# jeffreychou777/GenComm

Hardware: AMD Instinct MI355X
Metric: scenes/sec (higher is better)
Workload: dtype f32

## Files before the change

gencomm_amd/_lib.py:

```python
from __future__ import annotations

import ctypes as C
import os
import shutil
import subprocess
import threading
from typing import List, Tuple

PKG_DIR = os.path.dirname(os.path.abspath(__file__))
REPO_DIR = os.path.dirname(PKG_DIR)
CSRC_DIR = os.path.join(PKG_DIR, "csrc")
LIB_PATH = os.environ.get("GENCOMM_HIP_LIB", os.path.join(PKG_DIR, "libgencomm_hip.so"))
ABI_VERSION = 12
MODE_ARITH, MODE_SAMPLER, MODE_TILE_WANT, MODE_ENH_FUSE, MODE_CONV8H_MASK, MODE_XCD_REMAP, MODE_DATAFLOW, MODE_RESFUSE_EMU, MODE_TILE8, MODE_BWD_STREAMS, MODE_PERSIST = range(11)

_lock = threading.Lock()
_lib = None

c_float_p = C.c_void_p
_i, _ll, _p = C.c_int, C.c_longlong, C.c_void_p

_SIGNATURES = {
    "gencomm_abi_version": (_i, []),
    "gencomm_last_error": (C.c_char_p, []),
    "gencomm_build_info": (C.c_char_p, []),
    "gencomm_set_mode": (_i, [_i, _ll]),
    "gencomm_get_mode": (_ll, [_i]),
    "gencomm_timer_num_kernels": (_i, []),
    "gencomm_timer_kernel_name": (C.c_char_p, [_i]),
    "gencomm_timer_start": (_i, [_i, _i]),
    "gencomm_timer_stop": (_i, [C.POINTER(C.c_double), C.POINTER(_i)]),
    "gencomm_timer_start_mask": (_i, [C.c_ulonglong, _i]),
    "gencomm_timer_stop_families": (_i, [C.POINTER(C.c_double), C.POINTER(_i), C.POINTER(C.c_double), _i]),
    "gencomm_klog_start": (_i, []),
    "gencomm_klog_stop": (_i, [C.c_char_p, _i]),
    "gencomm_clock_probe": (_i, [_p, _i, _p]),
    "gencomm_quad_iou_fwd": (_i, [_p, _i, _p, _i, _p, _p]),
    "gencomm_unet_num_params": (_i, [_i, _i, _i, _i]),
    "gencomm_unet_param_info": (_i, [_i, _i, _i, _i, _i, C.c_char_p, _i, C.POINTER(_ll), C.POINTER(_ll)]),
    "gencomm_unet_raw_floats": (_ll, [_i, _i, _i, _i]),
    "gencomm_unet_prepared_floats": (_ll, [_i, _i, _i, _i, _i]),
    "gencomm_unet_prepare": (_i, [_p, _p, _i, _i, _i, _i, _i, _p]),
    "gencomm_unet_bwd_workspace_bytes": (_ll, [_i, _i, _i, _i, _i, _i, _i]),
    "gencomm_unet_fwd_train": (_i, [_p, _p, _p, _p, _i, _i, _i, _i, _i, _i, _i, _i, _i, _p, _ll, _p]),
    "gencomm_unet_fwd_train_step": (_i, [_p, _p, _p, _p, _i, _p, _p, C.c_ulonglong, _i, _i, _i, _i, _i, _i, _i, _i, _p, _ll, _p]),
    "gencomm_unet_bwd": (_i, [_p, _p, _p, _p, _i, _p, _p, _p, _p, _i, _i, _i, _i, _i, _i, _i, _i, _i, _p, _ll, _p]),
    "gencomm_unet_bwd_chain": (_i, [_p, _p, _p, _p, _i, _p, C.c_float, C.c_float, _p, _p, _p, _p, _i, _i, _i, _i, _i, _i, _i, _i, _i, _p, _ll, _p]),
    "gencomm_conv8_fwd": (_i, [_p, _p, _p, _p, _p, _p, _i, _i, _i, _i, _p]),
    "gencomm_denoise_workspace_bytes": (_ll, [_i, _i, _i, _i, _i, _i, _i]),
    "gencomm_dataflow_error": (_i, [_p, _i, _i, _i, _i, _i, _i, _i, _p]),
    "gencomm_dataflow_words": (_i, [_p, _i, _i, _i, _i, _i, _i, _i, C.POINTER(C.c_uint), _i, _p]),
    "gencomm_unet_fwd": (_i, [_p, _p, _p, _p, _i, _i, _i, _i, _i, _i, _i, _i, _i, _p, _ll, _p]),
    "gencomm_denoise_fwd": (_i, [_p, _p, _p, _i, _p, _p, _p, _p, _p, C.c_ulonglong,
                                 _i, _i, _i, _i, _i, _i, _i, _i, _p, _ll, _p]),
    "gencomm_denoise_fwd_dseed": (_i, [_p, _p, _p, _i, _p, _p, _p, _p, _p, C.c_ulonglong, _p,
                                       _i, _i, _i, _i, _i, _i, _i, _i, _p, _ll, _p]),
    "gencomm_q_sample_fwd": (_i, [_p, _p, _i, _p, _p, C.c_ulonglong, C.c_uint, _p, _i, _i, _i, _i, _p]),
    "gencomm_step_noise_fwd": (_i, [_p, C.c_ulonglong, C.c_uint, _p, _i, _i, _i, _i, _i, _p]),
    "gencomm_enhancer_num_params": (_i, [_i]),
    "gencomm_enhancer_param_info": (_i, [_i, _i, C.c_char_p, _i, C.POINTER(_ll), C.POINTER(_ll)]),
    "gencomm_enhancer_raw_floats": (_ll, [_i]),
    "gencomm_enhancer_workspace_bytes": (_ll, [_i, _i, _i, _i]),
    "gencomm_enhancer_fwd": (_i, [_p, _p, _p, _i, _i, _i, _i, _p, _ll, _p]),
    "gencomm_msgext_num_params": (_i, [_i]),
    "gencomm_msgext_param_info": (_i, [_i, _i, C.c_char_p, _i, C.POINTER(_ll), C.POINTER(_ll)]),
    "gencomm_msgext_raw_floats": (_ll, [_i]),
    "gencomm_msgext_workspace_bytes": (_ll, [_i, _i, _i, _i]),
    "gencomm_msgext_fwd": (_i, [_p, _p, _p, _i, _i, _i, _i, _p, _ll, _p]),
    "gencomm_pillar_encode_fwd": (_i, [_p, _p, _p, _p, _p, _p, _p, _p, _p, _p, _i, _i, _i, _i, _i,
                                       C.POINTER(C.c_float), C.POINTER(C.c_float), _p]),
    "gencomm_conv2d_prepare": (_i, [_p, _p, _i, _i, _i, _i, _i, _p]),
    "gencomm_conv2d_prepared_floats": (_ll, [_i, _i, _i, _i, _i]),
    "gencomm_conv2d_fold": (_i, [_p, _p, _p, _p, _p, C.c_float, _i, _p, _p, _p]),
    "gencomm_conv2d_fwd": (_i, [_p, _p, _p, _p, _p] + [_i] * 13 + [_p]),
    "gencomm_conv2d_act_res_fwd": (_i, [_p, _p, _p, _p, _p, _p] + [_i] * 10 + [_p]),
    "gencomm_split3_attn_fwd": (_i, [_p] * 10 + [_i, _i, _i, _p]),
    "gencomm_warp_affine_bwd": (_i, [_p, _p, _p, _i, _i, _i, _i, _p]),
    "gencomm_hgt_attn_bwd": (_i, [_p, _p, _p, _p, _i, _i, _i, _i, _p]),
    "gencomm_win_attn_bwd_scratch_floats": (_ll, [_i, _i, _i, _i, _i]),
    "gencomm_win_attn_bwd": (_i, [_p] * 7 + [_i] * 6 + [_p]),
    "gencomm_conv2d_wgrad": (_i, [_p, _p, _p, _p, _i, _i, _i, _i, _i, _i, _i, _i, _p]),
    "gencomm_conv2d_wgrad_scratch_floats": (_ll, [_i] * 8),
    "gencomm_conv2d_wgrad_ws": (_i, [_p, _p, _p, _p, _i, _i, _i, _i, _i, _i, _i, _i, _p, _ll, _p]),
    "gencomm_conv2d_wgrad_fixed_scratch_floats": (_ll, [_i] * 6),
    "gencomm_conv2d_wgrad_fixed": (_i, [_p, _p, _p, _p, _i, _i, _i, _i, _i, _i, _p, _ll, _p]),
    "gencomm_gn_nchw_fwd": (_i, [_p, _p, _p, _p, _p, C.c_float, _i, _i, _i, _i, _i, _p]),
    "gencomm_ln_nchw_fwd": (_i, [_p, _p, _p, _p, C.c_float, _i, _i, _i, _i, _p]),
    "gencomm_ln_nchw_bwd": (_i, [_p, _p, _p, _p, _p, _p, _p, C.c_float, _i, _i, _i, _i, _p]),
    "gencomm_dwconv3x3_fwd": (_i, [_p, _p, _p, _p, _i, _i, _i, _i, _i, _p]),
    "gencomm_dwconv3x3_wgrad": (_i, [_p, _p, _p, _p, _i, _i, _i, _i, _p]),
    "gencomm_conv3x3_c16_scratch_floats": (_ll, []),
    "gencomm_conv3x3_c16_fwd": (_i, [_p, _i, _p, _i, _p, _i, _p, _i, _i, _i, _p]),
    "gencomm_dwconv3x3_act_fwd": (_i, [_p, _i, _i, _p, _p, _p, _i, _i, _i, _i, _i, _p]),
    "gencomm_dwconv3x3_act_wgrad": (_i, [_p, _i, _i, _p, _p, _p, _i, _i, _i, _i, _p]),
    "gencomm_gelu_bwd": (_i, [_p, _p, _p, _ll, _p]),
    "gencomm_lincomb_fwd": (_i, [_p, _p, _p, _p, C.c_float, C.c_float, C.c_float, _ll, _p]),
    "gencomm_ew_slice_fwd": (_i, [_i, _p, _p, _p, _p, _p, _p] + [_i] * 9 + [_p]),
    "gencomm_nc_scale_fwd": (_i, [_p, _p, _p, _p, _i, _i, _i, _p]),
    "gencomm_nc_dot_fwd": (_i, [_p, _p, _p, _i, _i, _i, _p]),
    "gencomm_det_workspace_bytes": (C.c_longlong, [_i, _i, _i]),
    "gencomm_nms_workspace_bytes": (C.c_longlong, []),
    "gencomm_nms_max_candidates": (_i, []),
    "gencomm_det_decode_fwd": (_i, [_p, _p, _p, _p, _p, _i, _i, _i, _i, C.c_float, C.c_float, _i, _p, _p, _p, _p, _i, _p, C.c_longlong, _p]),
    "gencomm_nms_rotated_fwd": (_i, [_p, _p, _p, C.c_float, _i, _p, _p, _p, _p, _p, _p, C.c_longlong, _p]),
    "gencomm_bbox_overlaps_fwd": (_i, [_p, _p, _p, _i, _i, _p]),
    "gencomm_det_mc_workspace_bytes": (_ll, [_p, _p, _i, _i]),
    "gencomm_det_mc_decode_fwd": (_i, [_p, _p, _p, _p, _p, _p, _i, _i, _i, C.c_float, _i, _p, _p, _p, _p, _p, _p, _i, _p, _ll, _p]),
    "gencomm_det_mc_gather_fwd": (_i, [_p, _p, _p, _p, _p, _i, _i, _p, _p, _p]),
    "gencomm_warp_affine_fwd": (_i, [_p, _p, _p, _i, _i, _i, _i, _p]),
    "gencomm_hgt_attn_fwd": (_i, [_p, _p, _p, _i, _i, _i, _i, _p]),
    "gencomm_win_attn_fwd": (_i, [_p, _p, _p, _i, _i, _i, _i, _i, _i, _p]),
    "gencomm_swap_attn_fwd": (_i, [_p, _p, _p, _p] + [_i] * 8 + [_p]),
    "gencomm_swap_attn_train_fwd": (_i, [_p] * 5 + [_i] * 8 + [_p]),
    "gencomm_swap_attn_bwd": (_i, [_p] * 8 + [_i] * 8 + [_p]),
    "gencomm_agent_mean_fwd": (_i, [_p, _p, _i, _i, _ll, _p]),
    "gencomm_v2v_warp_pairs_fwd": (_i, [_p, _p, _p, _p, _i, _i, _i, _i, _p]),
    "gencomm_v2v_aggregate_fwd": (_i, [_p] * 7 + [_i] * 6 + [_p]),
    "gencomm_gru_gate_fwd": (_i, [_p, _p, _i, _i, _i, _p]),
    "gencomm_gru_gate_bwd": (_i, [_p, _p, _p, _i, _i, _i, _p]),
    "gencomm_v2v_aggregate_train_fwd": (_i, [_p] * 8 + [_i] * 6 + [_p]),
    "gencomm_v2v_aggregate_bwd": (_i, [_p] * 7 + [_i] * 6 + [_p]),
    "gencomm_v2v_warp_pairs_bwd_scratch_floats": (_ll, [_i]),
    "gencomm_v2v_warp_pairs_bwd": (_i, [_p] * 7 + [_i] * 6 + [_p]),
    "gencomm_umgm_param_floats": (_ll, [_i, _i, C.POINTER(_i), _i]),
    "gencomm_umgm_workspace_bytes": (_ll, [_ll, _i]),
    "gencomm_umgm_fwd": (_i, [_p, _p, _p, _p, C.c_ulonglong, _i, _p, _p, _p, _p, _p, _ll, _i, _i, _i, C.POINTER(_i), _i, _p, _ll, _p]),
    "gencomm_umgm_encode_fwd": (_i, [_p, _p, _p, _ll, _i, _i, _i, C.POINTER(_i), _i, _p]),
    "gencomm_umgm_decode_fwd": (_i, [_p, _p, _p, _ll, _i, _i, _i, C.POINTER(_i), _i, _p]),
    "gencomm_umgm_noise_fwd": (_i, [_p, C.c_ulonglong, _ll, _i, C.POINTER(_i), _i, _p]),
    "gencomm_umgm_bwd_workspace_bytes": (_ll, [_ll, _i, _i, C.POINTER(_i), _i]),
    "gencomm_umgm_bwd": (_i, [_p, _p, _p, _p, C.c_ulonglong, _i, _p, _p, _p, _p, _p, _i, _ll, _i, _i, _i, C.POINTER(_i), _i, _p, _ll, _p]),
    "gencomm_rows_wgrad_fixed_scratch_floats": (_ll, [_ll, _i, _i]),
    "gencomm_rows_wgrad_fixed": (_i, [_p, _p, _p, _ll, _i, _i, _p, _ll, _p]),
    "gencomm_convnext_block_fwd": (_i, [_p] * 11 + [_i] * 4 + [_p]),
    "gencomm_convnext_block_bwd_workspace_bytes": (_ll, [_i] * 6),
    "gencomm_convnext_block_bwd": (_i, [_p] * 21 + [_i] * 6 + [_p, _ll, _p]),
    "gencomm_gconv3x3_prepare": (_i, [_p, _p, _i, _p]),
    "gencomm_gconv3x3_fwd": (_i, [_p] * 5 + [_i] * 7 + [_p]),
    "gencomm_pyramid_score_fwd": (_i, [_p] * 6 + [_i] * 4 + [_p]),
    "gencomm_warp_weightfuse_fwd": (_i, [_p] * 5 + [_i] * 5 + [_p]),
    "gencomm_iou3d_pairwise_fwd": (_i, [_p, _i, _p, _i, _i, _p, _p]),
    "gencomm_iou3d_max_boxes": (_i, []),
    "gencomm_iou3d_nms_workspace_bytes": (_ll, [_i]),
    "gencomm_iou3d_nms_fwd": (_i, [_p, _i, C.c_float, _i, _p, _p, _p, _ll, _p]),
    "gencomm_bn2d_train_fwd": (_i, [_p, _p, _p, _p, _p, _p, _p, _p, C.c_float, C.c_float, _i, _i, _i, _i, _p, _p]),
    "gencomm_bn2d_train_bwd": (_i, [_p, _p, _p, _p, _p, _p, _p, _p, _p, _i, _i, _i, _i, _p]),
    "gencomm_slot_max_fwd": (_i, [_p, _p, _p, _i, _i, _i, _p]),
    "gencomm_convbn_train_fwd": (_i, [_p] * 10 + [C.c_float, C.c_float, _i] + [_p] * 5 + [_i] * 8 + [_p]),
    "gencomm_convbn_train_bwd": (_i, [_p] * 9 + [_i] + [_p] * 9 + [_ll] + [_i] * 7 + [_p]),
    "gencomm_pfn_train_fwd": (_i, [_p, _p, _p, _p, _p, _p, _p, C.c_float, C.c_float, _p, _p, _p, _p, _i, _i, _i, _i, _p]),
    "gencomm_pfn_train_bwd": (_i, [_p, _p, _p, _p, _p, _p, _p, _p, _p, _p, _p, _p, _i, _i, _i, _i, _p]),
    "gencomm_pfn_moment_doubles": (_ll, [_i]),
    "gencomm_pfn_bwd_scratch_doubles": (_ll, [_i, _i]),
    "gencomm_slot_max_bwd": (_i, [_p, _p, _p, _i, _i, _i, _p]),
    "gencomm_head_loss": (_i, [_p] * 10 + [_i] * 5 + [_p, C.c_double] + [C.c_float] * 7 + [_i, _p]),
    "gencomm_head_loss_mc": (_i, [_p] * 4 + [_i] + [_p] * 4 + [_i] * 5 + [C.c_double] * 2 + [_p]),
    "gencomm_target_assign_workspace_bytes": (_ll, [_i, _i, _i]),
    "gencomm_target_standup_fwd": (_i, [_p, _i, _i, _p, _p]),
    "gencomm_target_assign_fwd": (_i, [_p, _i, _i, _p, _i, _p, _p, _p, _p] + [_i] * 6 + [_p, _p, _p, _i, _p, _ll, _p]),
    "gencomm_dcn_sample_fwd": (_i, [_p, _p, _p, _i, _i, _i, _i, _p]),
    "gencomm_dcn_scatter_bwd": (_i, [_p, _p, _p, _p, _p, _i, _i, _i, _i, _p]),
    "gencomm_dcn_scatter_scratch_floats": (_ll, [_i, _i, _i, _i]),
    "gencomm_dcn_scatter_bwd_ws": (_i, [_p, _p, _p, _p, _p, _i, _i, _i, _i, _p, _ll, _p]),
    "gencomm_sp_out_dims": (_i, [_p, _p, _p, _p, _p]),
    "gencomm_sp_index_workspace_bytes": (_ll, [_i]),
    "gencomm_sp_index_fwd": (_i, [_p, _i, _i, _p, _p, _p, _p, _ll, _p]),
    "gencomm_sp_sites_capacity": (_ll, [_i, _p, _p]),
    "gencomm_sp_sites_workspace_bytes": (_ll, [_i, _p, _p]),
    "gencomm_sp_sites_fwd": (_i, [_p, _i, _i, _p, _p, _p, _p, _p, _p, _p, _ll, _p]),
    "gencomm_sp_rules_fwd": (_i, [_p, _i, _p, _i, _i, _p, _p, _p, _p, _p, _p]),
    "gencomm_sp_prepared_floats": (_ll, [_i, _i, _i]),
    "gencomm_sp_prepare": (_i, [_p, _p, _i, _i, _i, _i, _p]),
    "gencomm_sp_conv_fwd": (_i, [_p, _p, _p, _p, _p, _p, _i, _i, _i, _i, _i, _p]),
    "gencomm_sp_dense_fwd": (_i, [_p, _p, _i, _i, _i, _p, _p, _p]),
    "gencomm_mean_vfe_fwd": (_i, [_p, _p, _p, _p, _i, _i, _i, _p]),
    "gencomm_bnrow_train_fwd": (_i, [_p, _p, _p, _p, _p, _p, _p, _p, C.c_float, C.c_float, _i, _i, _i, _p]),
    "gencomm_bnrow_train_bwd": (_i, [_p, _p, _p, _p, _p, _p, _p, _p, _p, _i, _i, _i, _p]),
    "gencomm_sp_rules_inv_fwd": (_i, [_p, _i, _p, _i, _i, _p, _p, _p, _p, _p, _p]),
    "gencomm_sp_wgrad": (_i, [_p, _p, _p, _p, _i, _i, _i, _i, _p]),
    "gencomm_voxelize_workspace_bytes": (_ll, [_i]),
    "gencomm_voxelize_fwd": (_i, [_p, _i, _i, C.POINTER(C.c_float), C.POINTER(C.c_float), _i, _i, _p, _p, _p, _p, _p, _ll, _p]),
    "gencomm_voxelize_batch_workspace_bytes": (_ll, [_i, _i, _i]),
    "gencomm_voxelize_batch_fwd": (_i, [_p, _i, _i, _p, _i, _p, _p, _i, C.POINTER(C.c_float), C.POINTER(C.c_float), _i, _i, _i, _p, _p, _p, _p, _p, _p, _ll, _p]),
    "gencomm_warp_attfuse_fwd": (_i, [_p, _p, _p, _p, _i, _i, _i, _i, _i, _p]),
    "gencomm_warp_attfuse_bwd_scratch_floats": (_ll, [_i, _i, _i]),
    "gencomm_warp_attfuse_bwd": (_i, [_p, _p, _p, _p, _p, _p, _i, _i, _i, _i, _i, _p]),
    "gencomm_warp_maxfuse_fwd": (_i, [_p, _p, _p, _p, _i, _i, _i, _i, _i, _p]),
    "gencomm_warp_maxfuse_bwd_scratch_floats": (_ll, [_i, _i, _i, _i, _i]),
    "gencomm_warp_maxfuse_bwd": (_i, [_p, _p, _p, _p, _p, _p, _i, _i, _i, _i, _i, _p]),
    "gencomm_warp_attfuse_tok_fwd": (_i, [_p, _p, _p, _p, _i, _i, _i, _i, _i, _p]),
    "gencomm_lss_workspace_bytes": (_ll, [_i, _i, _i, _i, _i, _i, C.POINTER(_i)]),
    "gencomm_lss_splat_fwd": (_i, [_p] * 8 + [C.POINTER(C.c_float), C.POINTER(C.c_float), C.POINTER(_i)] + [_i] * 6 + [_p, _p, _p, _ll, _p]),
    "gencomm_lss_depth_target_fwd": (_i, [_p, _i, _i, _i, _i, _i, _i, C.c_float, C.c_float, _i, _p, _p, _p]),
    "gencomm_maxpool3x3s2_fwd": (_i, [_p, _p, _i, _i, _i, _i, _p]),
    "gencomm_lss_splat_bwd_workspace_bytes": (_ll, [_i, _i, C.POINTER(_i)]),
    "gencomm_lss_splat_bwd": (_i, [_p, _p, _ll, _p, C.POINTER(_i)] + [_i] * 6 + [_p, _p, _p, _ll, _p]),
    "gencomm_maxpool3x3s2_bwd": (_i, [_p, _p, _p, _i, _i, _i, _i, _p]),
    "gencomm_stem7x7_wgrad_scratch_floats": (_ll, [_i] * 5),
    "gencomm_stem7x7_wgrad": (_i, [_p, _p, _p] + [_i] * 5 + [_p, _ll, _p]),
    "gencomm_depth_focal_loss": (_i, [_p, _p, _p, _p, _i, _i, _i, _i, C.c_float, C.c_float, C.c_float, _p]),
}
EXPORTED_SYMBOLS = tuple(_SIGNATURES)


class GenCommHipError(RuntimeError):
    pass


def hip_sources() -> List[str]:
    return [os.path.join(CSRC_DIR, "gencomm_abi.hip"), os.path.join(CSRC_DIR, "gencomm_abi_aux.hip")]


def source_hash() -> str:
    import hashlib
    h = hashlib.sha256()
    for f in sorted(os.listdir(CSRC_DIR)) + [os.path.join(REPO_DIR, "include", "gencomm_hip.h")]:
# ... 144 lines not shown
```

gencomm_amd/csrc/common.h:

```cpp
#pragma once
#include <hip/hip_runtime.h>
#include <stdint.h>
#include <stdio.h>
#include <string.h>

namespace gc {

constexpr int kWave = 64;
constexpr int kMaxResBlocks = 48;

enum Status : int {
  GC_OK = 0,
  GC_ERR_ARG = 1,
  GC_ERR_WORKSPACE = 2,
  GC_ERR_HIP = 3,
};

char* last_error_buf();
inline int fail(int code, const char* msg) {
  snprintf(last_error_buf(), 512, "%s", msg);
  return code;
}
#define GC_CHECK_ARG(cond, msg) \
  do {                          \
    if (!(cond)) return ::gc::fail(::gc::GC_ERR_ARG, msg); \
  } while (0)
#define GC_HIP(expr)                                                             \
  do {                                                                           \
    hipError_t e__ = (expr);                                                     \
    if (e__ != hipSuccess) {                                                     \
      snprintf(::gc::last_error_buf(), 512, "%s failed: %s", #expr, hipGetErrorString(e__)); \
      return ::gc::GC_ERR_HIP;                                                   \
    }                                                                            \
  } while (0)

struct LdsAttrOnce {
  unsigned long long done = 0;
  template <class K>
  int set(K kernel, int bytes) {
    int d = 0;
    GC_HIP(hipGetDevice(&d));
    const unsigned long long bit = d < 64 ? 1ull << d : 0ull;
    if (done & bit) return 0;
    GC_HIP(hipFuncSetAttribute((const void*)kernel, hipFuncAttributeMaxDynamicSharedMemorySize, bytes));
    __atomic_fetch_or(&done, bit, __ATOMIC_RELAXED);
    return 0;
  }
};

inline size_t align_up(size_t v, size_t a) { return (v + a - 1) / a * a; }

enum ModeKey : int {
  MODE_ARITH = 0,
  MODE_SAMPLER = 1,
  MODE_TILE_WANT = 2,
  MODE_ENH_FUSE = 3,
  MODE_CONV8H_MASK = 4,
  MODE_XCD_REMAP = 5,
  MODE_DATAFLOW = 6,
  MODE_RESFUSE_EMU = 7,
  MODE_TILE8 = 8,
  MODE_BWD_STREAMS = 9,
  MODE_PERSIST = 10,
  MODE_COUNT = 11
};
struct Modes {
  long long v[MODE_COUNT];
  bool split() const { return v[MODE_ARITH] != 1; }
  bool split2() const { return v[MODE_ARITH] == 3; }
  bool bf16() const { return v[MODE_ARITH] == 2; }
  int xcd() const { return v[MODE_XCD_REMAP] != 0 ? 1 : 0; }
};
Modes modes_snapshot();

enum KernelFamily : int {
  KF_CONV_IN = 0, KF_CONV8 = 1, KF_CONV16 = 2, KF_DOWN = 3, KF_UP = 4, KF_CONV_OUT = 5, KF_Q_SAMPLE = 6,
  KF_ENH_LN = 7, KF_ENH_PCONV = 8, KF_ENH_GEMM1 = 9, KF_ENH_DWGATE = 10, KF_ENH_GEMM2 = 11,
  KF_ENH_GATE = 12, KF_ENH_OUT = 13, KF_WARP_ATTFUSE = 14, KF_LATENT_STEP = 15, KF_CONV8_RES1 = 16, KF_CONV8_RES2 = 17,
  KF_DATAFLOW = 18,
  KF_CONV2D = 19,
  KF_COUNT = 20
};
inline const char* kernel_family_name(int id) {
  static const char* names[KF_COUNT] = {
      "conv_in_h_kernel | conv_in_kernel", "conv8h_kernel<1,GN,0> | conv8_kernel (ResnetBlock conv1, 8 -> 8)",
      "conv8h_kernel<2,GN,0> | conv8_kernel (ResnetBlock conv1, 16 -> 8)", "down8x2_kernel | down8_kernel",
      "conv8h_kernel<UP> | conv8_kernel<UP>", "conv_out_h_kernel | conv_out_kernel", "q_sample_kernel", "enh_ln_kernel",
      "enh_pconv_h_kernel | enh_pconv_kernel", "enh_front_h_kernel | gemm_*_mfma_kernel<0>", "enh_dwgate_kernel",
      "gemm_*_mfma_kernel<1>", "enh_gate_kernel", "enh_scale_transpose_kernel", "warp_attfuse_kernel | warp_attfuse_tok_kernel",
      "latent_step_h_kernel | latent_step_kernel", "conv8h_kernel<1,GN,RES=1> | conv8_kernel (ResnetBlock conv2 + identity)",
      "conv8h_kernel<1,GN,RES=2> | conv8_kernel (ResnetBlock conv2 + nin_shortcut)",
      "unet_dataflow_kernel (UNet body of one call, persistent)",
      "conv2d_h3l_kernel | conv2d_h3_kernel | conv2d_igemm_kernel (general 3x3 / 1x1 / 2x2 convolution; slot = FLOPs)"};
  return (id >= 0 && id < KF_COUNT) ? names[id] : "?";
}
struct KernelTimer {
  unsigned long long mask = 0;
  int cap = 0, count = 0;
  hipEvent_t* ev = nullptr;
  int* fam = nullptr;
  double* bytes = nullptr;
};
KernelTimer& kernel_timer();
struct TimedLaunch {
  bool armed;
  hipStream_t st;
  TimedLaunch(int family, hipStream_t s, double algorithmic_bytes = 0.0) : st(s) {
    KernelTimer& t = kernel_timer();
    armed = ((t.mask >> family) & 1ull) && t.count < t.cap;
    if (armed) {
      t.fam[t.count] = family;
      t.bytes[t.count] = algorithmic_bytes;
      (void)hipEventRecord(t.ev[2 * t.count], st);
    }
  }
  ~TimedLaunch() {
    if (armed) {
      KernelTimer& t = kernel_timer();
      (void)hipEventRecord(t.ev[2 * t.count + 1], st);
      ++t.count;
    }
  }
};

bool klog_armed();
void klog_note(const char* name);
#define GC_KLOG(name)                                   \
  do {                                                  \
    if (::gc::klog_armed()) ::gc::klog_note(name);      \
  } while (0)

typedef const float __attribute__((address_space(4)))* cfloat_p;
__device__ __forceinline__ cfloat_p as_const(const float* p) { return (cfloat_p)(p); }

struct BlockId { int x, y, z; };
__device__ __forceinline__ BlockId xcd_block_dims(int remap, unsigned lin, unsigned gx, unsigned gy, unsigned total) {
  unsigned nl = lin;
  if (remap) {
    const unsigned xcd = lin & 7u, j = lin >> 3;
    const unsigned q = total >> 3, r = total & 7u;
    nl = xcd * q + (xcd < r ? xcd : r) + j;
  }
  BlockId b;
  const unsigned row = nl / gx;
  b.x = (int)(nl - row * gx);
  b.z = (int)(row / gy);
  b.y = (int)(row - (unsigned)b.z * gy);
  return b;
}
__device__ __forceinline__ BlockId xcd_block_lin(int remap, unsigned lin) {
  const unsigned gx = gridDim.x, gy = gridDim.y;
  BlockId b;
  {
    const unsigned row = lin / gx;
    b.x = (int)(lin - row * gx);
    b.z = (int)(row / gy);
    b.y = (int)(row - (unsigned)b.z * gy);
  }
  if (remap) {
    const unsigned total = gx * gy * gridDim.z;
    const unsigned xcd = lin & 7u, j = lin >> 3;
    const unsigned q = total >> 3, r = total & 7u;
    const unsigned nl = xcd * q + (xcd < r ? xcd : r) + j;
    const unsigned row = nl / gx;
    b.x = (int)(nl - row * gx);
    b.z = (int)(row / gy);
    b.y = (int)(row - (unsigned)b.z * gy);
  }
  return b;
}
__device__ __forceinline__ BlockId xcd_block(int remap) {
  BlockId b{(int)blockIdx.x, (int)blockIdx.y, (int)blockIdx.z};
  if (remap) {
    const unsigned gx = gridDim.x, gy = gridDim.y;
    const unsigned total = gx * gy * gridDim.z;
    const unsigned lin = blockIdx.x + gx * (blockIdx.y + gy * blockIdx.z);
    const unsigned xcd = lin & 7u, j = lin >> 3;
    const unsigned q = total >> 3, r = total & 7u;
    const unsigned nl = xcd * q + (xcd < r ? xcd : r) + j;
    const unsigned row = nl / gx;
    b.x = (int)(nl - row * gx);
    b.z = (int)(row / gy);
    b.y = (int)(row - (unsigned)b.z * gy);
  }
  return b;
}

__device__ __forceinline__ float sigmoid_f(float x) {
  return __builtin_amdgcn_rcpf(1.0f + __builtin_amdgcn_exp2f(x * -1.4426950408889634f));
}
__device__ __forceinline__ float silu_f(float x) { return x * sigmoid_f(x); }
__device__ __forceinline__ float gelu_erf_f(float x) {
  const float t = fminf(fabsf(x) * 0.70710678118654752440f, 4.3f);
  float q = fmaf(-1.0021018e-4f, t, 4.6151079e-4f);
  q = fmaf(q, t, 2.3023714e-3f);
  q = fmaf(q, t, -2.9452650e-2f);
  q = fmaf(q, t, 1.4896373e-1f);
  q = fmaf(q, t, 9.1832864e-1f);
  q = fmaf(q, t, 1.6279137e+0f);
  const float erf_abs = 1.0f - __builtin_amdgcn_exp2f(-t * q);
  const float h = 0.5f * x;
  return fmaf(h, copysignf(erf_abs, x), h);
}
__device__ __forceinline__ void gelu_and_grad_f(float x, float* gelu, float* grad) {
  const float t = fminf(fabsf(x) * 0.70710678118654752440f, 4.3f);
  float q = fmaf(-1.0021018e-4f, t, 4.6151079e-4f);
  q = fmaf(q, t, 2.3023714e-3f);
  q = fmaf(q, t, -2.9452650e-2f);
  q = fmaf(q, t, 1.4896373e-1f);
  q = fmaf(q, t, 9.1832864e-1f);
  q = fmaf(q, t, 1.6279137e+0f);
  const float erf_abs = 1.0f - __builtin_amdgcn_exp2f(-t * q);
  const float Phi = fmaf(0.5f, copysignf(erf_abs, x), 0.5f);
  const float phi = 0.3989422804014327f * __builtin_amdgcn_exp2f(x * x * -0.72134752044448170368f);
  *gelu = x * Phi;
  *grad = fmaf(x, phi, Phi);
}
// ... 205 lines not shown
```

gencomm_amd/csrc/enhancer_host.h:

```cpp
#pragma once
#include <algorithm>
#include <stdlib.h>
#include <string.h>
#include <string>
#include <vector>

#include "enhancer_kernels.h"
#include "unet_plan.h"

namespace gc {

struct EnhancerPlan {
  int C = 0, dc = 0, dcp = 0, hid = 0;
  std::vector<ParamEntry> params;
  long long raw_floats = 0;
  long long n1w, n1b, n2w, n2b, pcw, l1w, l1b, dww, dwb, l2w, l2b, fc1, bnw, bnb, fc2;

  long long add(const std::string& name, long long numel) {
    params.push_back({name, numel, raw_floats});
    const long long o = raw_floats;
    raw_floats += numel;
    return o;
  }
  const char* build(int C_) {
    if (C_ < 8 || C_ % 8 != 0) return "enhancer: C must be a positive multiple of 8";
    C = C_; dc = C / 4; dcp = (dc + 15) / 16 * 16; hid = 2 * C;
    params.clear(); raw_floats = 0;
    n1w = add("block_1.norm1.weight", C);
    n1b = add("block_1.norm1.bias", C);
    n2w = add("block_1.norm2.weight", C);
    n2b = add("block_1.norm2.bias", C);
    pcw = add("block_1.mlp.partial_conv3.weight", (long long)dc * dc * 9);
    l1w = add("block_1.mlp.linear1.0.weight", (long long)2 * hid * C);
    l1b = add("block_1.mlp.linear1.0.bias", 2 * hid);
    dww = add("block_1.mlp.dwconv.0.weight", (long long)hid * 9);
    dwb = add("block_1.mlp.dwconv.0.bias", hid);
    l2w = add("block_1.mlp.linear2.0.weight", (long long)C * hid);
    l2b = add("block_1.mlp.linear2.0.bias", C);
    fc1 = add("split_attn.fc1.weight", (long long)C * C);
    bnw = add("split_attn.bn1.weight", C);
    bnb = add("split_attn.bn1.bias", C);
    fc2 = add("split_attn.fc2.weight", (long long)C * C);
    return nullptr;
  }
};

struct EnhancerWs {
  size_t Y, Z, Zc, Hd, G, O, colsum, gate, wT, tab1, tab2, wsc, total;
};

inline EnhancerWs enhancer_ws(const EnhancerPlan& p, int n, int H, int W) {
  const size_t M = (size_t)n * H * W;
  EnhancerWs w{};
  size_t off = 0;
  auto take = [&](size_t floats) { const size_t o = off; off += align_up(floats * sizeof(float), 256); return o; };
  w.colsum = take((size_t)n * p.C);
  w.gate = take((size_t)n * p.C);
  w.wT = take(std::max((size_t)9 * p.dc * p.dcp, (size_t)(p.dc / 16) * ((9 * p.dc + 31) / 32) * 896 + 64));
  w.Y = take(M * p.C);
  w.Z = take(M * p.C);
  w.Zc = take(M * p.dc);
  w.Hd = take(M * 2 * p.hid);
  w.G = take(M * p.hid);
  w.O = w.Hd;
  w.tab1 = take((size_t)(p.hid / 16) * (p.C / 16) * 896);
  w.tab2 = take((size_t)(p.hid / 16) * (p.C / 32 > 0 ? p.C / 32 : 1) * 896);
  w.wsc = take(64);
  w.total = off;
  return w;
}
inline int enh_fuse_level(const Modes& m, int C) { return (m.split() && C == 64) ? (int)m.v[MODE_ENH_FUSE] : 0; }
inline size_t enhancer_workspace_bytes(const EnhancerPlan& p, int n, int H, int W) { return enhancer_ws(p, n, H, W).total; }

inline int enhancer_enqueue(const EnhancerPlan& p, const float* raw, const float* x, float* out,
                            int n, int H, int W, char* wsp, hipStream_t st, const Modes& m) {
  const EnhancerWs w = enhancer_ws(p, n, H, W);
  const int HW = H * W, C = p.C;
  auto F = [&](size_t off) { return reinterpret_cast<float*>(wsp + off); };
  GC_HIP(hipMemsetAsync(F(w.colsum), 0, (size_t)n * C * sizeof(float), st));

  {
    EnhLnArgs a{x, raw + p.n1w, raw + p.n1b, raw + p.n2w, raw + p.n2b, F(w.Y), F(w.Z), F(w.Zc), C, p.dc, HW};
    const size_t sh = ((size_t)C * 65 + 256 + 128) * sizeof(float);
    if (sh > 48 * 1024) GC_HIP(hipFuncSetAttribute((const void*)enh_ln_kernel, hipFuncAttributeMaxDynamicSharedMemorySize, (int)sh));
    TimedLaunch tl(KF_ENH_LN, st);
    if (C == 64) enh_ln64_kernel<<<dim3((HW + 255) / 256, n), 256, 0, st>>>(a);
    else enh_ln_kernel<<<dim3((HW + 63) / 64, n), 256, sh, st>>>(a);
  }
  if (m.split() && (p.dc == 16 || p.dc == 32 || p.dc == 64) && (C & 3) == 0) {
    const int nslice = (9 * p.dc + 31) / 32;
    enh_prep_pconv_h_kernel<<<(p.dc / 16) * nslice * 4, 256, 0, st>>>(raw + p.pcw, F(w.wT), p.dc, nslice);
    TimedLaunch tl(KF_ENH_PCONV, st);
    EnhPconvHArgs a{F(w.Zc), F(w.wT), F(w.Z), C, p.dc, H, W, nslice};
    const bool wide = p.dc <= 32 && (long long)((W + 31) / 32) * ((H + 15) / 16) * n >= 256;
    const size_t sh = (size_t)18 * (wide ? 34 : 18) * p.dc * 5;
    if (wide) {
      if (sh > 48 * 1024) GC_HIP(hipFuncSetAttribute((const void*)enh_pconv_h_kernel<32>, hipFuncAttributeMaxDynamicSharedMemorySize, (int)sh));
      enh_pconv_h_kernel<32><<<dim3((W + 31) / 32, (H + 15) / 16, n), 256, sh, st>>>(a);
    } else {
      if (sh > 48 * 1024) GC_HIP(hipFuncSetAttribute((const void*)enh_pconv_h_kernel<16>, hipFuncAttributeMaxDynamicSharedMemorySize, (int)sh));
      enh_pconv_h_kernel<16><<<dim3((W + 15) / 16, (H + 15) / 16, n), 256, sh, st>>>(a);
    }
  } else
  {
    enh_prep_pconv_kernel<<<(9 * p.dc * p.dcp + 255) / 256, 256, 0, st>>>(raw + p.pcw, F(w.wT), p.dc, p.dcp);
    TimedLaunch tl(KF_ENH_PCONV, st);
    EnhPconvArgs a{F(w.Zc), F(w.wT), F(w.Z), C, p.dc, p.dcp, H, W};
    if (p.dc <= 32) {
      const size_t sh = (size_t)18 * 18 * (p.dc + 1) * sizeof(float);
      enh_pconv_kernel<16, 16><<<dim3((W + 15) / 16, (H + 15) / 16, n), 256, sh, st>>>(a);
    } else {
      const size_t sh = (size_t)10 * 18 * (p.dc + 1) * sizeof(float);
      if (sh > 48 * 1024) GC_HIP(hipFuncSetAttribute((const void*)enh_pconv_kernel<16, 8>, hipFuncAttributeMaxDynamicSharedMemorySize, (int)sh));
      enh_pconv_kernel<16, 8><<<dim3((W + 15) / 16, (H + 7) / 8, n), 128, sh, st>>>(a);
    }
  }
  const int fuse = enh_fuse_level(m, C);
  if (fuse != 0) {
    enh_wscale_kernel<<<2, 256, 0, st>>>(raw + p.l1w, (long long)2 * p.hid * C, raw + p.l2w, (long long)C * p.hid, F(w.wsc));
    enh_prep_front_kernel<<<32, 256, 0, st>>>(raw + p.l1w, F(w.tab1), C, p.hid, F(w.wsc));
    if (fuse >= 2) enh_prep_back_kernel<<<16, 256, 0, st>>>(raw + p.l2w, F(w.tab2), C, p.hid, F(w.wsc));
    EnhFrontArgs a{F(w.Z), F(w.tab1), raw + p.l1b, raw + p.dww, raw + p.dwb, F(w.G), C, p.hid, H, W,
                   F(w.tab2), raw + p.l2b, F(w.Y), F(w.O), F(w.colsum), F(w.wsc)};
    TimedLaunch tl(KF_ENH_GEMM1, st);
    if (fuse >= 2) enh_front_h_kernel<true><<<dim3((W + 7) / 8, (H + 7) / 8, n), 256, 0, st>>>(a);
    else enh_front_h_kernel<false><<<dim3((W + 7) / 8, (H + 7) / 8, n), 256, 0, st>>>(a);
  } else {
  {
    GemmArgs a{F(w.Z), raw + p.l1w, raw + p.l1b, nullptr, F(w.Hd), nullptr, HW, 2 * p.hid, C};
    TimedLaunch tl(KF_ENH_GEMM1, st);
    if (m.split() && (C & 3) == 0) gemm_f16s_mfma_kernel<0><<<dim3((HW + 127) / 128, (2 * p.hid + 63) / 64, n), 256, 0, st>>>(a);
    else gemm_f32_mfma_kernel<0><<<dim3((HW + 127) / 128, (2 * p.hid + 63) / 64, n), 256, 0, st>>>(a);
  }
  {
    constexpr int SL = 8;
    EnhDwArgs a{F(w.Hd), raw + p.dww, raw + p.dwb, F(w.G), p.hid, H, W};
    const long long total = (long long)H * ((W + SL - 1) / SL) * p.hid;
    TimedLaunch tl(KF_ENH_DWGATE, st);
    enh_dwgate_kernel<SL><<<dim3((unsigned)((total + 255) / 256), n), 256, 0, st>>>(a);
  }
  }
  float* const Otok = F(w.O);
  if (fuse < 2) {
    GemmArgs a{F(w.G), raw + p.l2w, raw + p.l2b, F(w.Y), F(w.O), F(w.colsum), HW, C, p.hid};
    TimedLaunch tl(KF_ENH_GEMM2, st);
    if (m.split() && (p.hid & 3) == 0) gemm_f16s_mfma_kernel<1><<<dim3((HW + 127) / 128, (C + 63) / 64, n), 256, 0, st>>>(a);
    else gemm_f32_mfma_kernel<1><<<dim3((HW + 127) / 128, (C + 63) / 64, n), 256, 0, st>>>(a);
  }
  {
    EnhGateArgs a{F(w.colsum), raw + p.fc1, raw + p.bnw, raw + p.bnb, raw + p.fc2, F(w.gate), C, 1.0f / (float)HW};
    TimedLaunch tl(KF_ENH_GATE, st);
    enh_gate_kernel<<<n, 256, (2 * C + 8) * sizeof(float), st>>>(a);
  }
  if (out != nullptr) {
    EnhOutArgs a{Otok, F(w.gate), out, C, HW};
    const size_t sh = (size_t)32 * (C + 1) * sizeof(float);
    TimedLaunch tl(KF_ENH_OUT, st);
    enh_scale_transpose_kernel<<<dim3((HW + 31) / 32, n), 256, sh, st>>>(a);
  }
  GC_HIP(hipGetLastError());
  return GC_OK;
}

}
```

gencomm_amd/csrc/enhancer_kernels.h:

```cpp
#pragma once
#include "common.h"

namespace gc {

using f32x16 = __attribute__((ext_vector_type(16))) float;
using ef32x4 = __attribute__((ext_vector_type(4))) float;

struct EnhLnArgs {
  const float* x;
  const float* g1; const float* b1; const float* g2; const float* b2;
  float* Y; float* Z; float* Zc;
  int C, dc, HW;
};

__global__ __launch_bounds__(256) void enh_ln_kernel(const EnhLnArgs a) {
  extern __shared__ float smem[];
  const int C = a.C, S = 65;
  float* tile = smem;
  float* part = smem + (size_t)C * S;
  float* mu = part + 256;
  float* rs = mu + 64;
  const int tid = threadIdx.x, q = tid >> 6, p = tid & 63;
  const int n = blockIdx.y, p0 = blockIdx.x * 64;
  const int np = min(64, a.HW - p0);
  const bool pv = p < np;
  const float* __restrict__ xp = a.x + (size_t)n * C * a.HW + p0;
  for (int c = q; c < C; c += 4) tile[c * S + p] = pv ? xp[(size_t)c * a.HW + p] : 0.f;
  __syncthreads();
  const float invC = 1.0f / (float)C;

  auto moments = [&](float eps) {
    float s = 0.f;
    for (int c = q; c < C; c += 4) s += tile[c * S + p];
    part[q * 64 + p] = s;
    __syncthreads();
    const float m = (part[p] + part[64 + p] + part[128 + p] + part[192 + p]) * invC;
    __syncthreads();
    float v = 0.f;
    for (int c = q; c < C; c += 4) { const float d = tile[c * S + p] - m; v = fmaf(d, d, v); }
    part[q * 64 + p] = v;
    __syncthreads();
    const float var = (part[p] + part[64 + p] + part[128 + p] + part[192 + p]) * invC;
    __syncthreads();
    if (q == 0) { mu[p] = m; rs[p] = 1.0f / sqrtf(var + eps); }
    __syncthreads();
  };

  moments(1e-5f);
  {
    const float m = mu[p], r = rs[p];
    for (int c = q; c < C; c += 4) {
      const float v = tile[c * S + p];
      tile[c * S + p] = v + fmaf((v - m) * r, a.g1[c], a.b1[c]);
    }
  }
  __syncthreads();
  moments(1e-5f);

  float* __restrict__ Yp = a.Y + ((size_t)n * a.HW + p0) * C;
  float* __restrict__ Zp = a.Z + ((size_t)n * a.HW + p0) * C;
  float* __restrict__ Zcp = a.Zc + ((size_t)n * a.HW + p0) * a.dc;
  const int tot = np * C;
  for (int i = tid; i < tot; i += 256) {
    const int pp = i / C, c = i - pp * C;
    const float y = tile[c * S + pp];
    const float z = fmaf((y - mu[pp]) * rs[pp], a.g2[c], a.b2[c]);
    Yp[i] = y;
    Zp[i] = z;
    if (c < a.dc) Zcp[pp * a.dc + c] = z;
  }
}

__global__ __launch_bounds__(256) void enh_ln64_kernel(const EnhLnArgs a) {
  constexpr int C = 64, S = 65;
  __shared__ float tile[4][64 * S];
  const int tid = threadIdx.x, wv = tid >> 6, p = tid & 63;
  const int n = blockIdx.y, p0 = (blockIdx.x * 4 + wv) * 64;
  if (p0 >= a.HW) return;
  const int np = min(64, a.HW - p0);
  const bool pv = p < np;
  const float* __restrict__ xp = a.x + (size_t)n * C * a.HW + p0 + p;
  float v[C];
#pragma unroll
  for (int c = 0; c < C; ++c) v[c] = pv ? xp[(size_t)c * a.HW] : 0.f;
  const float invC = 1.0f / (float)C;
  float s = 0.f;
#pragma unroll
  for (int c = 0; c < C; ++c) s += v[c];
  float m = s * invC, q = 0.f;
#pragma unroll
  for (int c = 0; c < C; ++c) { const float d = v[c] - m; q = fmaf(d, d, q); }
  float r = 1.0f / sqrtf(q * invC + 1e-5f);
#pragma unroll
  for (int c = 0; c < C; ++c) v[c] = v[c] + fmaf((v[c] - m) * r, as_const(a.g1)[c], as_const(a.b1)[c]);
  s = 0.f;
#pragma unroll
  for (int c = 0; c < C; ++c) s += v[c];
  m = s * invC; q = 0.f;
#pragma unroll
  for (int c = 0; c < C; ++c) { const float d = v[c] - m; q = fmaf(d, d, q); }
  r = 1.0f / sqrtf(q * invC + 1e-5f);
  float* __restrict__ tw = tile[wv];
  float* __restrict__ Yp = a.Y + ((size_t)n * a.HW + p0) * C;
  float* __restrict__ Zp = a.Z + ((size_t)n * a.HW + p0) * C;
  float* __restrict__ Zcp = a.Zc + ((size_t)n * a.HW + p0) * a.dc;
  const int tot = np * C;
#pragma unroll
  for (int c = 0; c < C; ++c) tw[p * S + c] = v[c];
  __builtin_amdgcn_wave_barrier();
  for (int i = p; i < tot; i += 64) Yp[i] = tw[(i >> 6) * S + (i & 63)];
  __builtin_amdgcn_wave_barrier();
#pragma unroll
  for (int c = 0; c < C; ++c) tw[p * S + c] = fmaf((v[c] - m) * r, as_const(a.g2)[c], as_const(a.b2)[c]);
  __builtin_amdgcn_wave_barrier();
  for (int i = p; i < tot; i += 64) Zp[i] = tw[(i >> 6) * S + (i & 63)];
  const int totc = np * a.dc;
  for (int i = p; i < totc; i += 64) { const int pp = i / a.dc, c = i - pp * a.dc; Zcp[i] = tw[pp * S + c]; }
}

struct EnhPconvArgs {
  const float* Zc;
  const float* wT;
  float* Z;
  int C, dc, dcp, H, W;
};

template <int TW, int TH>
__global__ __launch_bounds__(TW * TH) void enh_pconv_kernel(const EnhPconvArgs a) {
  extern __shared__ float smem[];
  const int dc = a.dc, PS = dc + 1;
  constexpr int LW = TW + 2, LH = TH + 2;
  const int tid = threadIdx.x, n = blockIdx.z;
  const int x0 = blockIdx.x * TW, y0 = blockIdx.y * TH;
  const float* __restrict__ zp = a.Zc + (size_t)n * a.H * a.W * dc;
  for (int i = tid; i < LH * LW * dc; i += TW * TH) {
    const int pix = i / dc, c = i - pix * dc;
    const int r = pix / LW, col = pix - r * LW;
    const int gy = y0 - 1 + r, gx = x0 - 1 + col;
    float v = 0.f;
    if (gy >= 0 && gy < a.H && gx >= 0 && gx < a.W) v = zp[((size_t)gy * a.W + gx) * dc + c];
    smem[pix * PS + c] = v;
  }
  __syncthreads();
  const int tx = tid % TW, ty = tid / TW;
  const int gy = y0 + ty, gx = x0 + tx;
  const bool ok = gy < a.H && gx < a.W;
  float* __restrict__ op = a.Z + ((size_t)n * a.H * a.W + (size_t)gy * a.W + gx) * a.C;
  for (int ob = 0; ob < dc; ob += 16) {
    float acc[16];
#pragma unroll
    for (int o = 0; o < 16; ++o) acc[o] = 0.f;
#pragma unroll 1
    for (int tap = 0; tap < 9; ++tap) {
      const int dy = tap / 3, dx = tap - dy * 3;
      const float* sp = smem + ((ty + dy) * LW + tx + dx) * PS;
      const float* __restrict__ wp = a.wT + (size_t)tap * dc * a.dcp + ob;
#pragma unroll 4
      for (int ic = 0; ic < dc; ++ic) {
        const float v = sp[ic];
#pragma unroll
        for (int o = 0; o < 16; ++o) acc[o] = fmaf(wp[(size_t)ic * a.dcp + o], v, acc[o]);
      }
    }
    if (ok) {
#pragma unroll
      for (int o = 0; o < 16; ++o) if (ob + o < dc) op[ob + o] = acc[o];
    }
  }
}

__global__ void enh_prep_pconv_kernel(const float* __restrict__ w, float* __restrict__ wT, int dc, int dcp) {
  const int total = 9 * dc * dcp;
  for (int i = blockIdx.x * blockDim.x + threadIdx.x; i < total; i += gridDim.x * blockDim.x) {
    const int tap = i / (dc * dcp), rem = i - tap * dc * dcp, ic = rem / dcp, oc = rem - ic * dcp;
    wT[i] = oc < dc ? w[((size_t)oc * dc + ic) * 9 + tap] : 0.f;
  }
}

struct GemmArgs {
  const float* A; const float* Bw; const float* bias; const float* res;
  float* out; float* colsum;
  int M, N, K;
};

template <int EPI>
__global__ __launch_bounds__(256) void gemm_f32_mfma_kernel(const GemmArgs a) {
  constexpr int BM = 128, BN = 64, KC = 32, S = KC + 2;
  __shared__ __align__(16) float As[BM * S];
  __shared__ __align__(16) float Bs[BN * S];
  const int tid = threadIdx.x, w = tid >> 6, l = tid & 63, r = l & 31, h = l >> 5;
  const int ag = blockIdx.z;
  const int m0 = blockIdx.x * BM, n0 = blockIdx.y * BN;
  const float* __restrict__ Ap = a.A + (size_t)ag * a.M * a.K;
  const bool kvec = (a.K & 3) == 0;

  f32x16 acc0, acc1;
#pragma unroll
  for (int i = 0; i < 16; ++i) { acc0[i] = 0.f; acc1[i] = 0.f; }

  for (int k0 = 0; k0 < a.K; k0 += KC) {
    __syncthreads();
    {
      const int kq = tid & 7, gk = k0 + 4 * kq;
#pragma unroll
      for (int i = 0; i < 4; ++i) {
        const int row = (tid >> 3) + 32 * i, gm = m0 + row;
        float4 v = make_float4(0.f, 0.f, 0.f, 0.f);
        if (gm < a.M) {
          const float* src = Ap + (size_t)gm * a.K + gk;
          if (kvec && gk + 3 < a.K) v = *reinterpret_cast<const float4*>(src);
          else {
            if (gk + 0 < a.K) v.x = src[0];
            if (gk + 1 < a.K) v.y = src[1];
            if (gk + 2 < a.K) v.z = src[2];
            if (gk + 3 < a.K) v.w = src[3];
          }
        }
        float* d = &As[row * S + 4 * kq];
        *reinterpret_cast<float2*>(d) = make_float2(v.x, v.y);
        *reinterpret_cast<float2*>(d + 2) = make_float2(v.z, v.w);
      }
#pragma unroll
      for (int i = 0; i < 2; ++i) {
        const int row = (tid >> 3) + 32 * i, gn = n0 + row;
        float4 v = make_float4(0.f, 0.f, 0.f, 0.f);
        if (gn < a.N) {
          const float* src = a.Bw + (size_t)gn * a.K + gk;
          if (kvec && gk + 3 < a.K) v = *reinterpret_cast<const float4*>(src);
          else {
            if (gk + 0 < a.K) v.x = src[0];
// ... 688 lines not shown
```

gencomm_amd/csrc/gencomm_abi.hip:

```cpp
#include "../../include/gencomm_hip.h"

#include "common.h"
#include "conv_kernels.h"
#include "detect_kernels.h"
#include "enhancer_host.h"
#include "fusion_kernels.h"
#include "msgext_host.h"
#include "noise_kernels.h"
#include "pillar_kernels.h"
#include "pfn_kernels.h"
#include "train_kernels.h"
#include "wgrad_h3_kernels.h"
#include "unet_bwd_host.h"
#include "unet_host.h"

#include <algorithm>
#include <atomic>
#include <map>
#include <mutex>
#include <string>
#include <stdlib.h>
#include <string.h>

namespace gc {
char* last_error_buf() {
  static thread_local char buf[512] = {0};
  return buf;
}
KernelTimer& kernel_timer() {
  static KernelTimer t;
  return t;
}
static std::atomic<long long> g_modes[MODE_COUNT] = {{0}, {0}, {0}, {2}, {-1}, {1}, {0}, {0}, {-1}, {1}, {16}};
static std::atomic<bool> g_klog_armed{false};
static std::mutex g_klog_mu;
static std::map<std::string, int> g_klog;
bool klog_armed() { return g_klog_armed.load(std::memory_order_relaxed); }
void klog_note(const char* name) {
  std::lock_guard<std::mutex> lk(g_klog_mu);
  ++g_klog[name];
}
Modes modes_snapshot() {
  Modes m;
  for (int i = 0; i < MODE_COUNT; ++i) m.v[i] = g_modes[i].load(std::memory_order_relaxed);
  return m;
}
}

using namespace gc;

extern "C" {

int gencomm_abi_version(void) { return GENCOMM_ABI_VERSION; }
#ifndef GENCOMM_BUILD_FLAGS
#define GENCOMM_BUILD_FLAGS "unknown"
#endif
const char* gencomm_build_info(void) { return GENCOMM_BUILD_FLAGS; }
const char* gencomm_last_error(void) { return last_error_buf(); }

int gencomm_set_mode(int key, long long value) {
  GC_CHECK_ARG(key >= 0 && key < MODE_COUNT, "unknown mode key");
  GC_CHECK_ARG(key != MODE_ARITH || (value >= 0 && value <= 3), "GENCOMM_MODE_ARITH: 0 (three-term f16-pipe path), 1 (exact fp32), 2 (bf16 denoise) or 3 (0 + two-term general convolutions)");
  GC_CHECK_ARG(key != MODE_SAMPLER || (value >= 0 && value <= 2), "GENCOMM_MODE_SAMPLER: 0 (automatic), 1 (direct) or 2 (latent)");
  GC_CHECK_ARG(key != MODE_TILE_WANT || value >= 0, "GENCOMM_MODE_TILE_WANT: 0 (automatic) or a positive workgroup count");
  GC_CHECK_ARG(key != MODE_TILE8 || value >= -1, "GENCOMM_MODE_TILE8: -1 (automatic), 0 (off) or a positive workgroup count");
  GC_CHECK_ARG(key != MODE_BWD_STREAMS || (value >= 0 && value <= 2), "GENCOMM_MODE_BWD_STREAMS: 0 (off), 1 (automatic) or 2 (always)");
  GC_CHECK_ARG(key != MODE_PERSIST || (value >= 0 && value <= 31), "GENCOMM_MODE_PERSIST: a mask of the five layer variants (0 .. 31)");
  g_modes[key].store(value, std::memory_order_relaxed);
  return GC_OK;
}
long long gencomm_get_mode(int key) {
  if (key < 0 || key >= MODE_COUNT) { fail(GC_ERR_ARG, "unknown mode key"); return -1; }
  return g_modes[key].load(std::memory_order_relaxed);
}

int gencomm_timer_num_kernels(void) { return KF_COUNT; }
const char* gencomm_timer_kernel_name(int family) { return kernel_family_name(family); }

int gencomm_timer_start_mask(unsigned long long mask, int capacity) {
  KernelTimer& t = kernel_timer();
  GC_CHECK_ARG(t.ev == nullptr, "timer already armed");
  GC_CHECK_ARG(mask != 0 && (mask >> KF_COUNT) == 0 && capacity >= 1 && capacity <= (1 << 20), "bad family mask / capacity");
  t.ev = new hipEvent_t[2 * (size_t)capacity];
  for (int i = 0; i < 2 * capacity; ++i) {
    if (hipEventCreate(&t.ev[i]) != hipSuccess) {
      for (int j = 0; j < i; ++j) (void)hipEventDestroy(t.ev[j]);
      delete[] t.ev;
      t.ev = nullptr;
      return fail(GC_ERR_HIP, "hipEventCreate failed");
    }
  }
  t.fam = new int[capacity];
  t.bytes = new double[capacity];
  t.mask = mask; t.cap = capacity; t.count = 0;
  return GC_OK;
}
int gencomm_timer_start(int family, int capacity) {
  GC_CHECK_ARG(family >= 0 && family < KF_COUNT, "bad family");
  return gencomm_timer_start_mask(1ull << family, capacity);
}

int gencomm_timer_stop_families(double* ms, int* launches, double* algorithmic_bytes, int n_families) {
  KernelTimer& t = kernel_timer();
  GC_CHECK_ARG(t.ev != nullptr, "timer not armed");
  GC_CHECK_ARG(n_families >= 0 && n_families <= KF_COUNT, "bad n_families");
  for (int f = 0; f < n_families; ++f) {
    if (ms) ms[f] = 0.0;
    if (launches) launches[f] = 0;
    if (algorithmic_bytes) algorithmic_bytes[f] = 0.0;
  }
  int rc = GC_OK;
  for (int i = 0; i < t.count; ++i) {
    float e = 0.f;
    if (hipEventSynchronize(t.ev[2 * i + 1]) != hipSuccess || hipEventElapsedTime(&e, t.ev[2 * i], t.ev[2 * i + 1]) != hipSuccess)
      rc = fail(GC_ERR_HIP, "event timing failed");
    const int f = t.fam[i];
    if (f < n_families) {
      if (ms) ms[f] += e;
      if (launches) launches[f] += 1;
      if (algorithmic_bytes) algorithmic_bytes[f] += t.bytes[i];
    }
  }
  for (int i = 0; i < 2 * t.cap; ++i) (void)hipEventDestroy(t.ev[i]);
  delete[] t.ev;
  delete[] t.fam;
  delete[] t.bytes;
  t = KernelTimer{};
  return rc;
}

int gencomm_timer_stop(double* total_ms, int* launches) {
  double ms[KF_COUNT];
  int n[KF_COUNT];
  const int rc = gencomm_timer_stop_families(ms, n, nullptr, KF_COUNT);
  double sum = 0.0;
  int cnt = 0;
  for (int f = 0; f < KF_COUNT; ++f) { sum += ms[f]; cnt += n[f]; }
  if (total_ms) *total_ms = sum;
  if (launches) *launches = cnt;
  return rc;
}

int gencomm_klog_start(void) {
  std::lock_guard<std::mutex> lk(g_klog_mu);
  g_klog.clear();
  g_klog_armed.store(true, std::memory_order_relaxed);
  return GC_OK;
}
__global__ void clock_probe_kernel(unsigned long long* out, long long spin_ticks) {
  const unsigned long long w0 = wall_clock64(), c0 = clock64();
  unsigned long long w1 = w0;
  while ((long long)(w1 - w0) < spin_ticks) w1 = wall_clock64();
  const unsigned long long c1 = clock64();
  if (threadIdx.x == 0) { out[0] = c1 - c0; out[1] = w1 - w0; }
}
int gencomm_clock_probe(unsigned long long* out_dev, int spin_us, void* stream) {
  GC_CHECK_ARG(out_dev && spin_us >= 1 && spin_us <= 100000, "bad arguments");
  clock_probe_kernel<<<1, 64, 0, (hipStream_t)stream>>>(out_dev, (long long)spin_us * 100);
  GC_HIP(hipGetLastError());
  return GC_OK;
}

int gencomm_klog_stop(char* buf, int cap) {
  g_klog_armed.store(false, std::memory_order_relaxed);
  std::lock_guard<std::mutex> lk(g_klog_mu);
  std::string out;
  for (const auto& kv : g_klog) out += kv.first + "\t" + std::to_string(kv.second) + "\n";
  g_klog.clear();
  GC_CHECK_ARG(buf != nullptr && cap > 0, "null buffer");
  GC_CHECK_ARG((int)out.size() < cap, "buffer too small for the kernel log");
  memcpy(buf, out.c_str(), out.size() + 1);
  return GC_OK;
}

#ifdef GC_STAMPS
int gencomm_diag_read_stamps(unsigned long long* host, int nblocks) {
  GC_HIP(hipDeviceSynchronize());
  GC_HIP(hipMemcpyFromSymbol(host, HIP_SYMBOL(gc::g_stamps), (size_t)nblocks * 8 * sizeof(unsigned long long)));
  return GC_OK;
}
#endif

int gencomm_unet_num_params(int C, int levels, int res_blocks, int attn_mask) {
  UNetPlan p;
  if (const char* e = p.build(C, levels, res_blocks, attn_mask, 1)) { fail(GC_ERR_ARG, e); return -1; }
  return (int)p.params.size();
}

int gencomm_unet_param_info(int C, int levels, int res_blocks, int attn_mask, int index, char* name, int name_cap,
                            long long* numel, long long* offset) {
  UNetPlan p;
  if (const char* e = p.build(C, levels, res_blocks, attn_mask, 1)) return fail(GC_ERR_ARG, e);
  GC_CHECK_ARG(index >= 0 && index < (int)p.params.size(), "param index out of range");
  GC_CHECK_ARG(name && name_cap > 0 && numel && offset, "null output pointer");
  snprintf(name, (size_t)name_cap, "%s", p.params[index].name.c_str());
  *numel = p.params[index].numel;
  *offset = p.params[index].off;
  return GC_OK;
}

long long gencomm_unet_raw_floats(int C, int levels, int res_blocks, int attn_mask) {
  UNetPlan p;
  if (const char* e = p.build(C, levels, res_blocks, attn_mask, 1)) { fail(GC_ERR_ARG, e); return -1; }
  return p.raw_floats;
}

long long gencomm_unet_prepared_floats(int C, int levels, int res_blocks, int attn_mask, int T) {
  UNetPlan p;
  if (const char* e = p.build(C, levels, res_blocks, attn_mask, T)) { fail(GC_ERR_ARG, e); return -1; }
  return p.prepared_floats;
}

int gencomm_unet_prepare(const float* raw, float* prepared, int C, int levels, int res_blocks, int attn_mask, int T, void* stream) {
  UNetPlan p;
  if (const char* e = p.build(C, levels, res_blocks, attn_mask, T)) return fail(GC_ERR_ARG, e);
  GC_CHECK_ARG(raw && prepared, "null pointer");
  return unet_prepare_enqueue(p, raw, prepared, (hipStream_t)stream);
}

long long gencomm_denoise_workspace_bytes(int n, int C, int H, int W, int levels, int res_blocks, int attn_mask) {
// ... 99 lines not shown
}

int gencomm_unet_fwd_train_step(const float* prepared, const float* x_t, const float* cond, float* x_prev, int t, const float* sched_row,
                                const float* step_noise, unsigned long long seed, int n, int C, int H, int W, int levels, int res_blocks,
                                int attn_mask, int T, void* workspace, long long workspace_bytes, void* stream) {
  UNetPlan p;
  if (const char* e = p.build(C, levels, res_blocks, attn_mask, T, true)) return fail(GC_ERR_ARG, e);
  if (int rc = check_dims(n, C, H, W)) return rc;
  GC_CHECK_ARG(attn_mask == 0, "gencomm_unet_fwd_train_step: AttnBlock backward is not implemented (attn_mask must be 0)");
  GC_CHECK_ARG(prepared && x_t && cond && x_prev && sched_row && workspace && x_prev != x_t, "null pointer / in place (x_t is kept for the backward)");
  GC_CHECK_ARG(t >= 1 && t < T, "timestep out of range (step 0 has no update: gencomm_unet_fwd_train)");
  UNetWorkspace w;
  if (const char* e = w.build(p, n, H, W)) return fail(GC_ERR_ARG, e);
  const UNetBwdWs bw = unet_bwd_ws(p, w, n, H, W);
  if ((long long)bw.total > workspace_bytes) return fail(GC_ERR_WORKSPACE, "workspace too small (see gencomm_unet_bwd_workspace_bytes)");
  UNetCall c{&p, &w, prepared, (char*)workspace, n, H, W, (hipStream_t)stream, modes_snapshot()};
  GC_CHECK_ARG(!c.m.bf16(), "gencomm_unet_fwd_train_step keeps fp32 intermediates: not available in bf16 denoise mode (GENCOMM_MODE_ARITH = 2)");
  GC_HIP(hipMemsetAsync(c.amax(), 0, 256, c.st));
  amax_kernel<<<256, 256, 0, c.st>>>(cond, (long long)n * 2 * H * W, c.amax());
  amax_kernel<<<1024, 256, 0, c.st>>>(x_t, (long long)n * C * H * W, c.amax() + 1);
  ConvOutArgs co{};
  co.out = x_prev;
  co.xt = x_t;
  co.sched = sched_row;
  co.noise = step_noise;
  co.seed = seed;
  co.stream_id = (unsigned)t;
  const int rc = unet_enqueue(c, x_t, cond, t, step_noise != nullptr ? 1 : 2, co);
  return rc;
}

int gencomm_unet_bwd_chain(const float* prepared, const float* raw, const float* x_t, const float* cond, int t, const float* grad_x0,
                           float alpha, float beta, const float* d_prev, float* grad_xt, float* grad_cond, float* grad_raw, int n, int C,
                           int H, int W, int levels, int res_blocks, int attn_mask, int T, int forward_done, void* workspace,
                           long long workspace_bytes, void* stream) {
  UNetPlan p;
  if (const char* e = p.build(C, levels, res_blocks, attn_mask, T, true)) return fail(GC_ERR_ARG, e);
  if (int rc = check_dims(n, C, H, W)) return rc;
  GC_CHECK_ARG(attn_mask == 0, "gencomm_unet_bwd: AttnBlock backward is not implemented (attn_mask must be 0)");
  GC_CHECK_ARG(prepared && raw && x_t && cond && grad_x0 && grad_xt && grad_cond && grad_raw && workspace, "null pointer");
  GC_CHECK_ARG(d_prev != grad_xt, "grad_xt must not alias d_prev (tiles read d_prev while others write grad_xt)");
  GC_CHECK_ARG(t >= 0 && t < T, "timestep out of range");
  UNetWorkspace w;
  if (const char* e = w.build(p, n, H, W)) return fail(GC_ERR_ARG, e);
  const UNetBwdWs bw = unet_bwd_ws(p, w, n, H, W);
  if ((long long)bw.total > workspace_bytes) return fail(GC_ERR_WORKSPACE, "workspace too small (see gencomm_unet_bwd_workspace_bytes)");
  const std::vector<DgradEntry> dg = dgrad_entries(p);
  UNetBwdCall b{UNetCall{&p, &w, prepared, (char*)workspace, n, H, W, (hipStream_t)stream, modes_snapshot()}, &bw, raw, grad_raw};
  b.dg = &dg;
  if (d_prev != nullptr) { b.chain_alpha = alpha; b.chain_beta = beta; b.chain_prev = d_prev; }
  GC_CHECK_ARG(!b.c.m.bf16(), "gencomm_unet_bwd reads fp32 intermediates: not available in bf16 denoise mode (GENCOMM_MODE_ARITH = 2)");
  return unet_bwd_enqueue(b, x_t, cond, t, grad_x0, grad_xt, grad_cond, forward_done != 0);
}
int gencomm_unet_bwd(const float* prepared, const float* raw, const float* x_t, const float* cond, int t, const float* grad_x0,
                     float* grad_xt, float* grad_cond, float* grad_raw, int n, int C, int H, int W, int levels, int res_blocks,
                     int attn_mask, int T, int forward_done, void* workspace, long long workspace_bytes, void* stream) {
  return gencomm_unet_bwd_chain(prepared, raw, x_t, cond, t, grad_x0, 1.0f, 0.0f, nullptr, grad_xt, grad_cond, grad_raw, n, C, H, W, levels,
                                res_blocks, attn_mask, T, forward_done, workspace, workspace_bytes, stream);
}

int gencomm_conv8_fwd(const float* src, const float* w_oihw, const float* bias, float* dst, double* dstat,
                      float* scratch, int n, int H, int W, int split, void* stream) {
  GC_CHECK_ARG(src && w_oihw && bias && dst && scratch, "null pointer");
  GC_CHECK_ARG(n >= 1 && n <= 65535 && H >= 1 && W >= 1, "bad n/H/W");
  hipStream_t st = (hipStream_t)stream;
  float* p_w = scratch;
  float* p_wh = scratch + 1024;
  float* p_b = scratch + 3840;
  prep_conv_w_kernel<<<cdiv(576, 256), 256, 0, st>>>(w_oihw, p_w, 8, 8, 8);
  prep_conv8h_kernel<<<1, 256, 0, st>>>(w_oihw, p_wh, 8);
  GC_HIP(hipMemcpyAsync(p_b, bias, 8 * sizeof(float), hipMemcpyDeviceToDevice, st));
  if (dstat) GC_HIP(hipMemsetAsync(dstat, 0, (size_t)n * 16 * sizeof(double), st));
  float* p_amax = scratch + 3856;
  GC_HIP(hipMemsetAsync(p_amax, 0, sizeof(float), st));
  amax_kernel<<<256, 256, 0, st>>>(src, (long long)n * 8 * H * W, p_amax);
  const Modes m = modes_snapshot();
  Conv8Args a{};
  a.src[0] = src; a.w = p_w; a.wh = split ? p_wh : nullptr; a.bias = p_b; a.dst = dst; a.dstat = dstat;
  a.H = a.Hin = H; a.W = a.Win = W;
  a.xcd = m.xcd();
  a.amax = p_amax;
  if (split & 0x100) {
    a.term_mask = split & 63;
    conv8h_kernel<1, false, false, 0, true><<<dim3(cdiv(W, 64), cdiv(H, 16), n), 256, 0, st>>>(a);
    GC_HIP(hipGetLastError());
    return GC_OK;
  }
  launch_conv8<1, false, false, 0>(m, pick_tile(m, n, H, W), a, n, st);
  GC_HIP(hipGetLastError());
  return GC_OK;
}

__global__ void prep_c16_kernel(const float* __restrict__ w, float* __restrict__ dst , int transposed) {
  const int i = blockIdx.x * blockDim.x + threadIdx.x;
  if (i < 8) dst[2 * 1152 + i] = 0.f;
  if (i >= 2 * 1152) return;
  const int o = i & 7, tap = (i >> 3) % 9, ic = (i / 72) & 15, g = i / 1152;
  const int oc = 8 * g + o;
  dst[i] = transposed ? w[((size_t)ic * 16 + oc) * 9 + (8 - tap)] : w[((size_t)oc * 16 + ic) * 9 + tap];
}
long long gencomm_conv3x3_c16_scratch_floats(void) { return 2 * 1152 + 64; }
int gencomm_conv3x3_c16_fwd(const float* x, int x_ct, const float* w, int transposed, float* y, int y_ct, float* scratch, int n, int H, int W,
                            void* stream) {
  GC_CHECK_ARG(x && w && y && scratch && n >= 1 && H >= 1 && W >= 1 && x_ct >= 16 && y_ct >= 16 && (transposed == 0 || transposed == 1), "bad arguments");
  GC_CHECK_ARG(x != y, "in place is not supported (a tile reads its neighbours' pixels)");
  hipStream_t st = (hipStream_t)stream;
  prep_c16_kernel<<<cdiv(2 * 1152, 256), 256, 0, st>>>(w, scratch, transposed);
  Modes m = modes_snapshot();
  m.v[MODE_ARITH] = 1;
  const size_t plane = (size_t)H * W;
  for (int g = 0; g < 2; ++g) {
    Conv8Args a{};
    a.src[0] = x; a.src[1] = x + 8 * plane; a.src_ct = x_ct;
    a.w = scratch + g * 1152; a.bias = scratch + 2 * 1152;
    a.dst = y + (size_t)8 * g * plane; a.dst_ct = y_ct;
    a.H = a.Hin = H; a.W = a.Win = W;
    a.xcd = m.xcd();
    launch_conv8<2, false, false, 0>(m, pick_tile(m, n, H, W), a, n, st);
  }
  GC_HIP(hipGetLastError());
  return GC_OK;
}

static void launch_q_sample(const QSampleArgs& q, int n, bool philox, hipStream_t st) {
  TimedLaunch tl(KF_Q_SAMPLE, st);
  const dim3 qgrid((unsigned)std::max<long long>(1, std::min<long long>((q.per_agent / 64 + 255) / 256, 2048)), n);
  GC_KLOG(philox ? "q_sample_kernel<true> (in-kernel Philox)" : "q_sample_kernel<false> (explicit noise)");
  if (philox) q_sample_kernel<true><<<qgrid, 256, 0, st>>>(q);
  else q_sample_kernel<false><<<qgrid, 256, 0, st>>>(q);
}

int gencomm_q_sample_fwd(const float* sched_row, const float* feat, int n_feat_rows, const int* src_row,
                         const float* noise, unsigned long long seed, unsigned int stream_id,
                         float* out, int n, int C, int H, int W, void* stream) {
  GC_CHECK_ARG(sched_row && feat && src_row && out, "null pointer");
  GC_CHECK_ARG(n >= 1 && n <= 65535 && n_feat_rows >= 1 && C >= 1 && H >= 1 && W >= 1, "bad n/C/H/W");
  QSampleArgs q{feat, src_row, noise, sched_row, out, seed, stream_id, (long long)C * H * W, nullptr, nullptr};
  launch_q_sample(q, n, noise == nullptr, (hipStream_t)stream);
  GC_HIP(hipGetLastError());
  return GC_OK;
}

int gencomm_step_noise_fwd(const float* sched_row, unsigned long long seed, unsigned int stream_id, float* out,
                           int n, int C, int H, int W, int unrounded, void* stream) {
  GC_CHECK_ARG(sched_row && out, "null pointer");
  GC_CHECK_ARG(n >= 1 && n <= 65535 && C >= 2 && (C & 1) == 0 && H >= 1 && W >= 1, "bad n/C/H/W (C must be even)");
  StepNoiseArgs a{out, sched_row, seed, stream_id, C, H, W, unrounded ? 1 : 0, (long long)n * (C / 2) * H * ((W + 3) / 4)};
  const unsigned grid = (unsigned)std::max<long long>(1, std::min<long long>((a.items + 255) / 256, 65536));
  step_noise_kernel<<<grid, 256, 0, (hipStream_t)stream>>>(a);
  GC_HIP(hipGetLastError());
  return GC_OK;
}

int gencomm_denoise_fwd(const float* prepared, const float* sched,
                        const float* feat, int n_feat_rows, const int* src_row, const float* cond,
                        float* out, const float* noise0, const float* step_noise, unsigned long long seed,
                        int n, int C, int H, int W, int levels, int res_blocks, int attn_mask, int T,
                        void* workspace, long long workspace_bytes, void* stream) {
  return gencomm_denoise_fwd_dseed(prepared, sched, feat, n_feat_rows, src_row, cond, out, noise0, step_noise, seed, nullptr,
                                   n, C, H, W, levels, res_blocks, attn_mask, T, workspace, workspace_bytes, stream);
}

int gencomm_denoise_fwd_dseed(const float* prepared, const float* sched,
                              const float* feat, int n_feat_rows, const int* src_row, const float* cond,
                              float* out, const float* noise0, const float* step_noise, unsigned long long seed,
                              const unsigned long long* seed_dev,
                              int n, int C, int H, int W, int levels, int res_blocks, int attn_mask, int T,
                              void* workspace, long long workspace_bytes, void* stream) {
  UNetPlan p;
  if (const char* e = p.build(C, levels, res_blocks, attn_mask, T)) return fail(GC_ERR_ARG, e);
  if (int rc = check_dims(n, C, H, W)) return rc;
  GC_CHECK_ARG(prepared && sched && feat && src_row && cond && out && workspace, "null pointer");
  GC_CHECK_ARG(n_feat_rows >= 1, "n_feat_rows must be positive");
  GC_CHECK_ARG((noise0 == nullptr) == (step_noise == nullptr), "noise0 and step_noise must both be given or both be null");
  UNetWorkspace w;
  if (const char* e = w.build(p, n, H, W)) return fail(GC_ERR_ARG, e);
  if ((long long)w.total > workspace_bytes) return fail(GC_ERR_WORKSPACE, "workspace too small (see gencomm_denoise_workspace_bytes)");
  hipStream_t st = (hipStream_t)stream;
  const bool philox = noise0 == nullptr;
  const long long per_agent = (long long)C * H * W;

  UNetCall c{&p, &w, prepared, (char*)workspace, n, H, W, st, modes_snapshot()};
  if (int rc = check_bf16_mode(c.m, p, W)) return rc;
  GC_HIP(hipMemsetAsync(c.amax(), 0, 256, st));
  amax_kernel<<<256, 256, 0, st>>>(cond, (long long)n * 2 * H * W, c.amax());
  QSampleArgs q{feat, src_row, noise0, sched + (size_t)(T - 1) * 5, out, seed, (unsigned)T, per_agent, seed_dev, c.amax() + 1};
  launch_q_sample(q, n, philox, st);

  const long long smode = c.m.v[MODE_SAMPLER];
  const bool want_latent = smode == 2 || (smode == 0 && pick_tile(c.m, n, H, W) == TILE_64x16);
  const bool latent = want_latent && T >= 2 && (W % 4) == 0;
  if (!latent) {
    for (int i = 0; i < T; ++i) {
      const int t = T - 1 - i;
      ConvOutArgs co{};
      co.out = out;
      co.xt = out;
      co.sched = sched + (size_t)t * 5;
      co.noise = philox ? nullptr : step_noise + (size_t)i * n * per_agent;
      co.seed = seed;
      co.seed_dev = seed_dev;
      co.stream_id = (unsigned)t;
      const int post = t == 0 ? 0 : (philox ? 2 : 1);
      if (int rc = unet_enqueue(c, out, cond, t, post, co)) return rc;
    }
    return GC_OK;
  }
  const int nops = (int)p.ops.size();
  kmap_enqueue(c, cond);
  for (int i = 0; i < T; ++i) {
    const int t = T - 1 - i;
    ConvOutArgs co{};
    co.out = out;
    if (int rc = unet_enqueue_range(c, out, cond, t, 0, co, i == 0 ? 0 : 1, t == 0 ? nops : nops - 1, i != 0, i == 0)) return rc;
    if (t > 0) {
      const float* nz = philox ? nullptr : step_noise + (size_t)i * n * per_agent;
      if (int rc = latent_step_enqueue(c, sched + (size_t)t * 5, nz, seed, (unsigned)t, seed_dev)) return rc;
    }
  }
  return GC_OK;
}

int gencomm_enhancer_num_params(int C) {
  EnhancerPlan p;
  if (const char* e = p.build(C)) { fail(GC_ERR_ARG, e); return -1; }
  return (int)p.params.size();
}
int gencomm_enhancer_param_info(int C, int index, char* name, int name_cap, long long* numel, long long* offset) {
  EnhancerPlan p;
  if (const char* e = p.build(C)) return fail(GC_ERR_ARG, e);
  GC_CHECK_ARG(index >= 0 && index < (int)p.params.size(), "param index out of range");
  GC_CHECK_ARG(name && name_cap > 0 && numel && offset, "null output pointer");
  snprintf(name, (size_t)name_cap, "%s", p.params[index].name.c_str());
  *numel = p.params[index].numel;
  *offset = p.params[index].off;
  return GC_OK;
}
long long gencomm_enhancer_raw_floats(int C) {
  EnhancerPlan p;
  if (const char* e = p.build(C)) { fail(GC_ERR_ARG, e); return -1; }
  return p.raw_floats;
}
long long gencomm_enhancer_workspace_bytes(int n, int C, int H, int W) {
  EnhancerPlan p;
  if (const char* e = p.build(C)) { fail(GC_ERR_ARG, e); return -1; }
  if (n < 1 || H < 1 || W < 1) { fail(GC_ERR_ARG, "n, H, W must be positive"); return -1; }
  return (long long)enhancer_workspace_bytes(p, n, H, W);
}
int gencomm_enhancer_fwd(const float* raw, const float* x, float* out, int n, int C, int H, int W,
                         void* workspace, long long workspace_bytes, void* stream) {
  EnhancerPlan p;
  if (const char* e = p.build(C)) return fail(GC_ERR_ARG, e);
  GC_CHECK_ARG(raw && x && workspace, "null pointer");
  GC_CHECK_ARG(n >= 1 && n <= 65535 && H >= 1 && W >= 1, "bad n/H/W");
  if ((long long)enhancer_workspace_bytes(p, n, H, W) > workspace_bytes)
    return fail(GC_ERR_WORKSPACE, "workspace too small (see gencomm_enhancer_workspace_bytes)");
  return enhancer_enqueue(p, raw, x, out, n, H, W, (char*)workspace, (hipStream_t)stream, modes_snapshot());
}

int gencomm_msgext_num_params(int C) {
  MsgExtPlan p;
  if (const char* e = p.build(C)) { fail(GC_ERR_ARG, e); return -1; }
  return (int)p.params.size();
}
int gencomm_msgext_param_info(int C, int index, char* name, int name_cap, long long* numel, long long* offset) {
  MsgExtPlan p;
  if (const char* e = p.build(C)) return fail(GC_ERR_ARG, e);
  GC_CHECK_ARG(index >= 0 && index < (int)p.params.size(), "param index out of range");
  GC_CHECK_ARG(name && name_cap > 0 && numel && offset, "null output pointer");
  snprintf(name, (size_t)name_cap, "%s", p.params[index].name.c_str());
  *numel = p.params[index].numel;
  *offset = p.params[index].off;
  return GC_OK;
}
long long gencomm_msgext_raw_floats(int C) {
  MsgExtPlan p;
  if (const char* e = p.build(C)) { fail(GC_ERR_ARG, e); return -1; }
  return p.raw_floats;
}
long long gencomm_msgext_workspace_bytes(int n, int C, int H, int W) {
  MsgExtPlan p;
  if (const char* e = p.build(C)) { fail(GC_ERR_ARG, e); return -1; }
  if (n < 1 || H < 1 || W < 1) { fail(GC_ERR_ARG, "n, H, W must be positive"); return -1; }
  return (long long)msgext_ws(p, n, H, W).total;
}
int gencomm_msgext_fwd(const float* raw, const float* x, float* out, int n, int C, int H, int W,
                       void* workspace, long long workspace_bytes, void* stream) {
  MsgExtPlan p;
  if (const char* e = p.build(C)) return fail(GC_ERR_ARG, e);
  GC_CHECK_ARG(raw && x && out && workspace, "null pointer");
  GC_CHECK_ARG(n >= 1 && n <= 65535 && H >= 1 && W >= 1 && (long long)H * W * (C + 64) < (1LL << 31), "bad n/H/W");
  if ((long long)msgext_ws(p, n, H, W).total > workspace_bytes)
    return fail(GC_ERR_WORKSPACE, "workspace too small (see gencomm_msgext_workspace_bytes)");
  return msgext_enqueue(p, raw, x, out, n, H, W, (char*)workspace, (hipStream_t)stream);
}

int gencomm_pillar_encode_fwd(const float* voxel_features, const int* voxel_num_points, const int* voxel_coords,
                              const float* linear_w, const float* bn_weight, const float* bn_bias,
                              const float* bn_running_mean, const float* bn_running_var,
                              float* out, float* scratch128, int M, int P, int B, int nx, int ny,
                              const float* voxel_size3, const float* pc_range6, void* stream) {
  GC_CHECK_ARG(voxel_features && voxel_num_points && voxel_coords && linear_w && bn_weight && bn_bias &&
               bn_running_mean && bn_running_var && out && scratch128 && voxel_size3 && pc_range6, "null pointer");
  GC_CHECK_ARG(M >= 0 && P >= 1 && P <= 32 && B >= 1 && nx >= 1 && ny >= 1, "bad M/P/B/nx/ny (P <= 32 point slots)");
  hipStream_t st = (hipStream_t)stream;
  GC_HIP(hipMemsetAsync(out, 0, (size_t)B * 64 * nx * ny * sizeof(float), st));
  bn_fold_kernel<<<1, 64, 0, st>>>(bn_weight, bn_bias, bn_running_mean, bn_running_var, 1e-3f, scratch128, scratch128 + 64, 64);
  if (M > 0) {
    PillarArgs a{voxel_features, voxel_num_points, voxel_coords, linear_w, scratch128, scratch128 + 64, out, M, P, B, nx, ny,
                 voxel_size3[0], voxel_size3[1], voxel_size3[2],
                 voxel_size3[0] / 2 + pc_range6[0], voxel_size3[1] / 2 + pc_range6[1], voxel_size3[2] / 2 + pc_range6[2]};
    pillar_vfe_scatter_kernel<<<(M + 3) / 4, 256, 0, st>>>(a);
  }
  GC_HIP(hipGetLastError());
  return GC_OK;
}

int gencomm_conv2d_prepare(const float* weight, float* prepared, int Cin, int Cout, int KH, int KW, int transposed, void* stream) {
  GC_CHECK_ARG(weight && prepared, "null pointer");
  GC_CHECK_ARG(Cin >= 1 && Cout >= 1 && KH >= 1 && KW >= 1, "bad Cin/Cout/KH/KW");
  GC_CHECK_ARG(transposed >= 0 && transposed <= 2, "transposed: 0 (Conv2d), 1 (ConvTranspose2d, kernel == stride) or 2 (input-gradient convolution)");
  const long long total = (long long)Cin * Cout * KH * KW;
  const int M = transposed == 1 ? Cout * KH * KW : Cout, T = transposed == 1 ? 1 : KH * KW;
  if (h3_eligible(Cin, M, transposed == 1 ? 1 : KH, transposed == 1 ? 1 : KW)) {
    unsigned char* blob = reinterpret_cast<unsigned char*>(prepared + total);
    PrepW3Args a{weight, prepared, blob, reinterpret_cast<float*>(blob + h3_blob_bytes(Cin, M, T)), Cin, Cout, KH, KW, transposed,
                 M, T, h3_chunks(Cin), h3_blocks(M)};
    GC_CHECK_ARG(a.nchunk <= 65535 && T <= 65535, "too many input-channel chunks");
    conv_w3_rowscale_kernel<<<16 * a.nb, 256, 0, (hipStream_t)stream>>>(a);
    conv_prep_w3_kernel<<<dim3(a.nb, a.nchunk, T), 128, 0, (hipStream_t)stream>>>(a);
    GC_HIP(hipGetLastError());
    return GC_OK;
  }
  PrepWArgs a{weight, prepared, Cin, Cout, KH, KW, transposed};
  conv_prep_w_kernel<<<(unsigned)((total + 255) / 256), 256, 0, (hipStream_t)stream>>>(a);
  GC_HIP(hipGetLastError());
  return GC_OK;
}
long long gencomm_conv2d_prepared_floats(int Cin, int Cout, int KH, int KW, int transposed) {
  if (Cin < 1 || Cout < 1 || KH < 1 || KW < 1 || transposed < 0 || transposed > 2) {
    fail(GC_ERR_ARG, "gencomm_conv2d_prepared_floats: bad dims");
    return -1;
  }
  return conv2d_prepared_floats(Cin, Cout, KH, KW, transposed);
}
static void conv2d_attach_w3(Conv2dArgs& a, const float* prepared, int KH, int KW) {
  if (!h3_eligible(a.Cin, a.CoutP, KH, KW)) return;
  const unsigned char* blob = reinterpret_cast<const unsigned char*>(prepared + (size_t)a.Cin * a.CoutP * KH * KW);
  a.w3 = blob;
  a.wsc = reinterpret_cast<const float*>(blob + h3_blob_bytes(a.Cin, a.CoutP, KH * KW));
}

int gencomm_conv2d_fold(const float* bn_weight, const float* bn_bias, const float* bn_running_mean, const float* bn_running_var,
                        const float* conv_bias, float eps, int C, float* scale, float* shift, void* stream) {
  GC_CHECK_ARG(scale && shift && C >= 1, "null pointer / bad C");
  GC_CHECK_ARG((bn_weight == nullptr) == (bn_bias == nullptr) && (bn_weight == nullptr) == (bn_running_mean == nullptr) &&
               (bn_weight == nullptr) == (bn_running_var == nullptr), "BatchNorm tensors must be all present or all null");
  FoldArgs a{bn_weight, bn_bias, bn_running_mean, bn_running_var, conv_bias, scale, shift, eps, C};
  conv_fold_kernel<<<(C + 63) / 64, 64, 0, (hipStream_t)stream>>>(a);
  GC_HIP(hipGetLastError());
  return GC_OK;
}

int gencomm_conv2d_fwd(const float* x, const float* prepared, const float* scale, const float* shift, float* y,
                       int N, int Cin, int H, int W, int Cout, int KH, int KW, int stride, int pad, int relu,
                       int ups, int out_ctotal, int out_coff, void* stream) {
  GC_CHECK_ARG(x && prepared && scale && shift && y, "null pointer");
  GC_CHECK_ARG(N >= 1 && Cin >= 1 && H >= 1 && W >= 1 && Cout >= 1 && stride >= 1 && pad >= 0 && ups >= 1, "bad dims");
  const bool subpixel = KH == 2 && KW == 2 && ups == 2 && stride == 1 && pad == 0;
  GC_CHECK_ARG(ups == 1 || subpixel || (KH == 1 && KW == 1 && stride == 1 && pad == 0),
               "ups > 1 runs as a 1x1 GEMM (ConvTranspose2d, kernel == stride) or as the 2x2 sub-pixel form of a transposed 3x3 stride-2 convolution");
  GC_CHECK_ARG(out_coff >= 0 && out_coff + Cout <= out_ctotal, "output channel slice out of range");
  const int Ho = subpixel ? H : (H + 2 * pad - KH) / stride + 1, Wo = subpixel ? W : (W + 2 * pad - KW) / stride + 1;
  GC_CHECK_ARG(Ho >= 1 && Wo >= 1, "empty output");
  Conv2dArgs a{x, prepared, scale, shift, y, Cin, H, W, Cout * ups * ups, Ho, Wo, stride, pad, relu, ups, out_ctotal, out_coff};
  conv2d_attach_w3(a, prepared, KH, KW);
  return conv2d_enqueue(a, N, KH, KW, (hipStream_t)stream);
}
int gencomm_conv2d_act_res_fwd(const float* x, const float* prepared, const float* scale, const float* shift, const float* residual, float* y,
                               int N, int Cin, int H, int W, int Cout, int KH, int KW, int stride, int pad, int act, void* stream) {
  GC_CHECK_ARG(x && prepared && scale && shift && y, "null pointer");
  GC_CHECK_ARG(N >= 1 && Cin >= 1 && H >= 1 && W >= 1 && Cout >= 1 && stride >= 1 && pad >= 0 && act >= 0 && act <= 3, "bad dims");
  const int Ho = (H + 2 * pad - KH) / stride + 1, Wo = (W + 2 * pad - KW) / stride + 1;
  GC_CHECK_ARG(Ho >= 1 && Wo >= 1, "empty output");
  Conv2dArgs a{x, prepared, scale, shift, y, Cin, H, W, Cout, Ho, Wo, stride, pad, act, 1, Cout, 0};
  a.res = residual;
  conv2d_attach_w3(a, prepared, KH, KW);
  return conv2d_enqueue(a, N, KH, KW, (hipStream_t)stream);
}

long long gencomm_conv2d_wgrad_scratch_floats(int N, int Cin, int Hi, int Wi, int Cout, int K, int stride, int pad) {
  if (!(N >= 1 && Cin >= 1 && Cout >= 1 && Hi >= 1 && Wi >= 1 && (K == 1 || K == 3) && (stride == 1 || stride == 2) && pad >= 0)) {
    fail(GC_ERR_ARG, "gencomm_conv2d_wgrad_scratch_floats: bad dims");
    return -1;
  }
  const int Ho = (Hi + 2 * pad - K) / stride + 1, Wo = (Wi + 2 * pad - K) / stride + 1;
  if (K == 3 && Cin >= 32 && Cout >= 32 && Ho >= 1 && Wo >= 1) return (long long)wgrad3x3_wide_scratch_floats(N, Cin, Cout, Ho, Wo, stride);
  return 0;
}
int gencomm_conv2d_wgrad_ws(const float* dy, const float* x, float* dw, float* db, int N, int Cin, int Hi, int Wi, int Cout,
                            int K, int stride, int pad, float* scratch, long long scratch_floats, void* stream) {
  GC_CHECK_ARG(dy && x && dw, "null pointer");
  GC_CHECK_ARG(N >= 1 && Cin >= 1 && Cout >= 1 && Hi >= 1 && Wi >= 1 && (K == 1 || K == 3) && (stride == 1 || stride == 2) && pad >= 0, "bad dims");
  const int Ho = (Hi + 2 * pad - K) / stride + 1, Wo = (Wi + 2 * pad - K) / stride + 1;
  GC_CHECK_ARG(Ho >= 1 && Wo >= 1, "empty output");
  if (K == 1 && stride == 1 && pad == 0 && ((Cin >= 32 && Cout >= 32) || ((long long)N * Hi * Wi >= (1 << 16) && std::max(Cin, Cout) >= 32)))
    return wgrad1x1_enqueue(dy, x, dw, db, N, Cin, Cout, Hi * Wi, (hipStream_t)stream);
  if (K == 3 && Cin >= 32 && Cout >= 32) {
    const long long need = (long long)wgrad3x3_wide_scratch_floats(N, Cin, Cout, Ho, Wo, stride);
    GC_CHECK_ARG(scratch == nullptr || scratch_floats >= need, "scratch smaller than gencomm_conv2d_wgrad_scratch_floats");
// ... 451 lines not shown
```

gencomm_amd/csrc/unet_host.h:

```cpp
#pragma once
#include <stdlib.h>

#include "attn_kernels.h"
#include "conv8b_kernels.h"
#include "conv8h_kernels.h"
#include "conv8h8_kernels.h"
#include "dataflow_kernels.h"
#include "latent_kernels.h"
#include "latenth_kernels.h"
#include "unet_kernels.h"
#include "unet_plan.h"

namespace gc {

inline int cdiv(int a, int b) { return (a + b - 1) / b; }

enum TileCfg { TILE_64x16 = 0, TILE_32x16 = 1, TILE_32x8 = 2 };
inline long long tile_want(const Modes& m) {
  return m.v[MODE_TILE_WANT] > 0 ? m.v[MODE_TILE_WANT] : (m.split() ? 160LL : 512LL);
}
inline TileCfg pick_tile(const Modes& m, int n, int H, int W, int zmul = 1) {
  if (m.bf16()) return TILE_64x16;
  const long long want = tile_want(m);
  if ((long long)cdiv(W, 64) * cdiv(H, 16) * n * zmul >= want) return TILE_64x16;
  if ((long long)cdiv(W, 32) * cdiv(H, 16) * n * zmul >= want) return TILE_32x16;
  return TILE_32x8;
}
inline void tile_dims(TileCfg t, int* tw, int* th) {
  *tw = t == TILE_64x16 ? 64 : 32;
  *th = t == TILE_32x8 ? 8 : 16;
}

inline int device_cu_count() {
  static int cus[64] = {0};
  int dev = 0;
  if (hipGetDevice(&dev) != hipSuccess || dev < 0 || dev >= 64) return 256;
  if (cus[dev] == 0) {
    int v = 0;
    if (hipDeviceGetAttribute(&v, hipDeviceAttributeMultiprocessorCount, dev) != hipSuccess || v <= 0) v = 256;
    cus[dev] = v;
  }
  return cus[dev];
}

template <int NSRC, bool GN, bool UP, int RES>
inline void launch_conv8(const Modes& m, TileCfg t, const Conv8Args& a, int n, hipStream_t st) {
  const double abytes = 4.0 * n * ((double)NSRC * 8 * a.Hin * a.Win + (RES == 1 ? 8.0 : RES == 2 ? 16.0 : 0.0) * a.H * a.W + 8.0 * a.H * a.W);
  TimedLaunch tl(UP ? KF_UP : (NSRC == 2 ? KF_CONV16 : (RES == 1 ? KF_CONV8_RES1 : RES == 2 ? KF_CONV8_RES2 : KF_CONV8)), st, abytes);
  int tw, th;
  tile_dims(t, &tw, &th);
  const dim3 grid(cdiv(a.W, tw), cdiv(a.H, th), n);
  const int variant = UP ? 16 : (RES == 2 ? 8 : (RES == 1 ? 4 : (NSRC == 2 ? 2 : 1)));
  if constexpr (RES != 3)
  if (t == TILE_64x16 && a.wh != nullptr && m.split() && (m.v[MODE_CONV8H_MASK] & variant)) {
    if constexpr (GN && !UP) {
      const long long t8 = m.v[MODE_TILE8] >= 0 ? m.v[MODE_TILE8] : (m.v[MODE_TILE_WANT] == 0 ? 256 : 0);
      if (t8 > 0 && (long long)grid.x * grid.y * grid.z < t8 && (a.W & 3) == 0 && a.W >= 4) {
        GC_KLOG(NSRC == 2 ? "conv8h8_kernel<2,GN,0> (64x8 tiles)" : RES == 2 ? "conv8h8_kernel<1,GN,2> (64x8 tiles)" : RES == 1 ? "conv8h8_kernel<1,GN,1> (64x8 tiles)" : "conv8h8_kernel<1,GN,0> (64x8 tiles)");
        conv8h8_kernel<NSRC, GN, RES><<<dim3(cdiv(a.W, 64), cdiv(a.H, 8), n), 256, 0, st>>>(a);
        return;
      }
    }
    if constexpr (GN || UP) {
      const long long tiles = (long long)grid.x * grid.y * grid.z;
      const int slots = 3 * device_cu_count();
      if ((m.v[MODE_PERSIST] & variant) && tiles > slots && (UP ? (a.Win & 1) == 0 : (a.W & 3) == 0)) {
        GC_KLOG(UP ? "conv8hp_kernel<1,0,UP,0> (persistent)" : NSRC == 2 ? "conv8hp_kernel<2,GN,0,0> (persistent)" : RES == 2 ? "conv8hp_kernel<1,GN,0,2> (persistent)"
                   : RES == 1 ? "conv8hp_kernel<1,GN,0,1> (persistent)" : "conv8hp_kernel<1,GN,0,0> (persistent)");
        conv8hp_kernel<NSRC, GN, UP, RES><<<dim3((unsigned)slots), 256, 0, st>>>(a, (int)grid.x, (int)grid.y, (int)grid.z);
        return;
      }
    }
    GC_KLOG(UP ? "conv8h_kernel<1,0,UP,0>" : NSRC == 2 ? "conv8h_kernel<2,GN,0,0>" : RES == 2 ? "conv8h_kernel<1,GN,0,2>" : RES == 1 ? "conv8h_kernel<1,GN,0,1>" : GN ? "conv8h_kernel<1,GN,0,0>" : "conv8h_kernel<1,0,0,0>");
    conv8h_kernel<NSRC, GN, UP, RES><<<grid, 256, 0, st>>>(a);
    return;
  }
  GC_KLOG(t == TILE_64x16 ? "conv8_kernel<64,16,4,...> (exact fp32)" : t == TILE_32x16 ? "conv8_kernel<32,16,4,...> (exact fp32)" : "conv8_kernel<32,8,1,...> (exact fp32)");
  switch (t) {
    case TILE_64x16: conv8_kernel<64, 16, 4, NSRC, GN, UP, RES><<<grid, 256, 0, st>>>(a); break;
    case TILE_32x16: conv8_kernel<32, 16, 4, NSRC, GN, UP, RES><<<grid, 128, 0, st>>>(a); break;
    default: conv8_kernel<32, 8, 1, NSRC, GN, UP, RES><<<grid, 256, 0, st>>>(a); break;
  }
}

template <int NSRC, bool GN, bool UP, int RES>
inline void launch_conv8b(const Conv8BArgs& a, int n, hipStream_t st) {
  const double elt = 2.0;
  const double abytes = elt * n * ((double)NSRC * 8 * a.Hin * a.Win + (RES == 1 ? 8.0 : RES == 2 ? 16.0 : 0.0) * a.H * a.W + 8.0 * a.H * a.W);
  TimedLaunch tl(UP ? KF_UP : (NSRC == 2 ? KF_CONV16 : (RES == 1 ? KF_CONV8_RES1 : RES == 2 ? KF_CONV8_RES2 : KF_CONV8)), st, abytes);
  GC_KLOG("conv8b_kernel<...> (bf16 storage)");
  conv8b_kernel<NSRC, GN, UP, RES><<<dim3(cdiv(a.W, 64), cdiv(a.H, 16), n), 256, 0, st>>>(a);
}

struct UNetCall {
  const UNetPlan* plan;
  const UNetWorkspace* ws;
  const float* prepared;
  char* wsp;
  int n, H, W;
  hipStream_t st;
  Modes m;
  float* amax() const { return reinterpret_cast<float*>(wsp + ws->amax_off); }
  int is_f32(int id) const { return (!m.bf16() || id == plan->hs0_tensor) ? 1 : 0; }

  float* tensor_ptr(int id) const {
    const TensorPlan& t = plan->tensors[id];
    return reinterpret_cast<float*>(wsp + ws->level_base[t.level] + ws->slot_bytes[t.level] * t.slot);
  }
  double* stat_ptr(int id) const { return reinterpret_cast<double*>(wsp) + (size_t)id * n * 16; }
};

inline Conv8Args conv1_args(const UNetCall& c, const Op& o, int t) {
  const ResBlockPlan& b = c.plan->blocks[o.blk];
  const float* P = c.prepared;
  const int Hl = c.ws->Hl[o.level], Wl = c.ws->Wl[o.level];
  Conv8Args a{};
  a.src[0] = c.tensor_ptr(o.src[0]); a.sstat[0] = c.stat_ptr(o.src[0]);
  if (o.src[1] >= 0) { a.src[1] = c.tensor_ptr(o.src[1]); a.sstat[1] = c.stat_ptr(o.src[1]); }
  a.gamma = P + b.n1w; a.beta = P + b.n1b;
  a.w = P + b.p_c1w; a.wh = P + b.p_c1wh; a.bias = P + b.p_bias1 + (size_t)t * 8;
  a.dst = c.tensor_ptr(o.dst); a.dstat = c.stat_ptr(o.dst);
  a.H = a.Hin = Hl; a.W = a.Win = Wl;
  a.inv_cnt = 1.0 / ((b.cin == 8 ? 2.0 : 4.0) * Hl * Wl);
  a.xcd = c.m.xcd();
  return a;
}
inline Conv8Args conv2_args(const UNetCall& c, const Op& o) {
  const ResBlockPlan& b = c.plan->blocks[o.blk];
  const float* P = c.prepared;
  const int Hl = c.ws->Hl[o.level], Wl = c.ws->Wl[o.level];
  Conv8Args a{};
  a.src[0] = c.tensor_ptr(o.src[0]); a.sstat[0] = c.stat_ptr(o.src[0]);
  a.gamma = P + b.n2w; a.beta = P + b.n2b;
  a.w = P + b.p_c2w; a.wh = P + b.p_c2wh; a.bias = P + b.p_bias2;
  a.res[0] = c.tensor_ptr(o.res[0]);
  if (o.res[1] >= 0) { a.res[1] = c.tensor_ptr(o.res[1]); a.ninw = P + b.p_ninw; }
  a.dst = c.tensor_ptr(o.dst); a.dstat = c.stat_ptr(o.dst);
  a.H = a.Hin = Hl; a.W = a.Win = Wl;
  a.inv_cnt = 1.0 / (2.0 * Hl * Wl);
  a.xcd = c.m.xcd();
  return a;
}
inline Conv8Args up_args(const UNetCall& c, const Op& o) {
  const UNetPlan& p = *c.plan;
  const float* P = c.prepared;
  const int lin = o.level + 1;
  Conv8Args a{};
  a.src[0] = c.tensor_ptr(o.src[0]);
  a.sstat[0] = c.stat_ptr(o.src[0]);
  a.w = P + p.up[lin].p_w; a.wh = P + p.up[lin].p_wh; a.bias = P + p.up[lin].b;
  a.dst = c.tensor_ptr(o.dst); a.dstat = c.stat_ptr(o.dst);
  a.H = c.ws->Hl[o.level]; a.W = c.ws->Wl[o.level]; a.Hin = c.ws->Hl[lin]; a.Win = c.ws->Wl[lin];
  a.xcd = c.m.xcd();
  return a;
}
inline DownArgs down_args(const UNetCall& c, const Op& o) {
  const UNetPlan& p = *c.plan;
  const float* P = c.prepared;
  const int lin = o.level - 1;
  return DownArgs{c.tensor_ptr(o.src[0]), P + p.down[lin].p_w, P + p.down[lin].b, c.tensor_ptr(o.dst), c.stat_ptr(o.dst),
                  c.ws->Hl[o.level], c.ws->Wl[o.level], c.ws->Hl[lin], c.ws->Wl[lin], !c.is_f32(o.src[0]), !c.is_f32(o.dst)};
}

inline bool resfuse_emulated(const UNetCall& c, const ResBlockPlan& b, TileCfg tc, bool wvec) {
  return c.m.v[MODE_RESFUSE_EMU] != 0 && b.cin == 8 && tc == TILE_64x16 && c.m.split() && !c.m.bf16() && wvec;
}

inline bool df_eligible(const UNetCall& c, int f, int l) {
  if (c.m.v[MODE_DATAFLOW] == 0 || !c.m.split() || c.m.bf16() || l - f < 2 || l - f > DF_MAX_OPS || c.n > 64 * 1024) return false;
  if (c.m.v[MODE_CONV8H_MASK] != -1) return false;
  for (int oi = f; oi < l; ++oi) {
    const Op& o = c.plan->ops[oi];
    if (o.kind != OP_RES_CONV1 && o.kind != OP_RES_CONV2 && o.kind != OP_DOWN && o.kind != OP_UP) return false;
    if (o.kind == OP_DOWN) {
      if ((c.ws->Wl[o.level - 1] & 3) != 0) return false;
    } else if (pick_tile(c.m, c.n, c.ws->Hl[o.level], c.ws->Wl[o.level]) != TILE_64x16) return false;
  }
  return true;
}
inline int df_enqueue(const UNetCall& c, int t, int f, int l, bool upload) {
  const UNetPlan& p = *c.plan;
  DfProgram* dprog = reinterpret_cast<DfProgram*>(c.wsp + c.ws->df_prog_off);
  unsigned* words = reinterpret_cast<unsigned*>(c.wsp + c.ws->df_words_off);
  const int nops = l - f;
  if (upload) {
    static thread_local DfProgram hp;
    hp.nops = nops; hp.n = c.n;
    int qlen[8] = {0, 0, 0, 0, 0, 0, 0, 0};
    for (int k = 0; k < nops; ++k) {
      const Op& o = p.ops[f + k];
      DfOp& d = hp.ops[k];
      d = DfOp{};
      const int Hl = c.ws->Hl[o.level], Wl = c.ws->Wl[o.level];
      if (o.kind == OP_DOWN) {
        d.kind = DF_DOWN; d.tx = cdiv(Hl * ((Wl + 1) / 2), 256); d.ty = 1; d.down = down_args(c, o);
      } else {
        d.tx = cdiv(Wl, 64); d.ty = cdiv(Hl, 16);
        if (o.kind == OP_RES_CONV1) {
          d.kind = p.blocks[o.blk].cin == 8 ? DF_CONV1 : DF_CONV16; d.conv = conv1_args(c, o, 0); d.bias_stride = 8;
        } else if (o.kind == OP_RES_CONV2) {
          d.kind = p.blocks[o.blk].cin == 8 ? DF_CONV2_RES1 : DF_CONV2_RES2; d.conv = conv2_args(c, o);
        } else {
          d.kind = DF_UP; d.conv = up_args(c, o);
        }
      }
      d.tiles = d.tx * d.ty;
      d.items = d.tiles * c.n;
      const int qq = d.items >> 3, rr = d.items & 7;
      for (int x = 0; x <= 8; ++x) d.item_base[x] = x * qq + (x < rr ? x : rr);
      for (int x = 0; x < 8; ++x) { d.ticket_base[x] = qlen[x]; qlen[x] += d.item_base[x + 1] - d.item_base[x]; }
    }
    for (int x = 0; x < 8; ++x) hp.queue_len[x] = qlen[x];
    for (int k0 = 0; k0 < nops; k0 += DF_CHUNK) {
      DfUploadArgs ua{};
      ua.dst = dprog; ua.first = k0; ua.count = std::min(DF_CHUNK, nops - k0); ua.nops = nops; ua.n = c.n;
      for (int x = 0; x < 8; ++x) ua.queue_len[x] = qlen[x];
      for (int k = 0; k < ua.count; ++k) ua.ops[k] = hp.ops[k0 + k];
      df_upload_kernel<<<1, 64, 0, c.st>>>(ua);
    }
  }
  int dev = 0, cus = 256;
  if (hipGetDevice(&dev) == hipSuccess) (void)hipDeviceGetAttribute(&cus, hipDeviceAttributeMultiprocessorCount, dev);
  DfArgs da{dprog, words, words + 8, words + 8 + 64 * (size_t)c.n, t, c.m.v[MODE_DATAFLOW] == 2 ? 1 : 0};
  GC_KLOG("unet_dataflow_kernel (persistent, per-agent layer dependencies)");
  TimedLaunch tl(KF_DATAFLOW, c.st);
  unet_dataflow_kernel<<<dim3(3 * cus), HC_NT, 0, c.st>>>(da);
  GC_HIP(hipGetLastError());
  return GC_OK;
}

inline int unet_enqueue_range(const UNetCall& c, const float* x_t, const float* cond, int t, int post,
                              ConvOutArgs co, int first, int last, bool keep_hs0_stats, bool df_upload = true) {
  const UNetPlan& p = *c.plan;
  const float* P = c.prepared;
  {
    const size_t skip = keep_hs0_stats ? (size_t)c.n * 16 * sizeof(double) : 0;
    GC_HIP(hipMemsetAsync(c.wsp + skip, 0, c.ws->stats_bytes - skip, c.st));
  }
  const int df_f = std::max(first, 1), df_l = std::min(last, (int)p.ops.size() - 1);
  const bool dataflow = df_eligible(c, df_f, df_l);
  for (int oi = first; oi < last; ++oi) {
    if (dataflow && oi == df_f) {
      if (int rc = df_enqueue(c, t, df_f, df_l, df_upload)) return rc;
      oi = df_l - 1;
      continue;
    }
    const Op& o = p.ops[oi];
    const int Hl = c.ws->Hl[o.level], Wl = c.ws->Wl[o.level];
    switch (o.kind) {
      case OP_CONV_IN: {
        ConvInArgs a{cond, x_t, P + p.conv_in.p_w, P + p.conv_in.b, c.tensor_ptr(o.dst), c.stat_ptr(o.dst), p.C, Hl, Wl, c.m.xcd()};
        const TileCfg tc = pick_tile(c.m, c.n, Hl, Wl);
        int tw, th;
        tile_dims(tc, &tw, &th);
        const dim3 grid(cdiv(Wl, tw), cdiv(Hl, th), c.n);
        TimedLaunch tl(KF_CONV_IN, c.st);
        if (tc == TILE_64x16 && c.m.split() && (Wl & 3) == 0) {
          ConvInHArgs ah{cond, x_t, P + p.p_wch, P + p.p_wxh, P + p.p_wc5h + HL_W5TAB3, P + p.conv_in.b, c.tensor_ptr(o.dst),
                         c.stat_ptr(o.dst), p.C, Hl, Wl, c.m.xcd(), c.amax()};
          GC_KLOG("conv_in_h_kernel");
          conv_in_h_kernel<<<grid, 256, 0, c.st>>>(ah);
        } else {
          GC_KLOG("conv_in_kernel<tile> (exact fp32)");
          if (tc == TILE_64x16) conv_in_kernel<64, 16, 4><<<grid, 256, 0, c.st>>>(a);
          else if (tc == TILE_32x16) conv_in_kernel<32, 16, 4><<<grid, 128, 0, c.st>>>(a);
          else conv_in_kernel<32, 8, 1><<<grid, 256, 0, c.st>>>(a);
        }
        break;
      }
      case OP_RES_CONV1: {
        const ResBlockPlan& b = p.blocks[o.blk];
        if (c.m.bf16()) {
          Conv8BArgs a{};
          a.src[0] = c.tensor_ptr(o.src[0]); a.src_f32[0] = c.is_f32(o.src[0]); a.sstat[0] = c.stat_ptr(o.src[0]);
          if (o.src[1] >= 0) { a.src[1] = c.tensor_ptr(o.src[1]); a.src_f32[1] = c.is_f32(o.src[1]); a.sstat[1] = c.stat_ptr(o.src[1]); }
          a.gamma = P + b.n1w; a.beta = P + b.n1b; a.wb = P + b.p_c1wb; a.bias = P + b.p_bias1 + (size_t)t * 8;
          a.dst = c.tensor_ptr(o.dst); a.dst_f32 = c.is_f32(o.dst); a.dstat = c.stat_ptr(o.dst);
          a.H = a.Hin = Hl; a.W = a.Win = Wl; a.inv_cnt = 1.0 / ((b.cin == 8 ? 2.0 : 4.0) * Hl * Wl); a.xcd = c.m.xcd();
          if (b.cin == 8) launch_conv8b<1, true, false, 0>(a, c.n, c.st);
          else launch_conv8b<2, true, false, 0>(a, c.n, c.st);
          break;
        }
        const Conv8Args a = conv1_args(c, o, t);
        const TileCfg tc = pick_tile(c.m, c.n, Hl, Wl);
        if (resfuse_emulated(c, b, tc, (Wl & 3) == 0)) {
          Conv8Args e = a;
          e.term_mask = 63 | 64;
          TimedLaunch tl(KF_CONV8, c.st, 4.0 * c.n * 8.0 * Hl * Wl);
          GC_KLOG("conv8h_kernel<1,GN,0,0,DIAG> (MODE_RESFUSE_EMU: statistics only)");
          conv8h_kernel<1, true, false, 0, true><<<dim3(cdiv(Wl, 64), cdiv(Hl, 16), c.n), 256, 0, c.st>>>(e);
          break;
        }
        if (b.cin == 8) launch_conv8<1, true, false, 0>(c.m, tc, a, c.n, c.st);
        else launch_conv8<2, true, false, 0>(c.m, tc, a, c.n, c.st);
        break;
      }
      case OP_RES_CONV2: {
        const ResBlockPlan& b = p.blocks[o.blk];
        if (c.m.bf16()) {
          Conv8BArgs a{};
          a.src[0] = c.tensor_ptr(o.src[0]); a.src_f32[0] = c.is_f32(o.src[0]); a.sstat[0] = c.stat_ptr(o.src[0]);
          a.gamma = P + b.n2w; a.beta = P + b.n2b; a.wb = P + b.p_c2wb; a.bias = P + b.p_bias2;
          a.res[0] = c.tensor_ptr(o.res[0]); a.res_f32[0] = c.is_f32(o.res[0]);
          if (o.res[1] >= 0) { a.res[1] = c.tensor_ptr(o.res[1]); a.res_f32[1] = c.is_f32(o.res[1]); a.ninw = P + b.p_ninw; }
          a.dst = c.tensor_ptr(o.dst); a.dst_f32 = c.is_f32(o.dst); a.dstat = c.stat_ptr(o.dst);
          a.H = a.Hin = Hl; a.W = a.Win = Wl; a.inv_cnt = 1.0 / (2.0 * Hl * Wl); a.xcd = c.m.xcd();
          if (b.cin == 8) launch_conv8b<1, true, false, 1>(a, c.n, c.st);
          else launch_conv8b<1, true, false, 2>(a, c.n, c.st);
          break;
        }
        const Conv8Args a = conv2_args(c, o);
        const TileCfg tc = pick_tile(c.m, c.n, Hl, Wl);
        if (resfuse_emulated(c, b, tc, (Wl & 3) == 0)) {
          Conv8Args e = a;
          e.src[0] = a.res[0]; e.sstat[0] = c.stat_ptr(o.res[0]); e.gamma = P + b.n1w; e.beta = P + b.n1b;
          e.term_mask = 63 | 128;
          TimedLaunch tl(KF_CONV8_RES1, c.st, 4.0 * c.n * 16.0 * Hl * Wl);
          GC_KLOG("conv8h_kernel<1,GN,0,1,DIAG> (MODE_RESFUSE_EMU: block input, double matrix work)");
          conv8h_kernel<1, true, false, 1, true><<<dim3(cdiv(Wl, 64), cdiv(Hl, 16), c.n), 256, 0, c.st>>>(e);
          break;
        }
        if (b.cin == 8) launch_conv8<1, true, false, 1>(c.m, tc, a, c.n, c.st);
        else launch_conv8<1, true, false, 2>(c.m, tc, a, c.n, c.st);
        break;
      }
      case OP_DOWN: {
        const DownArgs a = down_args(c, o);
        TimedLaunch tl(KF_DOWN, c.st, 4.0 * c.n * 8.0 * ((double)a.Hin * a.Win + (double)Hl * Wl));
        GC_KLOG((a.Win & 3) == 0 ? "down8x2_kernel" : "down8_kernel");
        if ((a.Win & 3) == 0) down8x2_kernel<<<dim3(cdiv(Hl * ((Wl + 1) / 2), 256), 1, c.n), 256, 0, c.st>>>(a);
        else down8_kernel<<<dim3(cdiv(Hl * Wl, 256), 1, c.n), 256, 0, c.st>>>(a);
        break;
      }
      case OP_UP: {
        const int lin = o.level + 1;
        if (c.m.bf16()) {
          Conv8BArgs a{};
          a.src[0] = c.tensor_ptr(o.src[0]); a.src_f32[0] = c.is_f32(o.src[0]);
          a.wb = P + p.up[lin].p_wb; a.bias = P + p.up[lin].b;
          a.dst = c.tensor_ptr(o.dst); a.dst_f32 = c.is_f32(o.dst); a.dstat = c.stat_ptr(o.dst);
          a.H = Hl; a.W = Wl; a.Hin = c.ws->Hl[lin]; a.Win = c.ws->Wl[lin]; a.xcd = c.m.xcd();
          launch_conv8b<1, false, true, 0>(a, c.n, c.st);
          break;
        }
        const Conv8Args a = up_args(c, o);
        launch_conv8<1, false, true, 0>(c.m, pick_tile(c.m, c.n, Hl, Wl), a, c.n, c.st);
        break;
      }
      case OP_ATTN: {
        const AttnPlan& at = p.attns[o.blk];
        const int HW = Hl * Wl;
        float* Q = c.tensor_ptr(o.src[1]); float* K = c.tensor_ptr(o.res[0]); float* V = c.tensor_ptr(o.res[1]);
        AttnQkvArgs qa{c.tensor_ptr(o.src[0]), c.stat_ptr(o.src[0]), P + at.nw, P + at.nb, P + at.qw, P + at.qb,
                       P + at.kw, P + at.kb, P + at.vw, P + at.vb, Q, K, V, 1.0 / (2.0 * HW), HW};
        attn_qkv_kernel<<<dim3(cdiv(HW, 256), c.n), 256, 0, c.st>>>(qa);
        AttnFlashArgs fa{Q, K, V, c.tensor_ptr(o.src[0]), P + at.pw, P + at.pb, c.tensor_ptr(o.dst), c.stat_ptr(o.dst), HW};
        if (HW >= 128) attn_flash_mfma_kernel<<<dim3(cdiv(HW, 64), c.n), 512, 0, c.st>>>(fa);
        else attn_flash_kernel<<<dim3(cdiv(HW, 256), c.n), 256, 0, c.st>>>(fa);
        break;
      }
      case OP_CONV_OUT: {
        co.src = c.tensor_ptr(o.src[0]); co.sstat = c.stat_ptr(o.src[0]);
        co.gamma = P + p.nout_w; co.beta = P + p.nout_b;
        co.w = P + p.conv_out.p_w; co.wh = P + p.conv_out.p_wh; co.bias = P + p.conv_out.b;
        co.C = p.C; co.H = Hl; co.W = Wl;
        co.inv_cnt = 1.0 / (2.0 * Hl * Wl);
        co.xcd = c.m.xcd();
        co.amax_out = post != 0 ? c.amax() + 1 : nullptr;
        co.src_bf16 = !c.is_f32(o.src[0]);
        const int nocb = (p.C + 15) / 16;
        const TileCfg tc = pick_tile(c.m, c.n, Hl, Wl, nocb) == TILE_64x16 ? TILE_64x16 : TILE_32x8;
        int tw, th;
        tile_dims(tc, &tw, &th);
        const dim3 grid(cdiv(Wl, tw), cdiv(Hl, th), c.n * nocb);
#define GC_LAUNCH_CO(POST)                                                             \
  do {                                                                                 \
    if (tc == TILE_64x16) conv_out_kernel<64, 16, 4, POST><<<grid, 256, 0, c.st>>>(co); \
    else conv_out_kernel<32, 8, 1, POST><<<grid, 256, 0, c.st>>>(co);                  \
  } while (0)
        TimedLaunch tl(KF_CONV_OUT, c.st);
        if (c.m.split() && (Wl & 3) == 0 && pick_tile(c.m, c.n, Hl, Wl) == TILE_64x16) {
          const dim3 gh(cdiv(Wl, 64), cdiv(Hl, 16), c.n);
          GC_KLOG(post == 0 ? "conv_out_h_kernel<0> (x0_hat)" : post == 1 ? "conv_out_h_kernel<1> (explicit noise)" : "conv_out_h_kernel<2> (in-kernel Philox)");
          if (post == 0) conv_out_h_kernel<0><<<gh, 256, 0, c.st>>>(co);
          else if (post == 1) conv_out_h_kernel<1><<<gh, 256, 0, c.st>>>(co);
          else conv_out_h_kernel<2><<<gh, 256, 0, c.st>>>(co);
        } else {
          GC_KLOG(post == 0 ? "conv_out_kernel<tile,0> (exact fp32, x0_hat)" : post == 1 ? "conv_out_kernel<tile,1> (exact fp32, explicit noise)" : "conv_out_kernel<tile,2> (exact fp32, in-kernel Philox)");
          if (post == 0) GC_LAUNCH_CO(0);
          else if (post == 1) GC_LAUNCH_CO(1);
          else GC_LAUNCH_CO(2);
        }
#undef GC_LAUNCH_CO
        break;
      }
    }
  }
  GC_HIP(hipGetLastError());
  return GC_OK;
}

inline int unet_enqueue(const UNetCall& c, const float* x_t, const float* cond, int t, int post, ConvOutArgs co) {
  return unet_enqueue_range(c, x_t, cond, t, post, co, 0, (int)c.plan->ops.size(), false);
}

inline void kmap_enqueue(const UNetCall& c, const float* cond) {
  const UNetPlan& p = *c.plan;
  ConvInArgs a{cond, nullptr, c.prepared + p.conv_in.p_w, c.prepared + p.conv_in.b,
               reinterpret_cast<float*>(c.wsp + c.ws->kmap_off), nullptr, 0, c.H, c.W, c.m.xcd()};
  const TileCfg tc = pick_tile(c.m, c.n, c.H, c.W);
  int tw, th;
  tile_dims(tc, &tw, &th);
  const dim3 grid(cdiv(c.W, tw), cdiv(c.H, th), c.n);
  if (tc == TILE_64x16 && c.m.split() && (c.W & 3) == 0) {
    ConvInHArgs ah{cond, nullptr, c.prepared + p.p_wch, c.prepared + p.p_wxh, c.prepared + p.p_wc5h + HL_W5TAB3, c.prepared + p.conv_in.b,
                   reinterpret_cast<float*>(c.wsp + c.ws->kmap_off), nullptr, 0, c.H, c.W, c.m.xcd(), c.amax()};
    conv_in_h_kernel<<<grid, 256, 0, c.st>>>(ah);
  } else if (tc == TILE_64x16) conv_in_kernel<64, 16, 4><<<grid, 256, 0, c.st>>>(a);
  else if (tc == TILE_32x16) conv_in_kernel<32, 16, 4><<<grid, 128, 0, c.st>>>(a);
  else conv_in_kernel<32, 8, 1><<<grid, 256, 0, c.st>>>(a);
}

inline int latent_step_enqueue(const UNetCall& c, const float* sched_row, const float* noise, unsigned long long seed,
                               unsigned stream_id, const unsigned long long* seed_dev = nullptr) {
  const UNetPlan& p = *c.plan;
  const float* P = c.prepared;
  GC_HIP(hipMemsetAsync(c.stat_ptr(p.hs0_tensor), 0, (size_t)c.n * 16 * sizeof(double), c.st));
  LatentArgs a{};
  a.a_src = c.tensor_ptr(p.last_body_tensor); a.a_stat = c.stat_ptr(p.last_body_tensor);
  a.gamma = P + p.nout_w; a.beta = P + p.nout_b;
  a.kmap = reinterpret_cast<const float*>(c.wsp + c.ws->kmap_off);
  a.hs0 = c.tensor_ptr(p.hs0_tensor); a.hs0_stat = c.stat_ptr(p.hs0_tensor);
  a.wc5 = P + p.p_wc5; a.wc1 = P + p.p_wc1; a.bring = P + p.p_bring; a.bsum = P + p.p_bsum;
  a.wx = P + p.conv_in.p_w + 144;
  a.wc5h = P + p.p_wc5h; a.wxh = P + p.p_wxh;
  a.noise = noise; a.sched = sched_row; a.inv_cnt = 1.0 / (2.0 * c.H * c.W);
  a.seed = seed; a.seed_dev = seed_dev; a.stream_id = stream_id; a.C = p.C; a.H = c.H; a.W = c.W;
  a.xcd = c.m.xcd();
  a.a_bf16 = !c.is_f32(p.last_body_tensor);
  TimedLaunch tl(KF_LATENT_STEP, c.st, 4.0 * c.n * 32.0 * c.H * c.W);
  const bool small_h = c.m.split() && (c.W & 3) == 0 && c.W >= 64 && c.H >= 16 && c.m.v[MODE_TILE_WANT] == 0;
  if ((pick_tile(c.m, c.n, c.H, c.W) == TILE_64x16 || small_h) && c.m.split()) {
    const dim3 grid(cdiv(c.W, 64), cdiv(c.H, 16), c.n);
    GC_KLOG(noise ? "latent_step_h_kernel<1> (explicit noise)" : "latent_step_h_kernel<2> (in-kernel Philox)");
    if (noise) latent_step_h_kernel<1><<<grid, 256, 0, c.st>>>(a);
    else latent_step_h_kernel<2><<<grid, 256, 0, c.st>>>(a);
  } else if (pick_tile(c.m, c.n, c.H, c.W) == TILE_64x16) {
    const dim3 grid(cdiv(c.W, 64), cdiv(c.H, 16), c.n);
    GC_KLOG(noise ? "latent_step_kernel<64,16,1> (exact fp32, explicit noise)" : "latent_step_kernel<64,16,2> (exact fp32, in-kernel Philox)");
    if (noise) latent_step_kernel<64, 16, 1><<<grid, 256, 0, c.st>>>(a);
    else latent_step_kernel<64, 16, 2><<<grid, 256, 0, c.st>>>(a);
  } else {
    const dim3 grid(cdiv(c.W, 32), cdiv(c.H, 16), c.n);
    GC_KLOG(noise ? "latent_step_kernel<32,16,1> (exact fp32, explicit noise)" : "latent_step_kernel<32,16,2> (exact fp32, in-kernel Philox)");
    if (noise) latent_step_kernel<32, 16, 1><<<grid, 128, 0, c.st>>>(a);
    else latent_step_kernel<32, 16, 2><<<grid, 128, 0, c.st>>>(a);
  }
  GC_HIP(hipGetLastError());
  return GC_OK;
}

inline int unet_prepare_enqueue(const UNetPlan& p, const float* raw, float* prepared, hipStream_t st) {
  GC_HIP(hipMemcpyAsync(prepared, raw, (size_t)p.raw_floats * sizeof(float), hipMemcpyDeviceToDevice, st));
  auto conv_w = [&](long long src, long long dst, int OC, int IC, int OCB) {
    const int total = OC * IC * 9;
    prep_conv_w_kernel<<<cdiv(total, 256), 256, 0, st>>>(raw + src, prepared + dst, OC, IC, OCB);
  };
  conv_w(p.conv_in.w, p.conv_in.p_w, 8, p.C + 2, 8);
  GC_HIP(hipMemsetAsync(prepared + p.conv_out.p_w, 0, (size_t)((p.C + 15) / 16 * 16) * 72 * sizeof(float), st));
  conv_w(p.conv_out.w, p.conv_out.p_w, p.C, 8, 16);
  prep_conv_out_h_kernel<<<1, 256, 0, st>>>(raw + p.conv_out.w, prepared + p.conv_out.p_wh, p.C);
  for (int l = 0; l < p.L; ++l) {
    if (p.down[l].w >= 0) conv_w(p.down[l].w, p.down[l].p_w, 8, 8, 8);
    if (p.up[l].w >= 0) {
      conv_w(p.up[l].w, p.up[l].p_w, 8, 8, 8);
      prep_conv8h_kernel<<<1, 256, 0, st>>>(raw + p.up[l].w, prepared + p.up[l].p_wh, 8);
      prep_conv8b_kernel<<<1, 256, 0, st>>>(raw + p.up[l].w, prepared + p.up[l].p_wb, 8);
    }
  }
  TembArgs ta{};
  ta.raw = raw; ta.prepared = prepared;
  ta.d0w = p.d0w; ta.d0b = p.d0b; ta.d1w = p.d1w; ta.d1b = p.d1b;
  ta.nblocks = (int)p.blocks.size(); ta.T = p.T;
  for (size_t i = 0; i < p.blocks.size(); ++i) {
    const ResBlockPlan& b = p.blocks[i];
    conv_w(b.c1w, b.p_c1w, 8, b.cin, 8);
    conv_w(b.c2w, b.p_c2w, 8, 8, 8);
    prep_conv8h_kernel<<<1, 256, 0, st>>>(raw + b.c1w, prepared + b.p_c1wh, b.cin);
    prep_conv8h_kernel<<<1, 256, 0, st>>>(raw + b.c2w, prepared + b.p_c2wh, 8);
    prep_conv8b_kernel<<<1, 256, 0, st>>>(raw + b.c1w, prepared + b.p_c1wb, b.cin);
    prep_conv8b_kernel<<<1, 256, 0, st>>>(raw + b.c2w, prepared + b.p_c2wb, 8);
    if (b.cin != 8) prep_nin_w_kernel<<<1, 256, 0, st>>>(raw + b.ninw, prepared + b.p_ninw, 8, b.cin);
    prep_add_kernel<<<1, 64, 0, st>>>(raw + b.c2b, b.cin != 8 ? raw + b.ninb : nullptr, prepared + b.p_bias2, 8);
    ta.tpw[i] = b.tpw; ta.tpb[i] = b.tpb; ta.c1b[i] = b.c1b; ta.dst[i] = b.p_bias1;
  }
  prep_temb_kernel<<<p.T, 64, 0, st>>>(ta);
  {
    PrepLatentArgs la{raw + p.conv_in.w, raw + p.conv_out.w, raw + p.conv_out.b, prepared + p.p_wc5, prepared + p.p_wc1,
                      prepared + p.p_bring, prepared + p.p_bsum, p.C};
    prep_latent_kernel<<<cdiv(1600 + 5184 + 72 + 8, 256), 256, 0, st>>>(la);
    prep_latent_h_kernel<<<1, 256, 0, st>>>(prepared + p.p_wc5, raw + p.conv_in.w, prepared + p.p_wc5h, prepared + p.p_wxh,
                                           prepared + p.p_wch, p.C);
  }
  GC_HIP(hipGetLastError());
  return GC_OK;
}

}
```

gencomm_amd/csrc/unet_plan.h:

```cpp
#pragma once
#include <string>
#include <vector>

#include "common.h"

namespace gc {

constexpr int kWtab3 = 3 * (3 * 64 * 4 + 64 * 2);

struct ParamEntry {
  std::string name;
  long long numel;
  long long off;
};

struct ResBlockPlan {
  int cin;
  long long n1w, n1b, c1w, c1b, tpw, tpb, n2w, n2b, c2w, c2b, ninw, ninb;
  long long p_c1w, p_c2w, p_ninw, p_bias1 , p_bias2 ;
  long long p_c1wh, p_c2wh;
  long long p_c1wb, p_c2wb;
};

struct AttnPlan {
// ... 99 lines not shown

  int emit_resblock(int blk, int in0, int in1, int level) {
    const int tmp = new_tensor(level), out = new_tensor(level);
    ops.push_back({OP_RES_CONV1, blk, {in0, in1}, {-1, -1}, tmp, level});
    ops.push_back({OP_RES_CONV2, blk, {tmp, -1}, {in0, in1}, out, level});
    return out;
  }

  const char* build(int C_, int L_, int R_, int attn_mask_, int T_, bool keep_all = false) {
    C = C_; L = L_; R = R_; T = T_; attn_mask = attn_mask_;
    if (attn_mask < 0 || attn_mask >= (1 << L_)) return "attn_mask has bits beyond the number of levels";
    if (C < 8 || C % 8 != 0) return "C must be a positive multiple of 8";
    if (L < 1 || L > 4) return "levels must be in 1..4";
    if (R < 1 || R > 4) return "res_blocks must be in 1..4";
    if (T < 1) return "T must be >= 1";
    params.clear(); blocks.clear(); ops.clear(); tensors.clear(); attns.clear();
    raw_floats = prepared_floats = 0;
    down.assign(L, ConvPlan{-1, -1, -1});
    up.assign(L, ConvPlan{-1, -1, -1});

    d0w = add("temb.dense.0.weight", 32 * 8);
    d0b = add("temb.dense.0.bias", 32);
    d1w = add("temb.dense.1.weight", 32 * 32);
    d1b = add("temb.dense.1.bias", 32);
    conv_in.w = add("conv_in.weight", 8LL * (C + 2) * 9);
    conv_in.b = add("conv_in.bias", 8);
    std::vector<std::vector<int>> down_blk(L), up_blk(L), down_att(L), up_att(L);
    for (int l = 0; l < L; ++l) {
      for (int b = 0; b < R; ++b) {
        down_blk[l].push_back(add_resblock("down." + std::to_string(l) + ".block." + std::to_string(b), 8));
        if (attn_mask >> l & 1) down_att[l].push_back(add_attn("down." + std::to_string(l) + ".attn." + std::to_string(b)));
      }
      if (l != L - 1) {
        down[l].w = add("down." + std::to_string(l) + ".downsample.conv.weight", 8 * 8 * 9);
        down[l].b = add("down." + std::to_string(l) + ".downsample.conv.bias", 8);
      }
    }
    const int mid1 = add_resblock("mid.block_1", 8), mid2 = add_resblock("mid.block_2", 8);
    for (int l = L - 1; l >= 0; --l) {
      for (int b = 0; b <= R; ++b) {
        up_blk[l].push_back(add_resblock("up." + std::to_string(l) + ".block." + std::to_string(b), 16));
        if (attn_mask >> l & 1) up_att[l].push_back(add_attn("up." + std::to_string(l) + ".attn." + std::to_string(b)));
      }
      if (l != 0) {
        up[l].w = add("up." + std::to_string(l) + ".upsample.conv.weight", 8 * 8 * 9);
        up[l].b = add("up." + std::to_string(l) + ".upsample.conv.bias", 8);
      }
    }
    nout_w = add("norm_out.weight", 8);
    nout_b = add("norm_out.bias", 8);
    conv_out.w = add("conv_out.weight", (long long)C * 8 * 9);
    conv_out.b = add("conv_out.bias", C);
    if ((int)blocks.size() > kMaxResBlocks) return "too many res-blocks";

    prepared_floats = (raw_floats + 63) / 64 * 64;
    conv_in.p_w = padd(8LL * (C + 2) * 9);
    conv_out.p_w = padd((long long)((C + 15) / 16 * 16) * 8 * 9);
    conv_out.p_wh = padd((long long)((C + 15) / 16) * kWtab3 + 64);
    for (int l = 0; l < L; ++l) {
      if (down[l].w >= 0) down[l].p_w = padd(8 * 8 * 9);
      if (up[l].w >= 0) { up[l].p_w = padd(8 * 8 * 9); up[l].p_wh = padd(kWtab3 + 64); up[l].p_wb = padd(768); }
    }
    p_wc5 = padd(1600); p_wc1 = padd(5184); p_bring = padd(72); p_bsum = padd(8);
    p_wc5h = padd(8 * (kWtab3 / 3) + 64); p_wxh = padd((long long)(C / 8) * kWtab3); p_wch = padd(kWtab3);
    for (auto& b : blocks) {
      b.p_c1w = padd(8LL * b.cin * 9);
      b.p_c2w = padd(8 * 8 * 9);
      b.p_ninw = b.cin != 8 ? padd(8LL * b.cin) : -1;
      b.p_bias1 = padd((long long)T * 8);
      b.p_bias2 = padd(8);
      b.p_c1wh = padd((long long)(b.cin / 8) * kWtab3 + 64);
      b.p_c2wh = padd(kWtab3 + 64);
      b.p_c1wb = padd((long long)(b.cin / 8) * 768);
      b.p_c2wb = padd(768);
    }

    std::vector<int> hs;
    int h = new_tensor(0);
    ops.push_back({OP_CONV_IN, 0, {-1, -1}, {-1, -1}, h, 0});
    hs.push_back(h);
    for (int l = 0; l < L; ++l) {
      for (int b = 0; b < R; ++b) {
        int t = emit_resblock(down_blk[l][b], hs.back(), -1, l);
        if (attn_mask >> l & 1) t = emit_attn(down_att[l][b], t, l);
        hs.push_back(t);
      }
      if (l != L - 1) {
        const int d = new_tensor(l + 1);
        ops.push_back({OP_DOWN, l, {hs.back(), -1}, {-1, -1}, d, l + 1});
        hs.push_back(d);
      }
    }
    h = hs.back();
    h = emit_resblock(mid1, h, -1, L - 1);
    h = emit_resblock(mid2, h, -1, L - 1);
    for (int l = L - 1; l >= 0; --l) {
      for (int b = 0; b <= R; ++b) {
        const int skip = hs.back();
        hs.pop_back();
        h = emit_resblock(up_blk[l][b], h, skip, l);
        if (attn_mask >> l & 1) h = emit_attn(up_att[l][b], h, l);
      }
      if (l != 0) {
        const int u = new_tensor(l - 1);
        ops.push_back({OP_UP, l, {h, -1}, {-1, -1}, u, l - 1});
        h = u;
      }
    }
    ops.push_back({OP_CONV_OUT, 0, {h, -1}, {-1, -1}, -1, 0});
    hs0_tensor = ops[0].dst;
    last_body_tensor = h;

    for (int i = 0; i < (int)ops.size(); ++i) {
      const Op& o = ops[i];
      for (int k = 0; k < 2; ++k) {
        if (o.src[k] >= 0) tensors[o.src[k]].last_use = i;
        if (o.res[k] >= 0) tensors[o.res[k]].last_use = i;
      }
    }
    tensors[hs0_tensor].last_use = (int)ops.size();
    slots_per_level.assign(L, 0);
    std::vector<std::vector<int>> free_slots(L);
    auto take_slot = [&](int id) {
      TensorPlan& t = tensors[id];
      if (!free_slots[t.level].empty()) {
        t.slot = free_slots[t.level].back();
        free_slots[t.level].pop_back();
      } else {
        t.slot = slots_per_level[t.level]++;
      }
    };
    for (int i = 0; i < (int)ops.size(); ++i) {
      const Op& o = ops[i];
      if (o.kind == OP_ATTN) { take_slot(o.src[1]); take_slot(o.res[0]); take_slot(o.res[1]); }
      if (o.dst >= 0) take_slot(o.dst);
      for (int k = 0; k < 4; ++k) {
        const int id = k < 2 ? o.src[k] : o.res[k - 2];
        if (id >= 0 && tensors[id].last_use == i && tensors[id].slot >= 0) {
          bool dup = false;
          for (int k2 = 0; k2 < k; ++k2) dup |= ((k2 < 2 ? o.src[k2] : o.res[k2 - 2]) == id);
          if (!dup && !keep_all) free_slots[tensors[id].level].push_back(tensors[id].slot);
        }
      }
    }
    return nullptr;
  }
};

struct UNetWorkspace {
  std::vector<int> Hl, Wl;
  std::vector<size_t> level_base, slot_bytes;
  size_t stats_bytes = 0, total = 0, kmap_off = 0, amax_off = 0;
  size_t df_words_off = 0, df_prog_off = 0;

  const char* build(const UNetPlan& p, int n, int H, int W) {
    Hl.assign(p.L, 0); Wl.assign(p.L, 0);
    Hl[0] = H; Wl[0] = W;
    for (int l = 1; l < p.L; ++l) {
      if ((Hl[l - 1] & 1) || (Wl[l - 1] & 1)) return "H and W must be even at every level that is downsampled";
      Hl[l] = Hl[l - 1] / 2; Wl[l] = Wl[l - 1] / 2;
    }
    if (Hl[p.L - 1] < 1 || Wl[p.L - 1] < 1) return "feature map too small for the number of levels";
    df_words_off = align_up(p.tensors.size() * (size_t)n * 16 * sizeof(double), 256);
    stats_bytes = align_up(df_words_off + (8 + 64 * (size_t)n + 4) * sizeof(unsigned), 256);
    size_t off = stats_bytes;
    level_base.assign(p.L, 0); slot_bytes.assign(p.L, 0);
    for (int l = 0; l < p.L; ++l) {
      slot_bytes[l] = align_up((size_t)n * 8 * Hl[l] * Wl[l] * sizeof(float), 256);
      level_base[l] = off;
      off += slot_bytes[l] * p.slots_per_level[l];
    }
    kmap_off = off;
    off += slot_bytes[0];
    amax_off = off;
    off += 256;
    df_prog_off = off;
    off += 1 << 16;
    total = off;
    return nullptr;
  }
};

}
```

gencomm_amd/enhancer.py:

```python
from __future__ import annotations

import torch
import torch.nn as nn

from . import _lib
from .runtime import PackedParams, f32c, ptr, record_len_list, require_gpu, stream_ptr, workspaces


class LinearProjection(nn.Module):
    def __init__(self, dim, heads=8, dim_head=64, dropout=0.0, bias=True):
        super().__init__()
        inner_dim = dim_head * heads
        self.heads = heads
        self.to_q = nn.Linear(dim, inner_dim, bias=bias)
        self.to_kv = nn.Linear(dim, inner_dim * 2, bias=bias)
        self.dim, self.inner_dim = dim, inner_dim


class Attention(nn.Module):
    def __init__(self, dim, num_heads, token_projection="linear", qkv_bias=True, qk_scale=None, attn_drop=0.0, proj_drop=0.0):
        super().__init__()
        self.dim, self.num_heads = dim, num_heads
        head_dim = dim // num_heads
        self.scale = qk_scale or head_dim ** -0.5
        self.angle_bins = 5
        self.angle_bias_table = nn.Parameter(torch.ones(self.angle_bins, num_heads))
        self.qkv = LinearProjection(dim, num_heads, dim // num_heads, bias=qkv_bias)
        self.token_projection = token_projection
        self.attn_drop = nn.Dropout(attn_drop)
        self.proj = nn.Linear(dim, dim)
        self.proj_drop = nn.Dropout(proj_drop)
        self.softmax = nn.Softmax(dim=-1)


class FRFN(nn.Module):
    def __init__(self, dim=32, hidden_dim=128, act_layer=nn.GELU, drop=0.0, use_eca=False):
        super().__init__()
        self.linear1 = nn.Sequential(nn.Linear(dim, hidden_dim * 2), act_layer())
        self.dwconv = nn.Sequential(nn.Conv2d(hidden_dim, hidden_dim, groups=hidden_dim, kernel_size=3, stride=1, padding=1), act_layer())
        self.linear2 = nn.Sequential(nn.Linear(hidden_dim, dim))
        self.dim, self.hidden_dim = dim, hidden_dim
        self.dim_conv = self.dim // 4
        self.dim_untouched = self.dim - self.dim_conv
        self.partial_conv3 = nn.Conv2d(self.dim_conv, self.dim_conv, 3, 1, 1, bias=False)


class SplitAttn(nn.Module):
    def __init__(self, input_dim):
        super().__init__()
        self.input_dim = input_dim
        self.fc1 = nn.Linear(input_dim, input_dim, bias=False)
        self.bn1 = nn.LayerNorm(input_dim)
        self.act1 = nn.ReLU()
        self.fc2 = nn.Linear(input_dim, input_dim, bias=False)


class Enhancer_block(nn.Module):
    def __init__(self, C, win_size, num_heads):
        super().__init__()
        self.window_size = win_size
        self.attn = Attention(dim=C, num_heads=num_heads, qkv_bias=True, qk_scale=None, attn_drop=0.1, proj_drop=0.1, token_projection="linear")
        self.mlp = FRFN(dim=C, hidden_dim=C * 2, act_layer=nn.GELU, drop=0.0)
        self.norm1 = nn.LayerNorm(C)
        self.norm2 = nn.LayerNorm(C)
        self.drop_path = nn.Identity()


class Enhancer(nn.Module):
    def __init__(self, C, win_size, num_heads):
        super().__init__()
        self.C = C
        self.block_1 = Enhancer_block(C, [4, 4], num_heads)
        self.block_2 = Enhancer_block(C, win_size, num_heads)
        self.block_3 = Enhancer_block(C, [16, 16], num_heads)
        self.split_attn = SplitAttn(C)
        self._packed = None

    def _raw_params(self, device: torch.device) -> torch.Tensor:
        if self._packed is None:
            table = _lib.enhancer_param_table(self.C)
            self._packed = PackedParams(table, _lib.check_size(_lib.lib().gencomm_enhancer_raw_floats(self.C), "gencomm_enhancer_raw_floats"))
        self._packed.update(dict(self.named_parameters()))
        require_gpu(self._packed.flat, "Enhancer parameters")
        return self._packed.flat

    def forward(self, x, affine_matrix=None, record_len=None):
        require_gpu(x, "Enhancer.forward")
        lens = record_len_list(record_len)
        n, C, H, W = x.shape
        if C != self.C:
            raise ValueError(f"Enhancer built for C={self.C}, got {C}")
        if lens is not None and sum(lens) != n:
            raise ValueError(f"record_len sums to {sum(lens)} but x has {n} agents")
        x = f32c(x)
        if torch.is_grad_enabled() and (x.requires_grad or any(p.requires_grad for p in self.parameters())):
            from .autograd import EnhancerFunction
            return EnhancerFunction.apply(self, x, *list(self.parameters()))
        return self._forward_hip(x)

    def _forward_hip(self, x: torch.Tensor) -> torch.Tensor:
        n, C, H, W = x.shape
        l = _lib.lib()
        raw = self._raw_params(x.device)
        ws = workspaces.get(x.device, _lib.check_size(l.gencomm_enhancer_workspace_bytes(n, C, H, W), "gencomm_enhancer_workspace_bytes"), "enhancer")
        out = torch.empty_like(x)
        _lib.check(l.gencomm_enhancer_fwd(ptr(raw), ptr(x), ptr(out), n, C, H, W, ptr(ws), ws.numel(), stream_ptr(x.device)),
                   "gencomm_enhancer_fwd")
        return out
```

gencomm_amd/pipeline.py:

```python
from __future__ import annotations

from typing import Optional, Sequence, Tuple

import torch

from . import _lib
from .cond_diff import GenComm
from .enhancer import Enhancer
from .fusion import MAX_AGENTS_PER_SCENE, gather_ego_thetas
from .runtime import f32c, ptr, stream_ptr


class ScenePipeline:
    def __init__(self, gencomm: GenComm, enhancer: Optional[Enhancer], record_len: Sequence[int],
                 C: int, H: int, W: int, device: torch.device, token_fast_path: Optional[bool] = None,
                 graph: bool = False):
        self.gen, self.enh = gencomm, enhancer
        self.use_graph = bool(graph)
        self._graph = None
        self.token_fast_path = (C in (64, 128, 256)) if token_fast_path is None else bool(token_fast_path)
        self.lens = [int(v) for v in record_len]
        if min(self.lens) < 1 or max(self.lens) > MAX_AGENTS_PER_SCENE:
            raise ValueError(f"each scene needs 1..{MAX_AGENTS_PER_SCENE} agents, got {self.lens}")
        self.B, self.n = len(self.lens), sum(self.lens)
        self.C, self.H, self.W = C, H, W
        self.device = torch.device(device)
        self.T = gencomm.num_timesteps
        den = gencomm.denoiser
        self.L, self.R, self.A = den.num_resolutions, den.num_res_blocks, den.attn_mask
        l = _lib.lib()
        dev = self.device
        rows, off, o = [], [0], 0
        for k in self.lens:
            rows += [o] * k
            o += k
            off.append(o)
        self.src_rows = torch.tensor(rows, dtype=torch.int32, device=dev)
        self.scene_off = torch.tensor(off, dtype=torch.int32, device=dev)
        self.theta = torch.zeros(self.n, 2, 3, dtype=torch.float64, device=dev)
        self.pred = torch.empty(self.n, C, H, W, dtype=torch.float32, device=dev)
        self.enhanced = torch.empty_like(self.pred) if enhancer is not None else self.pred
        self.fused = torch.empty(self.B, C, H, W, dtype=torch.float32, device=dev)
        ws_d = _lib.check_size(l.gencomm_denoise_workspace_bytes(self.n, C, H, W, self.L, self.R, self.A), "gencomm_denoise_workspace_bytes")
        ws_e = _lib.check_size(l.gencomm_enhancer_workspace_bytes(self.n, C, H, W), "gencomm_enhancer_workspace_bytes") if enhancer is not None else 0
        self.ws = torch.empty(max(ws_d, ws_e, 256), dtype=torch.uint8, device=dev)
        self.seed_dev = torch.zeros(1, dtype=torch.int64, device=dev)
        if self.use_graph:
            self.in_feat = torch.empty(self.n, C, H, W, dtype=torch.float32, device=dev)
            self.in_cond = torch.empty(self.n, 2, H, W, dtype=torch.float32, device=dev)
        self.refresh_params()

    def refresh_params(self) -> None:
        prepared = self.gen.denoiser.prepared_params(self.T, self.device)
        enh_raw = self.enh._raw_params(self.device) if self.enh is not None else None
        if self._graph is not None and (prepared.data_ptr() != self.prepared.data_ptr() or
                                        (enh_raw is not None and enh_raw.data_ptr() != self.enh_raw.data_ptr())):
            self._graph = None
        self.prepared = prepared
        self.sched = self.gen._sched_table(self.device)
        self.enh_raw = enh_raw

    def set_affine(self, affine_matrix: torch.Tensor) -> None:
        self.theta.copy_(gather_ego_thetas(affine_matrix, self.lens))

    def run(self, feat: torch.Tensor, cond: torch.Tensor, seed: int = 0,
            noise: Optional[Tuple[torch.Tensor, torch.Tensor]] = None) -> torch.Tensor:
        n, C, H, W = self.n, self.C, self.H, self.W
        assert feat.is_cuda and cond.is_cuda and feat.dtype == torch.float32 and cond.dtype == torch.float32
        assert feat.is_contiguous() and cond.is_contiguous()
        assert tuple(feat.shape) == (n, C, H, W) and tuple(cond.shape) == (n, 2, H, W)
        if not self.use_graph or noise is not None:
            return self._enqueue(feat, cond, seed, noise, None)
        if feat.data_ptr() != self.in_feat.data_ptr():
            self.in_feat.copy_(feat, non_blocking=True)
        if cond.data_ptr() != self.in_cond.data_ptr():
            self.in_cond.copy_(cond, non_blocking=True)
        self.seed_dev.fill_(int(seed) & 0x7FFFFFFFFFFFFFFF)
        if self._graph is None:
            cur = torch.cuda.current_stream(self.device)
            side = torch.cuda.Stream(device=self.device)
            side.wait_stream(cur)
            with torch.cuda.stream(side):
                self._enqueue(self.in_feat, self.in_cond, 0, None, self.seed_dev)
            cur.wait_stream(side)
            g = torch.cuda.CUDAGraph()
            with torch.cuda.graph(g):
                self._enqueue(self.in_feat, self.in_cond, 0, None, self.seed_dev)
            self._graph = g
        self._graph.replay()
        return self.fused

    def _enqueue(self, feat, cond, seed, noise, seed_dev) -> torch.Tensor:
        l = _lib.lib()
        st = stream_ptr(self.device)
        n, C, H, W = self.n, self.C, self.H, self.W
        n0 = sn = None
        if noise is not None:
            n0, sn = f32c(noise[0]), f32c(noise[1])
        _lib.check(l.gencomm_denoise_fwd_dseed(ptr(self.prepared), ptr(self.sched), ptr(feat), n, ptr(self.src_rows), ptr(cond),
                                               ptr(self.pred), ptr(n0), ptr(sn), seed, ptr(seed_dev), n, C, H, W, self.L, self.R, self.A,
                                               self.T, ptr(self.ws), self.ws.numel(), st), "gencomm_denoise_fwd_dseed")
        if self.enh is not None and self.token_fast_path:
            _lib.check(l.gencomm_enhancer_fwd(ptr(self.enh_raw), ptr(self.pred), None, n, C, H, W,
                                              ptr(self.ws), self.ws.numel(), st), "gencomm_enhancer_fwd")
            _lib.check(l.gencomm_warp_attfuse_tok_fwd(ptr(self.ws), ptr(self.theta), ptr(self.scene_off), ptr(self.fused),
                                                      self.B, n, C, H, W, st), "gencomm_warp_attfuse_tok_fwd")
            return self.fused
        if self.enh is not None:
            _lib.check(l.gencomm_enhancer_fwd(ptr(self.enh_raw), ptr(self.pred), ptr(self.enhanced), n, C, H, W,
                                              ptr(self.ws), self.ws.numel(), st), "gencomm_enhancer_fwd")
        _lib.check(l.gencomm_warp_attfuse_fwd(ptr(self.enhanced), ptr(self.theta), ptr(self.scene_off), ptr(self.fused),
                                              self.B, n, C, H, W, st), "gencomm_warp_attfuse_fwd")
        return self.fused
```

include/gencomm_hip.h:

```cpp
#ifndef GENCOMM_HIP_H
#define GENCOMM_HIP_H

#ifdef __cplusplus
extern "C" {
#endif

#define GENCOMM_ABI_VERSION 12

int gencomm_abi_version(void);
const char* gencomm_last_error(void);
const char* gencomm_build_info(void);

enum {
  GENCOMM_MODE_ARITH = 0, GENCOMM_MODE_SAMPLER = 1, GENCOMM_MODE_TILE_WANT = 2, GENCOMM_MODE_ENH_FUSE = 3,
  GENCOMM_MODE_CONV8H_MASK = 4, GENCOMM_MODE_XCD_REMAP = 5, GENCOMM_MODE_DATAFLOW = 6, GENCOMM_MODE_RESFUSE_EMU = 7,
  GENCOMM_MODE_TILE8 = 8, GENCOMM_MODE_BWD_STREAMS = 9, GENCOMM_MODE_PERSIST = 10
};
int gencomm_set_mode(int key, long long value);
long long gencomm_get_mode(int key);

int gencomm_timer_num_kernels(void);
const char* gencomm_timer_kernel_name(int family);
int gencomm_timer_start(int family, int capacity);
int gencomm_timer_start_mask(unsigned long long family_mask, int capacity);
int gencomm_timer_stop(double* total_ms, int* launches);
int gencomm_timer_stop_families(double* ms, int* launches, double* algorithmic_bytes, int n_families);

int gencomm_klog_start(void);
int gencomm_klog_stop(char* buf, int cap);

int gencomm_clock_probe(unsigned long long* out_dev, int spin_us, void* stream);

int gencomm_quad_iou_fwd(const float* corners_a, int n_a, const float* corners_b, int n_b, double* out, void* stream);

int gencomm_unet_num_params(int C, int levels, int res_blocks, int attn_mask);
int gencomm_unet_param_info(int C, int levels, int res_blocks, int attn_mask, int index,
                            char* name, int name_cap, long long* numel, long long* offset);
long long gencomm_unet_raw_floats(int C, int levels, int res_blocks, int attn_mask);
long long gencomm_unet_prepared_floats(int C, int levels, int res_blocks, int attn_mask, int T);
int gencomm_unet_prepare(const float* raw, float* prepared, int C, int levels, int res_blocks, int attn_mask, int T,
                         void* stream);

long long gencomm_unet_bwd_workspace_bytes(int n, int C, int H, int W, int levels, int res_blocks, int attn_mask);
int gencomm_unet_fwd_train(const float* prepared, const float* x_t, const float* cond, float* x0_out, int t,
                           int n, int C, int H, int W, int levels, int res_blocks, int attn_mask, int T,
                           void* workspace, long long workspace_bytes, void* stream);
int gencomm_unet_fwd_train_step(const float* prepared, const float* x_t, const float* cond, float* x_prev, int t, const float* sched_row,
                                const float* step_noise, unsigned long long seed, int n, int C, int H, int W, int levels, int res_blocks,
                                int attn_mask, int T, void* workspace, long long workspace_bytes, void* stream);
int gencomm_unet_bwd(const float* prepared, const float* raw, const float* x_t, const float* cond, int t, const float* grad_x0,
                     float* grad_xt, float* grad_cond, float* grad_raw, int n, int C, int H, int W, int levels, int res_blocks,
                     int attn_mask, int T, int forward_done, void* workspace, long long workspace_bytes, void* stream);

int gencomm_unet_bwd_chain(const float* prepared, const float* raw, const float* x_t, const float* cond, int t, const float* grad_x0,
                           float alpha, float beta, const float* d_prev, float* grad_xt, float* grad_cond, float* grad_raw, int n, int C,
                           int H, int W, int levels, int res_blocks, int attn_mask, int T, int forward_done, void* workspace,
                           long long workspace_bytes, void* stream);

int gencomm_conv8_fwd(const float* src, const float* w_oihw, const float* bias, float* dst, double* dstat,
                      float* scratch, int n, int H, int W, int split, void* stream);

long long gencomm_conv3x3_c16_scratch_floats(void);
int gencomm_conv3x3_c16_fwd(const float* x, int x_ct, const float* w, int transposed, float* y, int y_ct, float* scratch, int n, int H, int W,
                            void* stream);

long long gencomm_denoise_workspace_bytes(int n, int C, int H, int W, int levels, int res_blocks, int attn_mask);

int gencomm_dataflow_error(const void* workspace, int n, int C, int H, int W, int levels, int res_blocks, int attn_mask, void* stream);
int gencomm_dataflow_words(const void* workspace, int n, int C, int H, int W, int levels, int res_blocks, int attn_mask,
                           unsigned int* host_out, int count, void* stream);

int gencomm_unet_fwd(const float* prepared, const float* x_t, const float* cond, float* x0_out, int t,
                     int n, int C, int H, int W, int levels, int res_blocks, int attn_mask, int T,
                     void* workspace, long long workspace_bytes, void* stream);

int gencomm_denoise_fwd(const float* prepared, const float* sched,
                        const float* feat, int n_feat_rows, const int* src_row, const float* cond,
                        float* out, const float* noise0, const float* step_noise, unsigned long long seed,
                        int n, int C, int H, int W, int levels, int res_blocks, int attn_mask, int T,
                        void* workspace, long long workspace_bytes, void* stream);

int gencomm_denoise_fwd_dseed(const float* prepared, const float* sched,
                              const float* feat, int n_feat_rows, const int* src_row, const float* cond,
                              float* out, const float* noise0, const float* step_noise, unsigned long long seed,
                              const unsigned long long* seed_dev,
                              int n, int C, int H, int W, int levels, int res_blocks, int attn_mask, int T,
                              void* workspace, long long workspace_bytes, void* stream);

int gencomm_q_sample_fwd(const float* sched_row, const float* feat, int n_feat_rows, const int* src_row,
                         const float* noise, unsigned long long seed, unsigned int stream_id,
                         float* out, int n, int C, int H, int W, void* stream);

int gencomm_step_noise_fwd(const float* sched_row, unsigned long long seed, unsigned int stream_id, float* out,
                           int n, int C, int H, int W, int unrounded, void* stream);

int gencomm_enhancer_num_params(int C);
int gencomm_enhancer_param_info(int C, int index, char* name, int name_cap, long long* numel, long long* offset);
long long gencomm_enhancer_raw_floats(int C);
long long gencomm_enhancer_workspace_bytes(int n, int C, int H, int W);
int gencomm_enhancer_fwd(const float* raw, const float* x, float* out, int n, int C, int H, int W,
                         void* workspace, long long workspace_bytes, void* stream);

int gencomm_msgext_num_params(int C);
int gencomm_msgext_param_info(int C, int index, char* name, int name_cap, long long* numel, long long* offset);
long long gencomm_msgext_raw_floats(int C);
long long gencomm_msgext_workspace_bytes(int n, int C, int H, int W);
int gencomm_msgext_fwd(const float* raw, const float* x, float* out, int n, int C, int H, int W,
                       void* workspace, long long workspace_bytes, void* stream);

int gencomm_pillar_encode_fwd(const float* voxel_features, const int* voxel_num_points, const int* voxel_coords,
                              const float* linear_w, const float* bn_weight, const float* bn_bias,
                              const float* bn_running_mean, const float* bn_running_var,
                              float* out, float* scratch128, int M, int P, int B, int nx, int ny,
                              const float* voxel_size3, const float* pc_range6, void* stream);

int gencomm_warp_attfuse_fwd(const float* x, const double* theta, const int* scene_off, float* out,
                             int B, int n, int C, int H, int W, void* stream);

int gencomm_conv2d_prepare(const float* weight, float* prepared, int Cin, int Cout, int KH, int KW, int transposed, void* stream);
long long gencomm_conv2d_prepared_floats(int Cin, int Cout, int KH, int KW, int transposed);
int gencomm_conv2d_fold(const float* bn_weight, const float* bn_bias, const float* bn_running_mean, const float* bn_running_var,
                        const float* conv_bias, float eps, int C, float* scale, float* shift, void* stream);
int gencomm_conv2d_fwd(const float* x, const float* prepared, const float* scale, const float* shift, float* y,
                       int N, int Cin, int H, int W, int Cout, int KH, int KW, int stride, int pad, int relu,
                       int ups, int out_ctotal, int out_coff, void* stream);
int gencomm_conv2d_act_res_fwd(const float* x, const float* prepared, const float* scale, const float* shift, const float* residual,
                               float* y, int N, int Cin, int H, int W, int Cout, int KH, int KW, int stride, int pad, int act,
                               void* stream);

long long gencomm_det_workspace_bytes(int H, int W, int A);
long long gencomm_nms_workspace_bytes(void);
int gencomm_nms_max_candidates(void);
int gencomm_det_decode_fwd(const float* cls_preds, const float* reg_preds, const float* dir_preds, const float* anchors,
                           const float* transformation_matrix, int H, int W, int A, int num_bins, float score_threshold,
                           float dir_offset, int order_hwl, float* corners, float* scores, int* anchor_index, int* count,
                           int capacity, void* workspace, long long workspace_bytes, void* stream);
int gencomm_nms_rotated_fwd(const float* corners, const float* scores, const int* n_candidates, float iou_threshold, int top,
                            const float* keep_range6, float* out_boxes, float* out_scores, int* out_index, int* out_count,
                            void* workspace, long long workspace_bytes, void* stream);
int gencomm_bbox_overlaps_fwd(const float* boxes, const float* query_boxes, float* overlaps, int N, int K, void* stream);
long long gencomm_det_mc_workspace_bytes(const int* H, const int* W, int n_agents, int A);
int gencomm_det_mc_decode_fwd(const float* const* cls_preds, const float* const* reg_preds, const float* const* anchors,
                              const float* const* transformation_matrices, const int* H, const int* W, int n_agents, int A,
                              int num_class, float score_threshold, int order_hwl, float* corners, float* unprojected,
                              float* scores, int* labels, int* count, int* violations, int capacity, void* workspace,
                              long long workspace_bytes, void* stream);
int gencomm_det_mc_gather_fwd(const int* out_index, const int* out_count, const float* out_scores, const int* labels,
                              const float* unprojected, int capacity, int top, float* score_labels, float* out_unprojected,
                              void* stream);

long long gencomm_warp_attfuse_bwd_scratch_floats(int n, int H, int W);
int gencomm_warp_attfuse_bwd(const float* x, const double* theta, const int* scene_off, const float* grad_out, float* grad_x, float* scratch,
                             int B, int n, int C, int H, int W, void* stream);
int gencomm_warp_maxfuse_fwd(const float* x, const double* theta, const int* scene_off, float* out,
                             int B, int n, int C, int H, int W, void* stream);

long long gencomm_warp_maxfuse_bwd_scratch_floats(int B, int n, int C, int H, int W);
int gencomm_warp_maxfuse_bwd(const float* x, const double* theta, const int* scene_off, const float* grad_out, float* grad_x, float* scratch,
                             int B, int n, int C, int H, int W, void* stream);

int gencomm_warp_attfuse_tok_fwd(const void* enhancer_workspace, const double* theta, const int* scene_off, float* out,
                                 int B, int n, int C, int H, int W, void* stream);

int gencomm_conv2d_wgrad(const float* dy, const float* x, float* dw, float* db, int N, int Cin, int Hi, int Wi, int Cout,
                         int K, int stride, int pad, void* stream);
long long gencomm_conv2d_wgrad_scratch_floats(int N, int Cin, int Hi, int Wi, int Cout, int K, int stride, int pad);
long long gencomm_conv2d_wgrad_fixed_scratch_floats(int N, int Cin, int Hi, int Wi, int Cout, int K);
int gencomm_conv2d_wgrad_fixed(const float* dy, const float* x, float* dw, float* db, int N, int Cin, int Hi, int Wi, int Cout, int K,
                               float* scratch, long long scratch_floats, void* stream);
int gencomm_conv2d_wgrad_ws(const float* dy, const float* x, float* dw, float* db, int N, int Cin, int Hi, int Wi, int Cout,
                            int K, int stride, int pad, float* scratch, long long scratch_floats, void* stream);
int gencomm_gn_nchw_fwd(const float* x, const float* gamma, const float* beta, float* y, float* stat, float eps, int silu,
                        int n, int C, int groups, int HW, void* stream);
int gencomm_ln_nchw_fwd(const float* x, const float* gamma, const float* beta, float* out, float eps, int residual, int n, int C, int HW, void* stream);
int gencomm_ln_nchw_bwd(const float* x, const float* gamma, const float* dy, float* dx, float* dgamma, float* dbeta, float* scratch,
                        float eps, int accumulate, int n, int C, int HW, void* stream);
int gencomm_dwconv3x3_fwd(const float* x, const float* w, const float* b, float* y, int n, int C, int H, int W, int flip, void* stream);
int gencomm_dwconv3x3_wgrad(const float* x, const float* dy, float* dw, float* db, int n, int C, int H, int W, void* stream);
int gencomm_dwconv3x3_act_fwd(const float* x, int x_ct, int act, const float* w, const float* b, float* y, int n, int C, int H, int W, int flip,
                              void* stream);
int gencomm_dwconv3x3_act_wgrad(const float* x, int x_ct, int act, const float* dy, float* dw, float* db, int n, int C, int H, int W, void* stream);
int gencomm_gelu_bwd(const float* v, const float* g, float* out, long long count, void* stream);
int gencomm_lincomb_fwd(float* out, const float* x, const float* y, const float* z, float a, float b, float c, long long count, void* stream);
int gencomm_ew_slice_fwd(int op, const float* a, const float* b, const float* c, const float* d, float* o0, float* o1, int n, int nch, int HW,
                         int a_ct, int a_c0, int o0_ct, int o0_c0, int o1_ct, int o1_c0, void* stream);
int gencomm_nc_scale_fwd(const float* x, const float* a, const float* b, float* out, int n, int C, int HW, void* stream);
int gencomm_nc_dot_fwd(const float* x, const float* y, float* out, int n, int C, int HW, void* stream);

int gencomm_iou3d_pairwise_fwd(const float* boxes_a, int num_a, const float* boxes_b, int num_b, int mode, float* out, void* stream);
int gencomm_iou3d_max_boxes(void);
long long gencomm_iou3d_nms_workspace_bytes(int n);
int gencomm_iou3d_nms_fwd(const float* boxes, int n, float thresh, int normal, long long* keep, int* count,
                          void* workspace, long long workspace_bytes, void* stream);

long long gencomm_voxelize_workspace_bytes(int n);
int gencomm_voxelize_fwd(const float* points, int n, int nfeat, const float* voxel_size3, const float* range6, int max_points,
                         int max_voxels, float* voxels, int* coords_zyx, int* num_points, int* count,
                         void* workspace, long long workspace_bytes, void* stream);

long long gencomm_voxelize_batch_workspace_bytes(int n, int A, int max_voxels);
int gencomm_voxelize_batch_fwd(const float* points, int n, int nfeat, const int* offsets, int A, const float* transforms, const int* perm,
                               int mask_ego, const float* voxel_size3, const float* range6, int max_points, int max_voxels, int cap_rows,
                               float* voxels, int* coords_azyx, int* num_points, int* counts, int* total,
                               void* workspace, long long workspace_bytes, void* stream);

int gencomm_warp_affine_fwd(const float* x, const double* theta, float* out, int n, int C, int H, int W, void* stream);
int gencomm_hgt_attn_fwd(const float* qkv, const int* scene_off, float* out, int B, int heads, int dim_head, int HW, void* stream);
int gencomm_win_attn_fwd(const float* qkv, const float* pos_embedding, float* out, int n, int heads, int dim_head, int window, int H, int W,
                         void* stream);
int gencomm_warp_affine_bwd(const double* theta, const float* dout, float* dx, int n, int C, int H, int W, void* stream);
int gencomm_hgt_attn_bwd(const float* qkv, const int* scene_off, const float* dout, float* dqkv, int B, int heads, int dim_head, int HW,
                         void* stream);
long long gencomm_win_attn_bwd_scratch_floats(int n, int heads, int window, int H, int W);
int gencomm_win_attn_bwd(const float* qkv, const float* pos_embedding, const float* out, const float* dout, float* dqkv, float* dpos,
                         float* scratch, int n, int heads, int dim_head, int window, int H, int W, void* stream);
int gencomm_swap_attn_fwd(const float* qkv, const float* bias_table, const int* num_agents, float* out, int B, int L, int heads, int dim_head,
                          int window, int H, int W, int grid_mode, void* stream);
int gencomm_agent_mean_fwd(const float* x, float* out, int B, int L, long long count, void* stream);
int gencomm_swap_attn_train_fwd(const float* qkv, const float* bias_table, const int* num_agents, float* out, float* lse, int B, int L, int heads,
                                int dim_head, int window, int H, int W, int grid_mode, void* stream);
int gencomm_swap_attn_bwd(const float* qkv, const float* bias_table, const int* num_agents, const float* out, const float* lse, const float* dout,
                          float* dqkv, float* dtable, int B, int L, int heads, int dim_head, int window, int H, int W, int grid_mode,
                          void* stream);
int gencomm_v2v_warp_pairs_fwd(const float* x, const double* theta, const int* src_row, float* out, int P, int C, int H, int W, void* stream);
int gencomm_v2v_aggregate_fwd(const float* y, const float* e, const float* h, const double* theta, const int* node_row, const int* pair_off,
                              float* out, int n_nodes, int C, int H, int W, int op, int out_mode, void* stream);
int gencomm_gru_gate_fwd(const float* g, float* h, int n, int C, int HW, void* stream);
int gencomm_gru_gate_bwd(const float* g, const float* dh, float* dg, int n, int C, int HW, void* stream);
int gencomm_v2v_aggregate_train_fwd(const float* y, const float* e, const float* h, const double* theta, const int* node_row, const int* pair_off,
                                    float* out, unsigned char* winner, int n_nodes, int C, int H, int W, int op, int out_mode, void* stream);
int gencomm_v2v_aggregate_bwd(const float* dout, const double* theta, const int* node_row, const int* pair_off, const unsigned char* winner,
                              float* dy, float* de, int n_nodes, int C, int H, int W, int op, int out_mode, void* stream);
long long gencomm_v2v_warp_pairs_bwd_scratch_floats(int P);
int gencomm_v2v_warp_pairs_bwd(const float* dwarped, const double* theta, const int* src_row, const int* row_pair_off, const int* row_pairs,
                               float* dx, float* scratch, int P, int rows, int C, int H, int W, int accumulate, void* stream);
long long gencomm_umgm_param_floats(int C, int m, const int* k, int levels);
long long gencomm_umgm_workspace_bytes(long long rows, int C);
int gencomm_umgm_fwd(const float* params, const float* x, const unsigned char* keep, const float* uniforms, unsigned long long seed, int noise,
                     float* restored, long long* codes, long long* sampled, float* logits, float* code_loss, long long n, int HW, int C, int m,
                     const int* k, int levels, void* workspace, long long workspace_bytes, void* stream);
int gencomm_umgm_encode_fwd(const float* params, const float* x, long long* codes, long long n, int HW, int C, int m, const int* k, int levels,
                            void* stream);
int gencomm_umgm_decode_fwd(const float* params, const long long* codes, float* restored, long long n, int HW, int C, int m, const int* k, int levels,
                            void* stream);
int gencomm_umgm_noise_fwd(float* out, unsigned long long seed, long long n, int m, const int* k, int levels, void* stream);
long long gencomm_umgm_bwd_workspace_bytes(long long rows, int C, int m, const int* k, int levels);
int gencomm_umgm_bwd(const float* params, const float* x, const unsigned char* keep, const float* uniforms, unsigned long long seed, int noise,
                     const long long* sampled, const float* d_restored, const float* d_loss, float* dx, float* dparams, int dx_only, long long n,
                     int HW, int C, int m, const int* k, int levels, void* workspace, long long workspace_bytes, void* stream);
long long gencomm_rows_wgrad_fixed_scratch_floats(long long rows, int Co, int Ci);
int gencomm_rows_wgrad_fixed(const float* g, const float* a, float* dw, long long rows, int Co, int Ci, float* scratch, long long scratch_floats,
                             void* stream);
int gencomm_convnext_block_fwd(const float* x, const float* dw_weight, const float* dw_bias, const float* ln_weight, const float* ln_bias,
                               const float* w1, const float* b1, const float* w2, const float* b2, const float* gamma, float* y,
// ... 114 lines not shown
```

Measured before the change: 187.1.

## Cache enhancer weight tables and merge per-step stats memsets in denoise chain

Precomputes the enhancer's weight-derived tables (pconv transpose, front/back tables, scales) once per parameter generation instead of rebuilding them every forward. The colsum memset is folded into the LN kernel. In the latent denoise chain, the stats buffer is zeroed once up front together with amax (now placed adjacent), and hs0 stats ping-pong between two blocks so later steps skip their per-step stats memset. Together these cut kernel launches and memset calls per scene. The cost is extra cache-invalidation logic and a parity-based buffer scheme that must stay consistent with the latent step.

Measured after the change: 187.3 (median of 6 runs). About the same (+0.1%).

```diff
diff --git a/gencomm_amd/_lib.py b/gencomm_amd/_lib.py
--- a/gencomm_amd/_lib.py
+++ b/gencomm_amd/_lib.py
@@ -12,7 +12,7 @@
 CSRC_DIR = os.path.join(PKG_DIR, "csrc")
 LIB_PATH = os.environ.get("GENCOMM_HIP_LIB", os.path.join(PKG_DIR, "libgencomm_hip.so"))
 ABI_VERSION = 12
-MODE_ARITH, MODE_SAMPLER, MODE_TILE_WANT, MODE_ENH_FUSE, MODE_CONV8H_MASK, MODE_XCD_REMAP, MODE_DATAFLOW, MODE_RESFUSE_EMU, MODE_TILE8, MODE_BWD_STREAMS, MODE_PERSIST = range(11)
+MODE_ARITH, MODE_SAMPLER, MODE_TILE_WANT, MODE_ENH_FUSE, MODE_CONV8H_MASK, MODE_XCD_REMAP, MODE_DATAFLOW, MODE_RESFUSE_EMU, MODE_TILE8, MODE_BWD_STREAMS, MODE_PERSIST, MODE_CHAIN_FILLS = range(12)
 
 _lock = threading.Lock()
 _lib = None
@@ -62,6 +62,10 @@
     "gencomm_enhancer_raw_floats": (_ll, [_i]),
     "gencomm_enhancer_workspace_bytes": (_ll, [_i, _i, _i, _i]),
     "gencomm_enhancer_fwd": (_i, [_p, _p, _p, _i, _i, _i, _i, _p, _ll, _p]),
+    "gencomm_enhancer_prepared_floats": (_ll, [_i]),
+    "gencomm_enhancer_prepare": (_i, [_p, _p, _i, _p]),
+    "gencomm_enhancer_fwd_prepared": (_i, [_p, _p, _p, _p, _i, _i, _i, _i, _p, _ll, _p]),
+    "gencomm_denoise_stats_info": (_i, [_i, _i, _i, _i, _i, _i, _i, C.POINTER(_ll)]),
     "gencomm_msgext_num_params": (_i, [_i]),
     "gencomm_msgext_param_info": (_i, [_i, _i, C.c_char_p, _i, C.POINTER(_ll), C.POINTER(_ll)]),
     "gencomm_msgext_raw_floats": (_ll, [_i]),
diff --git a/gencomm_amd/csrc/common.h b/gencomm_amd/csrc/common.h
--- a/gencomm_amd/csrc/common.h
+++ b/gencomm_amd/csrc/common.h
@@ -62,7 +62,8 @@
   MODE_TILE8 = 8,
   MODE_BWD_STREAMS = 9,
   MODE_PERSIST = 10,
-  MODE_COUNT = 11
+  MODE_CHAIN_FILLS = 11,
+  MODE_COUNT = 12
 };
 struct Modes {
   long long v[MODE_COUNT];
diff --git a/gencomm_amd/csrc/enhancer_host.h b/gencomm_amd/csrc/enhancer_host.h
--- a/gencomm_amd/csrc/enhancer_host.h
+++ b/gencomm_amd/csrc/enhancer_host.h
@@ -72,26 +72,68 @@
 inline int enh_fuse_level(const Modes& m, int C) { return (m.split() && C == 64) ? (int)m.v[MODE_ENH_FUSE] : 0; }
 inline size_t enhancer_workspace_bytes(const EnhancerPlan& p, int n, int H, int W) { return enhancer_ws(p, n, H, W).total; }
 
+struct EnhancerTables {
+  size_t wT, tab1, tab2, wsc, total;
+};
+inline EnhancerTables enhancer_tables(const EnhancerPlan& p) {
+  const EnhancerWs w = enhancer_ws(p, 1, 1, 1);
+  EnhancerTables t{};
+  size_t off = 0;
+  auto take = [&](size_t bytes) { const size_t o = off; off += bytes; return o; };
+  t.wT = take(w.Y - w.wT);
+  t.tab1 = take(w.tab2 - w.tab1);
+  t.tab2 = take(w.wsc - w.tab2);
+  t.wsc = take(w.total - w.wsc);
+  t.total = off;
+  return t;
+}
+inline bool enh_pconv_on_f16(const EnhancerPlan& p, const Modes& m) { return m.split() && (p.dc == 16 || p.dc == 32 || p.dc == 64) && (p.C & 3) == 0; }
+inline int enhancer_tables_enqueue(const EnhancerPlan& p, const float* raw, float* wT, float* tab1, float* tab2, float* wsc,
+                                   hipStream_t st, const Modes& m, int fuse) {
+  const int C = p.C;
+  if (enh_pconv_on_f16(p, m)) {
+    const int nslice = (9 * p.dc + 31) / 32;
+    enh_prep_pconv_h_kernel<<<(p.dc / 16) * nslice * 4, 256, 0, st>>>(raw + p.pcw, wT, p.dc, nslice);
+  } else {
+    enh_prep_pconv_kernel<<<(9 * p.dc * p.dcp + 255) / 256, 256, 0, st>>>(raw + p.pcw, wT, p.dc, p.dcp);
+  }
+  if (fuse != 0) {
+    enh_wscale_kernel<<<2, 256, 0, st>>>(raw + p.l1w, (long long)2 * p.hid * C, raw + p.l2w, (long long)C * p.hid, wsc);
+    enh_prep_front_kernel<<<32, 256, 0, st>>>(raw + p.l1w, tab1, C, p.hid, wsc);
+    if (fuse >= 2) enh_prep_back_kernel<<<16, 256, 0, st>>>(raw + p.l2w, tab2, C, p.hid, wsc);
+  }
+  GC_HIP(hipGetLastError());
+  return GC_OK;
+}
+
 inline int enhancer_enqueue(const EnhancerPlan& p, const float* raw, const float* x, float* out,
-                            int n, int H, int W, char* wsp, hipStream_t st, const Modes& m) {
+                            int n, int H, int W, char* wsp, hipStream_t st, const Modes& m, const float* tables = nullptr) {
   const EnhancerWs w = enhancer_ws(p, n, H, W);
   const int HW = H * W, C = p.C;
   auto F = [&](size_t off) { return reinterpret_cast<float*>(wsp + off); };
-  GC_HIP(hipMemsetAsync(F(w.colsum), 0, (size_t)n * C * sizeof(float), st));
-
-  {
-    EnhLnArgs a{x, raw + p.n1w, raw + p.n1b, raw + p.n2w, raw + p.n2b, F(w.Y), F(w.Z), F(w.Zc), C, p.dc, HW};
+  const int fuse = enh_fuse_level(m, C);
+  const float *wT = F(w.wT), *tab1 = F(w.tab1), *tab2 = F(w.tab2), *wsc = F(w.wsc);
+  if (tables != nullptr) {
+    const EnhancerTables t = enhancer_tables(p);
+    const char* tb = reinterpret_cast<const char*>(tables);
+    wT = reinterpret_cast<const float*>(tb + t.wT); tab1 = reinterpret_cast<const float*>(tb + t.tab1);
+    tab2 = reinterpret_cast<const float*>(tb + t.tab2); wsc = reinterpret_cast<const float*>(tb + t.wsc);
+  } else if (int rc = enhancer_tables_enqueue(p, raw, F(w.wT), F(w.tab1), F(w.tab2), F(w.wsc), st, m, fuse)) {
+    return rc;
+  }
+
+  {
+    EnhLnArgs a{x, raw + p.n1w, raw + p.n1b, raw + p.n2w, raw + p.n2b, F(w.Y), F(w.Z), F(w.Zc), C, p.dc, HW, F(w.colsum)};
     const size_t sh = ((size_t)C * 65 + 256 + 128) * sizeof(float);
     if (sh > 48 * 1024) GC_HIP(hipFuncSetAttribute((const void*)enh_ln_kernel, hipFuncAttributeMaxDynamicSharedMemorySize, (int)sh));
     TimedLaunch tl(KF_ENH_LN, st);
     if (C == 64) enh_ln64_kernel<<<dim3((HW + 255) / 256, n), 256, 0, st>>>(a);
     else enh_ln_kernel<<<dim3((HW + 63) / 64, n), 256, sh, st>>>(a);
   }
-  if (m.split() && (p.dc == 16 || p.dc == 32 || p.dc == 64) && (C & 3) == 0) {
+  if (enh_pconv_on_f16(p, m)) {
     const int nslice = (9 * p.dc + 31) / 32;
-    enh_prep_pconv_h_kernel<<<(p.dc / 16) * nslice * 4, 256, 0, st>>>(raw + p.pcw, F(w.wT), p.dc, nslice);
     TimedLaunch tl(KF_ENH_PCONV, st);
-    EnhPconvHArgs a{F(w.Zc), F(w.wT), F(w.Z), C, p.dc, H, W, nslice};
+    EnhPconvHArgs a{F(w.Zc), wT, F(w.Z), C, p.dc, H, W, nslice};
     const bool wide = p.dc <= 32 && (long long)((W + 31) / 32) * ((H + 15) / 16) * n >= 256;
     const size_t sh = (size_t)18 * (wide ? 34 : 18) * p.dc * 5;
     if (wide) {
@@ -103,9 +145,8 @@
     }
   } else
   {
-    enh_prep_pconv_kernel<<<(9 * p.dc * p.dcp + 255) / 256, 256, 0, st>>>(raw + p.pcw, F(w.wT), p.dc, p.dcp);
     TimedLaunch tl(KF_ENH_PCONV, st);
-    EnhPconvArgs a{F(w.Zc), F(w.wT), F(w.Z), C, p.dc, p.dcp, H, W};
+    EnhPconvArgs a{F(w.Zc), wT, F(w.Z), C, p.dc, p.dcp, H, W};
     if (p.dc <= 32) {
       const size_t sh = (size_t)18 * 18 * (p.dc + 1) * sizeof(float);
       enh_pconv_kernel<16, 16><<<dim3((W + 15) / 16, (H + 15) / 16, n), 256, sh, st>>>(a);
@@ -115,13 +156,9 @@
       enh_pconv_kernel<16, 8><<<dim3((W + 15) / 16, (H + 7) / 8, n), 128, sh, st>>>(a);
     }
   }
-  const int fuse = enh_fuse_level(m, C);
   if (fuse != 0) {
-    enh_wscale_kernel<<<2, 256, 0, st>>>(raw + p.l1w, (long long)2 * p.hid * C, raw + p.l2w, (long long)C * p.hid, F(w.wsc));
-    enh_prep_front_kernel<<<32, 256, 0, st>>>(raw + p.l1w, F(w.tab1), C, p.hid, F(w.wsc));
-    if (fuse >= 2) enh_prep_back_kernel<<<16, 256, 0, st>>>(raw + p.l2w, F(w.tab2), C, p.hid, F(w.wsc));
-    EnhFrontArgs a{F(w.Z), F(w.tab1), raw + p.l1b, raw + p.dww, raw + p.dwb, F(w.G), C, p.hid, H, W,
-                   F(w.tab2), raw + p.l2b, F(w.Y), F(w.O), F(w.colsum), F(w.wsc)};
+    EnhFrontArgs a{F(w.Z), tab1, raw + p.l1b, raw + p.dww, raw + p.dwb, F(w.G), C, p.hid, H, W,
+                   tab2, raw + p.l2b, F(w.Y), F(w.O), F(w.colsum), wsc};
     TimedLaunch tl(KF_ENH_GEMM1, st);
     if (fuse >= 2) enh_front_h_kernel<true><<<dim3((W + 7) / 8, (H + 7) / 8, n), 256, 0, st>>>(a);
     else enh_front_h_kernel<false><<<dim3((W + 7) / 8, (H + 7) / 8, n), 256, 0, st>>>(a);
diff --git a/gencomm_amd/csrc/enhancer_kernels.h b/gencomm_amd/csrc/enhancer_kernels.h
--- a/gencomm_amd/csrc/enhancer_kernels.h
+++ b/gencomm_amd/csrc/enhancer_kernels.h
@@ -11,6 +11,7 @@
   const float* g1; const float* b1; const float* g2; const float* b2;
   float* Y; float* Z; float* Zc;
   int C, dc, HW;
+  float* colsum;
 };
 
 __global__ __launch_bounds__(256) void enh_ln_kernel(const EnhLnArgs a) {
@@ -22,6 +23,8 @@
   float* rs = mu + 64;
   const int tid = threadIdx.x, q = tid >> 6, p = tid & 63;
   const int n = blockIdx.y, p0 = blockIdx.x * 64;
+  if (blockIdx.x == 0)
+    for (int c = tid; c < C; c += 256) a.colsum[(size_t)n * C + c] = 0.f;
   const int np = min(64, a.HW - p0);
   const bool pv = p < np;
   const float* __restrict__ xp = a.x + (size_t)n * C * a.HW + p0;
@@ -76,6 +79,7 @@
   __shared__ float tile[4][64 * S];
   const int tid = threadIdx.x, wv = tid >> 6, p = tid & 63;
   const int n = blockIdx.y, p0 = (blockIdx.x * 4 + wv) * 64;
+  if (blockIdx.x == 0 && tid < C) a.colsum[(size_t)n * C + tid] = 0.f;
   if (p0 >= a.HW) return;
   const int np = min(64, a.HW - p0);
   const bool pv = p < np;
diff --git a/gencomm_amd/csrc/gencomm_abi.hip b/gencomm_amd/csrc/gencomm_abi.hip
--- a/gencomm_amd/csrc/gencomm_abi.hip
+++ b/gencomm_amd/csrc/gencomm_abi.hip
@@ -31,7 +31,7 @@
   static KernelTimer t;
   return t;
 }
-static std::atomic<long long> g_modes[MODE_COUNT] = {{0}, {0}, {0}, {2}, {-1}, {1}, {0}, {0}, {-1}, {1}, {16}};
+static std::atomic<long long> g_modes[MODE_COUNT] = {{0}, {0}, {0}, {2}, {-1}, {1}, {0}, {0}, {-1}, {1}, {16}, {1}};
 static std::atomic<bool> g_klog_armed{false};
 static std::mutex g_klog_mu;
 static std::map<std::string, int> g_klog;
@@ -66,6 +66,7 @@
   GC_CHECK_ARG(key != MODE_TILE8 || value >= -1, "GENCOMM_MODE_TILE8: -1 (automatic), 0 (off) or a positive workgroup count");
   GC_CHECK_ARG(key != MODE_BWD_STREAMS || (value >= 0 && value <= 2), "GENCOMM_MODE_BWD_STREAMS: 0 (off), 1 (automatic) or 2 (always)");
   GC_CHECK_ARG(key != MODE_PERSIST || (value >= 0 && value <= 31), "GENCOMM_MODE_PERSIST: a mask of the five layer variants (0 .. 31)");
+  GC_CHECK_ARG(key != MODE_CHAIN_FILLS || value == 0 || value == 1, "GENCOMM_MODE_CHAIN_FILLS: 0 or 1");
   g_modes[key].store(value, std::memory_order_relaxed);
   return GC_OK;
 }
@@ -471,6 +472,17 @@
   return GC_OK;
 }
 
+int gencomm_denoise_stats_info(int n, int C, int H, int W, int levels, int res_blocks, int attn_mask, long long* info) {
+  UNetPlan p;
+  if (const char* e = p.build(C, levels, res_blocks, attn_mask, 1)) return fail(GC_ERR_ARG, e);
+  if (int rc = check_dims(n, C, H, W)) return rc;
+  GC_CHECK_ARG(info != nullptr, "null pointer");
+  UNetWorkspace w;
+  if (const char* e = w.build(p, n, H, W)) return fail(GC_ERR_ARG, e);
+  info[0] = (long long)w.stats_bytes; info[1] = (long long)p.tensors.size(); info[2] = (long long)w.hs0_alt_off; info[3] = p.last_body_tensor;
+  return GC_OK;
+}
+
 int gencomm_denoise_fwd(const float* prepared, const float* sched,
                         const float* feat, int n_feat_rows, const int* src_row, const float* cond,
                         float* out, const float* noise0, const float* step_noise, unsigned long long seed,
@@ -501,14 +513,16 @@
 
   UNetCall c{&p, &w, prepared, (char*)workspace, n, H, W, st, modes_snapshot()};
   if (int rc = check_bf16_mode(c.m, p, W)) return rc;
-  GC_HIP(hipMemsetAsync(c.amax(), 0, 256, st));
+
+  const long long smode = c.m.v[MODE_SAMPLER];
+  const bool want_latent = smode == 2 || (smode == 0 && pick_tile(c.m, n, H, W) == TILE_64x16);
+  const bool latent = want_latent && T >= 2 && (W % 4) == 0;
+  const bool one_fill = latent && c.m.v[MODE_CHAIN_FILLS] != 0;
+  if (one_fill) GC_HIP(hipMemsetAsync(workspace, 0, w.stats_bytes + 256, st));
+  else GC_HIP(hipMemsetAsync(c.amax(), 0, 256, st));
   amax_kernel<<<256, 256, 0, st>>>(cond, (long long)n * 2 * H * W, c.amax());
   QSampleArgs q{feat, src_row, noise0, sched + (size_t)(T - 1) * 5, out, seed, (unsigned)T, per_agent, seed_dev, c.amax() + 1};
   launch_q_sample(q, n, philox, st);
-
-  const long long smode = c.m.v[MODE_SAMPLER];
-  const bool want_latent = smode == 2 || (smode == 0 && pick_tile(c.m, n, H, W) == TILE_64x16);
-  const bool latent = want_latent && T >= 2 && (W % 4) == 0;
   if (!latent) {
     for (int i = 0; i < T; ++i) {
       const int t = T - 1 - i;
@@ -531,10 +545,13 @@
     const int t = T - 1 - i;
     ConvOutArgs co{};
     co.out = out;
-    if (int rc = unet_enqueue_range(c, out, cond, t, 0, co, i == 0 ? 0 : 1, t == 0 ? nops : nops - 1, i != 0, i == 0)) return rc;
+    const StatFill fill = i != 0 ? FILL_KEEP_HS0 : (one_fill ? FILL_NONE : FILL_ALL);
+    if (int rc = unet_enqueue_range(c, out, cond, t, 0, co, i == 0 ? 0 : 1, t == 0 ? nops : nops - 1, fill, i == 0 || one_fill)) return rc;
     if (t > 0) {
       const float* nz = philox ? nullptr : step_noise + (size_t)i * n * per_agent;
-      if (int rc = latent_step_enqueue(c, sched + (size_t)t * 5, nz, seed, (unsigned)t, seed_dev)) return rc;
+      const int par = one_fill ? c.hs0_par ^ 1 : c.hs0_par;
+      if (int rc = latent_step_enqueue(c, sched + (size_t)t * 5, nz, seed, (unsigned)t, seed_dev, par, one_fill)) return rc;
+      c.hs0_par = par;
     }
   }
   return GC_OK;
@@ -575,6 +592,31 @@
   if ((long long)enhancer_workspace_bytes(p, n, H, W) > workspace_bytes)
     return fail(GC_ERR_WORKSPACE, "workspace too small (see gencomm_enhancer_workspace_bytes)");
   return enhancer_enqueue(p, raw, x, out, n, H, W, (char*)workspace, (hipStream_t)stream, modes_snapshot());
+}
+long long gencomm_enhancer_prepared_floats(int C) {
+  EnhancerPlan p;
+  if (const char* e = p.build(C)) { fail(GC_ERR_ARG, e); return -1; }
+  return (long long)(enhancer_tables(p).total / sizeof(float));
+}
+int gencomm_enhancer_prepare(const float* raw, float* prepared, int C, void* stream) {
+  EnhancerPlan p;
+  if (const char* e = p.build(C)) return fail(GC_ERR_ARG, e);
+  GC_CHECK_ARG(raw && prepared, "null pointer");
+  const Modes m = modes_snapshot();
+  const EnhancerTables t = enhancer_tables(p);
+  char* tb = reinterpret_cast<char*>(prepared);
+  return enhancer_tables_enqueue(p, raw, reinterpret_cast<float*>(tb + t.wT), reinterpret_cast<float*>(tb + t.tab1), reinterpret_cast<float*>(tb + t.tab2),
+                                 reinterpret_cast<float*>(tb + t.wsc), (hipStream_t)stream, m, (m.split() && C == 64) ? 2 : 0);
+}
+int gencomm_enhancer_fwd_prepared(const float* raw, const float* prepared, const float* x, float* out, int n, int C, int H, int W,
+                                  void* workspace, long long workspace_bytes, void* stream) {
+  EnhancerPlan p;
+  if (const char* e = p.build(C)) return fail(GC_ERR_ARG, e);
+  GC_CHECK_ARG(raw && x && workspace, "null pointer");
+  GC_CHECK_ARG(n >= 1 && n <= 65535 && H >= 1 && W >= 1, "bad n/H/W");
+  if ((long long)enhancer_workspace_bytes(p, n, H, W) > workspace_bytes)
+    return fail(GC_ERR_WORKSPACE, "workspace too small (see gencomm_enhancer_workspace_bytes)");
+  return enhancer_enqueue(p, raw, x, out, n, H, W, (char*)workspace, (hipStream_t)stream, modes_snapshot(), prepared);
 }
 
 int gencomm_msgext_num_params(int C) {
diff --git a/gencomm_amd/csrc/unet_host.h b/gencomm_amd/csrc/unet_host.h
--- a/gencomm_amd/csrc/unet_host.h
+++ b/gencomm_amd/csrc/unet_host.h
@@ -100,6 +100,7 @@
   int n, H, W;
   hipStream_t st;
   Modes m;
+  int hs0_par = 0;
   float* amax() const { return reinterpret_cast<float*>(wsp + ws->amax_off); }
   int is_f32(int id) const { return (!m.bf16() || id == plan->hs0_tensor) ? 1 : 0; }
 
@@ -107,7 +108,15 @@
     const TensorPlan& t = plan->tensors[id];
     return reinterpret_cast<float*>(wsp + ws->level_base[t.level] + ws->slot_bytes[t.level] * t.slot);
   }
-  double* stat_ptr(int id) const { return reinterpret_cast<double*>(wsp) + (size_t)id * n * 16; }
+  double* hs0_stat_block(int par) const {
+    return par ? reinterpret_cast<double*>(wsp + ws->hs0_alt_off) : reinterpret_cast<double*>(wsp) + (size_t)plan->hs0_tensor * n * 16;
+  }
+  double* stat_ptr(int id) const { return id == plan->hs0_tensor ? hs0_stat_block(hs0_par) : reinterpret_cast<double*>(wsp) + (size_t)id * n * 16; }
+};
+enum StatFill : int {
+  FILL_ALL = 0,
+  FILL_KEEP_HS0 = 1,
+  FILL_NONE = 2
 };
 
 inline Conv8Args conv1_args(const UNetCall& c, const Op& o, int t) {
@@ -230,12 +239,16 @@
 }
 
 inline int unet_enqueue_range(const UNetCall& c, const float* x_t, const float* cond, int t, int post,
-                              ConvOutArgs co, int first, int last, bool keep_hs0_stats, bool df_upload = true) {
+                              ConvOutArgs co, int first, int last, StatFill fill, bool df_upload = true) {
   const UNetPlan& p = *c.plan;
   const float* P = c.prepared;
-  {
-    const size_t skip = keep_hs0_stats ? (size_t)c.n * 16 * sizeof(double) : 0;
-    GC_HIP(hipMemsetAsync(c.wsp + skip, 0, c.ws->stats_bytes - skip, c.st));
+  if (fill != FILL_NONE) {
+    size_t lo = 0, hi = c.ws->stats_bytes;
+    if (fill == FILL_KEEP_HS0) {
+      if (c.hs0_par) hi = c.ws->hs0_alt_off;
+      else lo = (size_t)c.n * 16 * sizeof(double);
+    }
+    GC_HIP(hipMemsetAsync(c.wsp + lo, 0, hi - lo, c.st));
   }
   const int df_f = std::max(first, 1), df_l = std::min(last, (int)p.ops.size() - 1);
   const bool dataflow = df_eligible(c, df_f, df_l);
@@ -401,7 +414,7 @@
 }
 
 inline int unet_enqueue(const UNetCall& c, const float* x_t, const float* cond, int t, int post, ConvOutArgs co) {
-  return unet_enqueue_range(c, x_t, cond, t, post, co, 0, (int)c.plan->ops.size(), false);
+  return unet_enqueue_range(c, x_t, cond, t, post, co, 0, (int)c.plan->ops.size(), FILL_ALL);
 }
 
 inline void kmap_enqueue(const UNetCall& c, const float* cond) {
@@ -422,15 +435,15 @@
 }
 
 inline int latent_step_enqueue(const UNetCall& c, const float* sched_row, const float* noise, unsigned long long seed,
-                               unsigned stream_id, const unsigned long long* seed_dev = nullptr) {
+                               unsigned stream_id, const unsigned long long* seed_dev, int stat_par, bool stat_cleared) {
   const UNetPlan& p = *c.plan;
   const float* P = c.prepared;
-  GC_HIP(hipMemsetAsync(c.stat_ptr(p.hs0_tensor), 0, (size_t)c.n * 16 * sizeof(double), c.st));
+  if (!stat_cleared) GC_HIP(hipMemsetAsync(c.hs0_stat_block(stat_par), 0, (size_t)c.n * 16 * sizeof(double), c.st));
   LatentArgs a{};
   a.a_src = c.tensor_ptr(p.last_body_tensor); a.a_stat = c.stat_ptr(p.last_body_tensor);
   a.gamma = P + p.nout_w; a.beta = P + p.nout_b;
   a.kmap = reinterpret_cast<const float*>(c.wsp + c.ws->kmap_off);
-  a.hs0 = c.tensor_ptr(p.hs0_tensor); a.hs0_stat = c.stat_ptr(p.hs0_tensor);
+  a.hs0 = c.tensor_ptr(p.hs0_tensor); a.hs0_stat = c.hs0_stat_block(stat_par);
   a.wc5 = P + p.p_wc5; a.wc1 = P + p.p_wc1; a.bring = P + p.p_bring; a.bsum = P + p.p_bsum;
   a.wx = P + p.conv_in.p_w + 144;
   a.wc5h = P + p.p_wc5h; a.wxh = P + p.p_wxh;
diff --git a/gencomm_amd/csrc/unet_plan.h b/gencomm_amd/csrc/unet_plan.h
--- a/gencomm_amd/csrc/unet_plan.h
+++ b/gencomm_amd/csrc/unet_plan.h
@@ -275,6 +275,7 @@
   std::vector<size_t> level_base, slot_bytes;
   size_t stats_bytes = 0, total = 0, kmap_off = 0, amax_off = 0;
   size_t df_words_off = 0, df_prog_off = 0;
+  size_t hs0_alt_off = 0;
 
   const char* build(const UNetPlan& p, int n, int H, int W) {
     Hl.assign(p.L, 0); Wl.assign(p.L, 0);
@@ -285,8 +286,11 @@
     }
     if (Hl[p.L - 1] < 1 || Wl[p.L - 1] < 1) return "feature map too small for the number of levels";
     df_words_off = align_up(p.tensors.size() * (size_t)n * 16 * sizeof(double), 256);
-    stats_bytes = align_up(df_words_off + (8 + 64 * (size_t)n + 4) * sizeof(unsigned), 256);
+    hs0_alt_off = align_up(df_words_off + (8 + 64 * (size_t)n + 4) * sizeof(unsigned), 256);
+    stats_bytes = align_up(hs0_alt_off + (size_t)n * 16 * sizeof(double), 256);
     size_t off = stats_bytes;
+    amax_off = off;
+    off += 256;
     level_base.assign(p.L, 0); slot_bytes.assign(p.L, 0);
     for (int l = 0; l < p.L; ++l) {
       slot_bytes[l] = align_up((size_t)n * 8 * Hl[l] * Wl[l] * sizeof(float), 256);
@@ -295,8 +299,6 @@
     }
     kmap_off = off;
     off += slot_bytes[0];
-    amax_off = off;
-    off += 256;
     df_prog_off = off;
     off += 1 << 16;
     total = off;
diff --git a/gencomm_amd/enhancer.py b/gencomm_amd/enhancer.py
--- a/gencomm_amd/enhancer.py
+++ b/gencomm_amd/enhancer.py
@@ -75,6 +75,8 @@
         self.block_3 = Enhancer_block(C, [16, 16], num_heads)
         self.split_attn = SplitAttn(C)
         self._packed = None
+        self._prepared = None
+        self._prepared_key = None
 
     def _raw_params(self, device: torch.device) -> torch.Tensor:
         if self._packed is None:
@@ -83,6 +85,17 @@
         self._packed.update(dict(self.named_parameters()))
         require_gpu(self._packed.flat, "Enhancer parameters")
         return self._packed.flat
+
+    def prepared_tables(self, device: torch.device) -> torch.Tensor:
+        l = _lib.lib()
+        raw = self._raw_params(device)
+        key = (raw.data_ptr(), self._packed.generation, l.gencomm_get_mode(_lib.MODE_ARITH))
+        if self._prepared is None or self._prepared_key != key:
+            nflt = _lib.check_size(l.gencomm_enhancer_prepared_floats(self.C), "gencomm_enhancer_prepared_floats")
+            prepared = torch.empty(nflt, dtype=torch.float32, device=raw.device)
+            _lib.check(l.gencomm_enhancer_prepare(ptr(raw), ptr(prepared), self.C, stream_ptr(raw.device)), "gencomm_enhancer_prepare")
+            self._prepared, self._prepared_key = prepared, key
+        return self._prepared
 
     def forward(self, x, affine_matrix=None, record_len=None):
         require_gpu(x, "Enhancer.forward")
@@ -102,8 +115,9 @@
         n, C, H, W = x.shape
         l = _lib.lib()
         raw = self._raw_params(x.device)
+        tables = self.prepared_tables(x.device)
         ws = workspaces.get(x.device, _lib.check_size(l.gencomm_enhancer_workspace_bytes(n, C, H, W), "gencomm_enhancer_workspace_bytes"), "enhancer")
         out = torch.empty_like(x)
-        _lib.check(l.gencomm_enhancer_fwd(ptr(raw), ptr(x), ptr(out), n, C, H, W, ptr(ws), ws.numel(), stream_ptr(x.device)),
-                   "gencomm_enhancer_fwd")
+        _lib.check(l.gencomm_enhancer_fwd_prepared(ptr(raw), ptr(tables), ptr(x), ptr(out), n, C, H, W, ptr(ws), ws.numel(),
+                                                   stream_ptr(x.device)), "gencomm_enhancer_fwd_prepared")
         return out
diff --git a/gencomm_amd/pipeline.py b/gencomm_amd/pipeline.py
--- a/gencomm_amd/pipeline.py
+++ b/gencomm_amd/pipeline.py
@@ -53,12 +53,16 @@
     def refresh_params(self) -> None:
         prepared = self.gen.denoiser.prepared_params(self.T, self.device)
         enh_raw = self.enh._raw_params(self.device) if self.enh is not None else None
+        enh_tables = self.enh.prepared_tables(self.device) if self.enh is not None else None
         if self._graph is not None and (prepared.data_ptr() != self.prepared.data_ptr() or
-                                        (enh_raw is not None and enh_raw.data_ptr() != self.enh_raw.data_ptr())):
+                                        (enh_raw is not None and (enh_raw.data_ptr() != self.enh_raw.data_ptr() or
+                                                                  enh_tables.data_ptr() != self.enh_tables.data_ptr()))):
             self._graph = None
         self.prepared = prepared
         self.sched = self.gen._sched_table(self.device)
         self.enh_raw = enh_raw
+        self.enh_tables = enh_tables
+        self._enh_tables_arith = _lib.lib().gencomm_get_mode(_lib.MODE_ARITH)
 
     def set_affine(self, affine_matrix: torch.Tensor) -> None:
         self.theta.copy_(gather_ego_thetas(affine_matrix, self.lens))
@@ -94,6 +98,7 @@
         l = _lib.lib()
         st = stream_ptr(self.device)
         n, C, H, W = self.n, self.C, self.H, self.W
+        enh_tables = self.enh_tables if self.enh is not None and l.gencomm_get_mode(_lib.MODE_ARITH) == self._enh_tables_arith else None
         n0 = sn = None
         if noise is not None:
             n0, sn = f32c(noise[0]), f32c(noise[1])
@@ -101,14 +106,14 @@
                                                ptr(self.pred), ptr(n0), ptr(sn), seed, ptr(seed_dev), n, C, H, W, self.L, self.R, self.A,
                                                self.T, ptr(self.ws), self.ws.numel(), st), "gencomm_denoise_fwd_dseed")
         if self.enh is not None and self.token_fast_path:
-            _lib.check(l.gencomm_enhancer_fwd(ptr(self.enh_raw), ptr(self.pred), None, n, C, H, W,
-                                              ptr(self.ws), self.ws.numel(), st), "gencomm_enhancer_fwd")
+            _lib.check(l.gencomm_enhancer_fwd_prepared(ptr(self.enh_raw), ptr(enh_tables), ptr(self.pred), None, n, C, H, W,
+                                              ptr(self.ws), self.ws.numel(), st), "gencomm_enhancer_fwd_prepared")
             _lib.check(l.gencomm_warp_attfuse_tok_fwd(ptr(self.ws), ptr(self.theta), ptr(self.scene_off), ptr(self.fused),
                                                       self.B, n, C, H, W, st), "gencomm_warp_attfuse_tok_fwd")
             return self.fused
         if self.enh is not None:
-            _lib.check(l.gencomm_enhancer_fwd(ptr(self.enh_raw), ptr(self.pred), ptr(self.enhanced), n, C, H, W,
-                                              ptr(self.ws), self.ws.numel(), st), "gencomm_enhancer_fwd")
+            _lib.check(l.gencomm_enhancer_fwd_prepared(ptr(self.enh_raw), ptr(enh_tables), ptr(self.pred), ptr(self.enhanced), n, C, H, W,
+                                              ptr(self.ws), self.ws.numel(), st), "gencomm_enhancer_fwd_prepared")
         _lib.check(l.gencomm_warp_attfuse_fwd(ptr(self.enhanced), ptr(self.theta), ptr(self.scene_off), ptr(self.fused),
                                               self.B, n, C, H, W, st), "gencomm_warp_attfuse_fwd")
         return self.fused
diff --git a/include/gencomm_hip.h b/include/gencomm_hip.h
--- a/include/gencomm_hip.h
+++ b/include/gencomm_hip.h
@@ -14,7 +14,7 @@
 enum {
   GENCOMM_MODE_ARITH = 0, GENCOMM_MODE_SAMPLER = 1, GENCOMM_MODE_TILE_WANT = 2, GENCOMM_MODE_ENH_FUSE = 3,
   GENCOMM_MODE_CONV8H_MASK = 4, GENCOMM_MODE_XCD_REMAP = 5, GENCOMM_MODE_DATAFLOW = 6, GENCOMM_MODE_RESFUSE_EMU = 7,
-  GENCOMM_MODE_TILE8 = 8, GENCOMM_MODE_BWD_STREAMS = 9, GENCOMM_MODE_PERSIST = 10
+  GENCOMM_MODE_TILE8 = 8, GENCOMM_MODE_BWD_STREAMS = 9, GENCOMM_MODE_PERSIST = 10, GENCOMM_MODE_CHAIN_FILLS = 11
 };
 int gencomm_set_mode(int key, long long value);
 long long gencomm_get_mode(int key);
@@ -65,6 +65,7 @@
                             void* stream);
 
 long long gencomm_denoise_workspace_bytes(int n, int C, int H, int W, int levels, int res_blocks, int attn_mask);
+int gencomm_denoise_stats_info(int n, int C, int H, int W, int levels, int res_blocks, int attn_mask, long long* info);
 
 int gencomm_dataflow_error(const void* workspace, int n, int C, int H, int W, int levels, int res_blocks, int attn_mask, void* stream);
 int gencomm_dataflow_words(const void* workspace, int n, int C, int H, int W, int levels, int res_blocks, int attn_mask,
@@ -100,6 +101,10 @@
 long long gencomm_enhancer_workspace_bytes(int n, int C, int H, int W);
 int gencomm_enhancer_fwd(const float* raw, const float* x, float* out, int n, int C, int H, int W,
                          void* workspace, long long workspace_bytes, void* stream);
+long long gencomm_enhancer_prepared_floats(int C);
+int gencomm_enhancer_prepare(const float* raw, float* prepared, int C, void* stream);
+int gencomm_enhancer_fwd_prepared(const float* raw, const float* prepared, const float* x, float* out, int n, int C, int H, int W,
+                                  void* workspace, long long workspace_bytes, void* stream);
 
 int gencomm_msgext_num_params(int C);
 int gencomm_msgext_param_info(int C, int index, char* name, int name_cap, long long* numel, long long* offset);
```
